# CompVis/behavior-driven-video-synthesis

Hardware: AMD Instinct MI355X
Metric: frames/sec VUnet 256x256 bs=16 fwd+bwd (higher is better)
Workload: dtype f32 (operands scaled by a power of two and split into 2 fp16 terms, 3 partial products on fp16 MFMA, fp32 accumulate; weight gradients and uncovered layers: 3 bf16 terms / 6 products, fp32-input MFMA, fp32 VALU); 1 GPU; Human3.6m shape_and_pose_net VunetAlter 256x256 per-GPU bs=16 fwd+bwd, VGG19 perceptual + KL loss, fused Adam, dropout 0.05, regressor side loop off, seeded-synthetic VGG19 weights, rasterised synthetic stickmen; global_batch=16, parallelism=dp1, conv_precision=h2, hip_streams=4, hip_graph=True, graph_settle_steps=7, rccl_world_size=1, dp_backend=none

## Files before the change

behavior_driven_video_synthesis_amd/csrc/conv_p2.hip:

```cpp
#include <stdio.h>

#include <type_traits>

#include "common.h"
#include "split_h2.h"

namespace {

constexpr int P2_META = 128, P2_AMAX0 = 16, P2_NSLOT = 64;

struct P2Args {
  const uint4* x;
  const int* xmeta;
  const uint4* w;
  const float* wk;
  const float* shift;
  const uint4* mask;
  uint4* y;
  int* ymeta;
  int N, C, H, W, M;
  int relu;
};

__device__ __forceinline__ void p2_dma(uint32_t voff, const void* sbase, uint32_t lds_addr) {
  uint32_t keep;
  asm volatile("s_mov_b32 %0, m0\n\ts_mov_b32 m0, %3\n\ts_nop 0\n\tglobal_load_lds_dwordx4 %1, %2\n\ts_mov_b32 m0, %0"
               : "=&s"(keep)
               : "v"(voff), "s"(sbase), "s"(lds_addr)
               : "memory");
}
template <int N>
__device__ __forceinline__ void p2_dma_wait() {
  static_assert(N == 0 || N == 1 || N == 2 || N == 4, "counts in use");
  if constexpr (N == 0) asm volatile("s_waitcnt vmcnt(0)" ::: "memory");
  else if constexpr (N == 1) asm volatile("s_waitcnt vmcnt(1)" ::: "memory");
  else if constexpr (N == 2) asm volatile("s_waitcnt vmcnt(2)" ::: "memory");
  else asm volatile("s_waitcnt vmcnt(4)" ::: "memory");
}
__device__ __forceinline__ const void* p2_uniform_ptr(const void* p) {
  const uint64_t v = (uint64_t)p;
  const uint32_t lo = __builtin_amdgcn_readfirstlane((uint32_t)v), hi = __builtin_amdgcn_readfirstlane((uint32_t)(v >> 32));
  return (const void*)(((uint64_t)hi << 32) | lo);
}

union P2Unit {
  uint4 u;
  h2_f16x8 b;
};

__device__ __forceinline__ float p2_meta_amax(const int* meta, int lane) {
  return wave_max(__int_as_float(meta[P2_AMAX0 + (lane & (P2_NSLOT - 1))]));
}

__device__ __forceinline__ void p2_swap16(uint32_t& a, uint32_t& b) {
  const auto r = __builtin_amdgcn_permlane16_swap(a, b, false, false);
  a = r[0];
  b = r[1];
}

__device__ __forceinline__ uint32_t p2_nonzero_halves(uint32_t t) {
  typedef unsigned short u16x2 __attribute__((ext_vector_type(2)));
  u16x2 v = __builtin_bit_cast(u16x2, t);
  const u16x2 one = {1, 1}, all = {0xFFFF, 0xFFFF};
  v = __builtin_elementwise_min(v, one) * all;
  return __builtin_bit_cast(uint32_t, v);
}

template <int NW, int CT, int XBUF>
__global__ __launch_bounds__(64 * NW, NW == 8 ? 1 : 2) void conv_p2_kernel(const P2Args a) {
  static_assert(NW == 4 || NW == 8, "waves");
  static_assert(CT == 32 || CT == 16, "tile width");
  constexpr int MW = 16 * NW;
  constexpr int RT = 8, IH = RT + 2, CW = CT + 2, XPIX = IH * CW, XU = 8 * XPIX;
  constexpr int NXI = (XU + 63) / 64, XS = NXI * 64;
  constexpr int NXW = (NXI + NW - 1) / NW;
  constexpr int WU = MW * 8;
  constexpr int NWI = WU / 64 / NW;
  constexpr int PTR = CT / 16, NPT = 2 * PTR;
  static_assert(XBUF == 1 || NXW <= 8, "the next chunk's pieces ride on the first taps");
  extern __shared__ __attribute__((aligned(16))) uint4 smem[];
  uint4* const xL = smem;
  uint4* const wL = smem + XBUF * XS;

  const int tid = threadIdx.x, lane = tid & 63;
  const int wave = __builtin_amdgcn_readfirstlane(tid >> 6);
  const int mg = wave >> 2, rg = wave & 3;
  const int px = lane & 15, cg = lane >> 4;
  const int Hp = a.H + 2, Wp = a.W + 2, CB = a.C >> 3, MB = a.M >> 3;

  const unsigned bid = xcd_remap(blockIdx.x, gridDim.x);
  const int mblocks = a.M / MW;
  const int mb = bid % mblocks;
  int t = bid / mblocks;
  const int tiles_w = a.W / CT, tiles_h = a.H / RT;
  const int tx = t % tiles_w;
  t /= tiles_w;
  const int ty = t % tiles_h;
  const int n = t / tiles_h;
  const int row0 = ty * RT, col0 = tx * CT, m0 = mb * MW;

  uint32_t xoff[NXW];
#pragma unroll
  for (int i = 0; i < NXW; ++i) {
    int j = wave + NW * i;
    if (j >= NXI) j = NXI - 1;
    int u = 64 * j + lane;
    if (u >= XU) u = XU - 1;
    const int p = u / (4 * XPIX);
    int rem = u - p * 4 * XPIX;
    const int kq = rem / XPIX;
    rem -= kq * XPIX;
    const int r = rem / CW, c = rem - r * CW;
    xoff[i] = (uint32_t)((((size_t)p * a.N * CB + kq) * Hp + (row0 + r)) * Wp + col0 + c) * 16u;
  }
  const uint32_t xL_addr = (uint32_t)(uintptr_t)(__attribute__((address_space(3))) void*)xL;
  const uint32_t wL_addr = (uint32_t)(uintptr_t)(__attribute__((address_space(3))) void*)wL;
  const char* const xsrc0 = reinterpret_cast<const char*>(a.x) + (size_t)n * CB * Hp * Wp * 16;
  const size_t xchunk = (size_t)4 * Hp * Wp * 16;
  const char* const wsrc0 = reinterpret_cast<const char*>(a.w) + (size_t)mb * (MW / 16) * 128 * 16;
  const size_t wslab = (size_t)(a.M / 16) * 128 * 16;
  const uint32_t lane16 = (uint32_t)lane * 16u;

  auto issue_x = [&](int ch, int i) {
    int j = wave + NW * i;
    if (j >= NXI) j = NXI - 1;
    const int xb = XBUF == 2 ? (ch & 1) : 0;
    p2_dma(xoff[i], p2_uniform_ptr(xsrc0 + (size_t)ch * xchunk), xL_addr + (uint32_t)(xb * XS + 64 * j) * 16u);
  };
  auto issue_w = [&](int g, int buf) {
    const char* src = wsrc0 + (size_t)g * wslab;
#pragma unroll
    for (int i = 0; i < NWI; ++i) {
      const int part = wave * NWI + i;
      p2_dma(lane16, p2_uniform_ptr(src + (size_t)part * 1024), wL_addr + (uint32_t)(buf * WU + part * 64) * 16u);
    }
  };

  issue_w(0, 0);
#pragma unroll
  for (int i = 0; i < NXW; ++i) issue_x(0, i);

  float descale, descale2, sy;
  {
    const int ex = a.xmeta[0];
    const float amax_x = p2_meta_amax(a.xmeta, lane);
    const int ew = (int)a.wk[2];
    h2_pow2_pair(-(ex + ew), descale, descale2);
    const float bound = a.wk[0] * amax_x + a.wk[1];
    const int ey = h2_scale_exp(bound);
    sy = h2_pow2(ey);
    if (blockIdx.x == 0 && tid == 0) a.ymeta[0] = ey;
  }

  f32x4 acc[4][NPT], acx[4][NPT];
#pragma unroll
  for (int mt = 0; mt < 4; ++mt)
#pragma unroll
    for (int q = 0; q < NPT; ++q)
#pragma unroll
      for (int r = 0; r < 4; ++r) acc[mt][q][r] = acx[mt][q][r] = 0.f;

  p2_dma_wait<0>();
  __syncthreads();

  const int nch = a.C >> 5;
  const uint4* const wA0 = wL + (mg * 4) * 128 + lane;
  const uint4* const xB0 = xL + cg * XPIX + px + (2 * rg) * CW;

  auto chunk = [&](int ch, auto last_c) {
    constexpr bool LAST = decltype(last_c)::value;
    const uint4* const xB = xB0 + (XBUF == 2 ? (ch & 1) * XS : 0);
    const int wpar = (ch * 9) & 1;
#pragma unroll
    for (int tap = 0; tap < 9; ++tap) {
      const int kh = tap / 3, kw = tap - 3 * kh;
      const int g = ch * 9 + tap;
      const int buf = wpar ^ (tap & 1);
      constexpr bool dummy = false;
      (void)dummy;
      const bool more_w = !(LAST && tap == 8);
      const bool xpiece = XBUF == 2 && !LAST && tap < NXW;
      if (more_w) issue_w(g + 1, buf ^ 1);
      if (xpiece) issue_x(ch + 1, tap);
      const uint4* const wA = wA0 + buf * WU;
      P2Unit av[2][4], bv[2][NPT];
#pragma unroll
      for (int p = 0; p < 2; ++p) {
#pragma unroll
        for (int mt = 0; mt < 4; ++mt) av[p][mt].u = wA[(mt * 2 + p) * 64];
#pragma unroll
        for (int q = 0; q < NPT; ++q) bv[p][q].u = xB[p * 4 * XPIX + (q / PTR + kh) * CW + (q % PTR) * 16 + kw];
      }
#pragma unroll
      for (int mt = 0; mt < 4; ++mt)
#pragma unroll
        for (int q = 0; q < NPT; ++q)
          acx[mt][q] = __builtin_amdgcn_mfma_f32_16x16x32_f16(av[1][mt].b, bv[0][q].b, acx[mt][q], 0, 0, 0);
#pragma unroll
      for (int mt = 0; mt < 4; ++mt)
#pragma unroll
        for (int q = 0; q < NPT; ++q)
          acx[mt][q] = __builtin_amdgcn_mfma_f32_16x16x32_f16(av[0][mt].b, bv[1][q].b, acx[mt][q], 0, 0, 0);
#pragma unroll
      for (int mt = 0; mt < 4; ++mt)
#pragma unroll
        for (int q = 0; q < NPT; ++q)
          acc[mt][q] = __builtin_amdgcn_mfma_f32_16x16x32_f16(av[0][mt].b, bv[0][q].b, acc[mt][q], 0, 0, 0);
      __builtin_amdgcn_sched_barrier(0);
      if (more_w) {
        if (xpiece) p2_dma_wait<1>();
        else p2_dma_wait<0>();
        __syncthreads();
        if (XBUF == 1 && tap == 8) {
#pragma unroll
          for (int i = 0; i < NXW; ++i) issue_x(ch + 1, i);
          p2_dma_wait<0>();
          __syncthreads();
        }
      }
    }
  };
  for (int ch = 0; ch + 1 < nch; ++ch) chunk(ch, std::false_type{});
  chunk(nch - 1, std::true_type{});

  const bool relu = a.relu != 0;
  const size_t plane = (size_t)a.N * MB * Hp * Wp;
  float ymax = 0.f;
#pragma unroll
  for (int mt = 0; mt < 4; ++mt) {
    const int co = m0 + 64 * mg + 16 * mt + 4 * cg;
    float sh[4] = {0.f, 0.f, 0.f, 0.f};
    if (a.shift) {
      const float4 s4 = *reinterpret_cast<const float4*>(a.shift + co);
      sh[0] = s4.x; sh[1] = s4.y; sh[2] = s4.z; sh[3] = s4.w;
    }
#pragma unroll
    for (int qp = 0; qp < NPT; qp += 2) {
      uint32_t hh[2][2], ll[2][2];
#pragma unroll
      for (int s = 0; s < 2; ++s) {
        float v[4];
#pragma unroll
        for (int r = 0; r < 4; ++r) {
          float c = (acc[mt][qp + s][r] + acx[mt][qp + s][r] * (1.f / 2048.f)) * descale * descale2 + sh[r];
          c = (relu && !(c > 0.f)) ? 0.f : c;
          ymax = fmaxf(ymax, fabsf(c));
          v[r] = c * sy;
        }
        h2_split2(v[0], v[1], hh[s][0], ll[s][0]);
        h2_split2(v[2], v[3], hh[s][1], ll[s][1]);
      }
      p2_swap16(hh[0][0], hh[1][0]);
      p2_swap16(hh[0][1], hh[1][1]);
      p2_swap16(ll[0][0], ll[1][0]);
      p2_swap16(ll[0][1], ll[1][1]);
      uint4 uh = make_uint4(hh[0][0], hh[0][1], hh[1][0], hh[1][1]);
      uint4 ul = make_uint4(ll[0][0], ll[0][1], ll[1][0], ll[1][1]);
      const int q = qp + (cg & 1);
      const int orow = row0 + 2 * rg + q / PTR, ocol = col0 + (q % PTR) * 16 + px;
      const int cb = ((m0 + 64 * mg + 16 * mt) >> 3) + (cg >> 1);
      const size_t o = (((size_t)n * MB + cb) * Hp + (orow + 1)) * Wp + (ocol + 1);
      if (a.mask) {
        const uint4 mh = a.mask[o], ml = a.mask[plane + o];
        const uint32_t k0 = p2_nonzero_halves((mh.x | ml.x) & 0x7FFF7FFFu), k1 = p2_nonzero_halves((mh.y | ml.y) & 0x7FFF7FFFu);
        const uint32_t k2 = p2_nonzero_halves((mh.z | ml.z) & 0x7FFF7FFFu), k3 = p2_nonzero_halves((mh.w | ml.w) & 0x7FFF7FFFu);
        uh.x &= k0; uh.y &= k1; uh.z &= k2; uh.w &= k3;
        ul.x &= k0; ul.y &= k1; ul.z &= k2; ul.w &= k3;
      }
      a.y[o] = uh;
      a.y[plane + o] = ul;
    }
  }
  {
    const float m_ = wave_max(ymax);
    if (lane == 0)
      atomicMax(reinterpret_cast<unsigned*>(a.ymeta) + P2_AMAX0 + ((blockIdx.x * NW + wave) & (P2_NSLOT - 1)), __float_as_uint(m_));
  }
}

template <int CT>
__global__ __launch_bounds__(512, 1) void conv_p2a_kernel(const P2Args a) {
  constexpr int NW = 8, MW = 128;
  constexpr int RT = 8, IH = RT + 2, CW = CT + 2, XPIX = IH * CW, XU = 8 * XPIX;
  constexpr int NXI = (XU + 63) / 64, XS = NXI * 64;
  constexpr int NXG = (NXI + 3) / 4;
  constexpr int XPT = 2, NXT = (NXG + XPT - 1) / XPT;
  constexpr int WU = MW * 8;
  constexpr int PTR = CT / 16, NPT = 2 * PTR;
  static_assert(NXT <= 8, "the next chunk's pieces must be visible before its first tap");
  extern __shared__ __attribute__((aligned(16))) uint4 smem[];
  uint4* const xL = smem;
  uint4* const wL = smem + 2 * XS;

  const int tid = threadIdx.x, lane = tid & 63;
  const int wave = __builtin_amdgcn_readfirstlane(tid >> 6);
  const int mg = wave >> 2, rg = wave & 3;
  const int px = lane & 15, cg = lane >> 4;
  const int Hp = a.H + 2, Wp = a.W + 2, CB = a.C >> 3, MB = a.M >> 3;

  const unsigned bid = xcd_remap(blockIdx.x, gridDim.x);
  const int mblocks = a.M / MW;
  const int mb = bid % mblocks;
  int t = bid / mblocks;
  const int tiles_w = a.W / CT, tiles_h = a.H / RT;
  const int tx = t % tiles_w;
  t /= tiles_w;
  const int ty = t % tiles_h;
  const int n = t / tiles_h;
  const int row0 = ty * RT, col0 = tx * CT, m0 = mb * MW;

  uint32_t xoff[NXG];
#pragma unroll
  for (int i = 0; i < NXG; ++i) {
    int j = rg + 4 * i;
    if (j >= NXI) j = NXI - 1;
    int u = 64 * j + lane;
    if (u >= XU) u = XU - 1;
    const int p = u / (4 * XPIX);
    int rem = u - p * 4 * XPIX;
    const int kq = rem / XPIX;
    rem -= kq * XPIX;
    const int r = rem / CW, c = rem - r * CW;
    xoff[i] = (uint32_t)((((size_t)p * a.N * CB + kq) * Hp + (row0 + r)) * Wp + col0 + c) * 16u;
  }
  const uint32_t xL_addr = (uint32_t)(uintptr_t)(__attribute__((address_space(3))) void*)xL;
  const uint32_t wL_addr = (uint32_t)(uintptr_t)(__attribute__((address_space(3))) void*)wL;
  const char* const xsrc0 = reinterpret_cast<const char*>(a.x) + (size_t)n * CB * Hp * Wp * 16;
  const size_t xchunk = (size_t)4 * Hp * Wp * 16;
  const char* const wsrc0 = reinterpret_cast<const char*>(a.w) + (size_t)mb * (MW / 16) * 128 * 16;
  const size_t wslab = (size_t)(a.M / 16) * 128 * 16;
  const uint32_t lane16 = (uint32_t)lane * 16u;

  auto issue_x = [&](int ch, int i) {
    int j = rg + 4 * i;
    if (j >= NXI) j = NXI - 1;
    p2_dma(xoff[i], p2_uniform_ptr(xsrc0 + (size_t)ch * xchunk), xL_addr + (uint32_t)((ch & 1) * XS + 64 * j) * 16u);
  };
  auto issue_w = [&](int g, int buf) {
    const char* src = wsrc0 + (size_t)g * wslab;
#pragma unroll
    for (int i = 0; i < 4; ++i) {
      const int part = rg * 4 + i;
      p2_dma(lane16, p2_uniform_ptr(src + (size_t)part * 1024), wL_addr + (uint32_t)(buf * WU + part * 64) * 16u);
    }
  };

  if (mg == 0) issue_w(0, 0);
  else {
#pragma unroll
    for (int i = 0; i < NXG; ++i) issue_x(0, i);
  }
  float descale, descale2, sy;
  {
    const int ex = a.xmeta[0];
    const float amax_x = p2_meta_amax(a.xmeta, lane);
    const int ew = (int)a.wk[2];
    h2_pow2_pair(-(ex + ew), descale, descale2);
    const float bound = a.wk[0] * amax_x + a.wk[1];
    const int ey = h2_scale_exp(bound);
    sy = h2_pow2(ey);
    if (blockIdx.x == 0 && tid == 0) a.ymeta[0] = ey;
  }
  f32x4 acc[4][NPT], acx[4][NPT];
#pragma unroll
  for (int mt = 0; mt < 4; ++mt)
#pragma unroll
    for (int q = 0; q < NPT; ++q)
#pragma unroll
      for (int r = 0; r < 4; ++r) acc[mt][q][r] = acx[mt][q][r] = 0.f;
  p2_dma_wait<0>();
  __syncthreads();
  if (mg == 1) __builtin_amdgcn_s_barrier();

  const int nch = a.C >> 5;
  const uint4* const wA0 = wL + (mg * 4) * 128 + lane;
  const uint4* const xB0 = xL + cg * XPIX + px + (2 * rg) * CW;

  auto chunk = [&](int ch, auto last_c) {
    constexpr bool LAST = decltype(last_c)::value;
    const uint4* const xB = xB0 + (ch & 1) * XS;
    const int wpar = (ch * 9) & 1;
#pragma unroll
    for (int tap = 0; tap < 9; ++tap) {
      const int kh = tap / 3, kw = tap - 3 * kh;
      const int g = ch * 9 + tap;
      const int buf = wpar ^ (tap & 1);
      const bool more_w = !(LAST && tap == 8);
      if (mg == 0) {
        if (more_w) issue_w(g + 1, buf ^ 1);
      } else if (!LAST && tap < NXT) {
#pragma unroll
        for (int i = 0; i < XPT; ++i)
          if (tap * XPT + i < NXG) issue_x(ch + 1, tap * XPT + i);
      }
      const uint4* const wA = wA0 + buf * WU;
      P2Unit av[2][4], bv[2][NPT];
#pragma unroll
      for (int p = 0; p < 2; ++p) {
#pragma unroll
        for (int mt = 0; mt < 4; ++mt) av[p][mt].u = wA[(mt * 2 + p) * 64];
#pragma unroll
        for (int q = 0; q < NPT; ++q) bv[p][q].u = xB[p * 4 * XPIX + (q / PTR + kh) * CW + (q % PTR) * 16 + kw];
      }
      asm volatile("s_waitcnt lgkmcnt(0)" ::: "memory");
      __builtin_amdgcn_sched_barrier(0);
      __builtin_amdgcn_s_barrier();
      __builtin_amdgcn_sched_barrier(0);
      __builtin_amdgcn_s_setprio(1);
#pragma unroll
      for (int mt = 0; mt < 4; ++mt)
#pragma unroll
        for (int q = 0; q < NPT; ++q)
          acx[mt][q] = __builtin_amdgcn_mfma_f32_16x16x32_f16(av[1][mt].b, bv[0][q].b, acx[mt][q], 0, 0, 0);
#pragma unroll
      for (int mt = 0; mt < 4; ++mt)
#pragma unroll
        for (int q = 0; q < NPT; ++q)
          acx[mt][q] = __builtin_amdgcn_mfma_f32_16x16x32_f16(av[0][mt].b, bv[1][q].b, acx[mt][q], 0, 0, 0);
#pragma unroll
      for (int mt = 0; mt < 4; ++mt)
#pragma unroll
        for (int q = 0; q < NPT; ++q)
          acc[mt][q] = __builtin_amdgcn_mfma_f32_16x16x32_f16(av[0][mt].b, bv[0][q].b, acc[mt][q], 0, 0, 0);
      __builtin_amdgcn_s_setprio(0);
      __builtin_amdgcn_sched_barrier(0);
      p2_dma_wait<0>();
      __builtin_amdgcn_s_barrier();
      __builtin_amdgcn_sched_barrier(0);
    }
  };
  for (int ch = 0; ch + 1 < nch; ++ch) chunk(ch, std::false_type{});
  chunk(nch - 1, std::true_type{});
  if (mg == 0) __builtin_amdgcn_s_barrier();

  const bool relu = a.relu != 0;
  const size_t plane = (size_t)a.N * MB * Hp * Wp;
  float ymax = 0.f;
#pragma unroll
  for (int mt = 0; mt < 4; ++mt) {
    const int co = m0 + 64 * mg + 16 * mt + 4 * cg;
    float sh[4] = {0.f, 0.f, 0.f, 0.f};
    if (a.shift) {
      const float4 s4 = *reinterpret_cast<const float4*>(a.shift + co);
      sh[0] = s4.x; sh[1] = s4.y; sh[2] = s4.z; sh[3] = s4.w;
    }
#pragma unroll
    for (int qp = 0; qp < NPT; qp += 2) {
      uint32_t hh[2][2], ll[2][2];
#pragma unroll
      for (int s = 0; s < 2; ++s) {
        float v[4];
#pragma unroll
        for (int r = 0; r < 4; ++r) {
          float c = (acc[mt][qp + s][r] + acx[mt][qp + s][r] * (1.f / 2048.f)) * descale * descale2 + sh[r];
          c = (relu && !(c > 0.f)) ? 0.f : c;
          ymax = fmaxf(ymax, fabsf(c));
          v[r] = c * sy;
        }
        h2_split2(v[0], v[1], hh[s][0], ll[s][0]);
        h2_split2(v[2], v[3], hh[s][1], ll[s][1]);
      }
      p2_swap16(hh[0][0], hh[1][0]);
      p2_swap16(hh[0][1], hh[1][1]);
      p2_swap16(ll[0][0], ll[1][0]);
      p2_swap16(ll[0][1], ll[1][1]);
      uint4 uh = make_uint4(hh[0][0], hh[0][1], hh[1][0], hh[1][1]);
      uint4 ul = make_uint4(ll[0][0], ll[0][1], ll[1][0], ll[1][1]);
      const int q = qp + (cg & 1);
      const int orow = row0 + 2 * rg + q / PTR, ocol = col0 + (q % PTR) * 16 + px;
      const int cb = ((m0 + 64 * mg + 16 * mt) >> 3) + (cg >> 1);
      const size_t o = (((size_t)n * MB + cb) * Hp + (orow + 1)) * Wp + (ocol + 1);
      if (a.mask) {
        const uint4 mh = a.mask[o], ml = a.mask[plane + o];
        const uint32_t k0 = p2_nonzero_halves((mh.x | ml.x) & 0x7FFF7FFFu), k1 = p2_nonzero_halves((mh.y | ml.y) & 0x7FFF7FFFu);
        const uint32_t k2 = p2_nonzero_halves((mh.z | ml.z) & 0x7FFF7FFFu), k3 = p2_nonzero_halves((mh.w | ml.w) & 0x7FFF7FFFu);
        uh.x &= k0; uh.y &= k1; uh.z &= k2; uh.w &= k3;
        ul.x &= k0; ul.y &= k1; ul.z &= k2; ul.w &= k3;
      }
      a.y[o] = uh;
      a.y[plane + o] = ul;
    }
  }
  {
    const float m_ = wave_max(ymax);
    if (lane == 0)
      atomicMax(reinterpret_cast<unsigned*>(a.ymeta) + P2_AMAX0 + ((blockIdx.x * NW + wave) & (P2_NSLOT - 1)), __float_as_uint(m_));
  }
}

template <int CT>
int p2a_launch(const P2Args& a, hipStream_t st) {
  constexpr int XU = 8 * 10 * (CT + 2), XS = (XU + 63) / 64 * 64, WU = 128 * 8;
  constexpr size_t lds = (size_t)(2 * XS + 2 * WU) * 16;
  const int blocks = a.N * (a.H / 8) * (a.W / CT) * (a.M / 128);
  auto kern = conv_p2a_kernel<CT>;
  if (hipFuncSetAttribute((const void*)kern, hipFuncAttributeMaxDynamicSharedMemorySize, (int)lds) != hipSuccess) return VUNET_ERR_LAUNCH;
  VUNET_LAUNCH(kern, dim3((unsigned)blocks), dim3(512), lds, st, a);
  return vunet_check_launch();
}

template <int NW, int CT, int XBUF>
int p2_launch(const P2Args& a, hipStream_t st) {
  constexpr int XU = 8 * 10 * (CT + 2), XS = (XU + 63) / 64 * 64, WU = 16 * NW * 8;
  constexpr size_t lds = (size_t)(XBUF * XS + 2 * WU) * 16;
  const int blocks = a.N * (a.H / 8) * (a.W / CT) * (a.M / (16 * NW));
  auto kern = conv_p2_kernel<NW, CT, XBUF>;
  if (lds > 64 * 1024 && hipFuncSetAttribute((const void*)kern, hipFuncAttributeMaxDynamicSharedMemorySize, (int)lds) != hipSuccess)
    return VUNET_ERR_LAUNCH;
  VUNET_LAUNCH(kern, dim3((unsigned)blocks), dim3(64 * NW), lds, st, a);
  return vunet_check_launch();
}

}

static bool p2_shape_ok(const vunet_p2_desc* d) {
  if (!d || d->N < 1 || d->C < 32 || d->C % 32 || d->M < 64 || d->M % 64 || d->H < 8 || d->H % 8) return false;
  if (!(d->W == 16 || (d->W >= 32 && d->W % 32 == 0))) return false;
  const double plane_bytes = (double)d->N * (d->C / 8) * (d->H + 2) * (d->W + 2) * 16.0;
  return plane_bytes * 2.0 < 4.0e9;
}

extern "C" int vunet_p2_conv_supported(const vunet_p2_desc* d) { return p2_shape_ok(d) ? 1 : 0; }

static int p2_form(const vunet_p2_desc* d) {
  const long px_tiles = (long)d->N * (d->H / 8) * (d->W / (d->W == 16 ? 16 : 32));
  const int force = g_vunet_tune[VUNET_TUNE_P2_FORM];
  const bool wide = d->M % 128 == 0 && (force == 2 || force == 3 || (force != 1 && px_tiles * (d->M / 128) >= 256));
  return wide ? 8 : 4;
}

extern "C" int vunet_p2_conv(const vunet_p2_desc* d, const void* x, const int32_t* xmeta, const void* w_image, const float* wk,
                             const float* shift, const void* mask, void* y, int32_t* ymeta, void* stream) {
  if (!d || !x || !xmeta || !w_image || !wk || !y || !ymeta) return VUNET_ERR_ARG;
  if (!p2_shape_ok(d)) return VUNET_ERR_UNSUPPORTED;
  if (((uintptr_t)x | (uintptr_t)w_image | (uintptr_t)y | (uintptr_t)mask | (uintptr_t)shift) & 15) return VUNET_ERR_ARG;
  P2Args a;
  a.x = (const uint4*)x; a.xmeta = xmeta; a.w = (const uint4*)w_image; a.wk = wk; a.shift = shift; a.mask = (const uint4*)mask;
  a.y = (uint4*)y; a.ymeta = ymeta;
  a.N = d->N; a.C = d->C; a.H = d->H; a.W = d->W; a.M = d->M; a.relu = d->relu;
  hipStream_t st = (hipStream_t)stream;
  const int form = p2_form(d);
  const bool lockstep = g_vunet_tune[VUNET_TUNE_P2_FORM] == 3;
  if (d->W == 16) return form == 8 ? (lockstep ? p2_launch<8, 16, 2>(a, st) : p2a_launch<16>(a, st)) : p2_launch<4, 16, 1>(a, st);
  return form == 8 ? (lockstep ? p2_launch<8, 32, 2>(a, st) : p2a_launch<32>(a, st)) : p2_launch<4, 32, 1>(a, st);
}

extern "C" int vunet_p2_conv_variant(const vunet_p2_desc* d, char* name, int32_t len) {
  if (!d || !name || len < 32) return VUNET_ERR_ARG;
  if (!p2_shape_ok(d)) return VUNET_ERR_UNSUPPORTED;
  const int form = p2_form(d);
  if (form == 8 && g_vunet_tune[VUNET_TUNE_P2_FORM] != 3) snprintf(name, (size_t)len, "conv_p2a_kernel<%d>", d->W == 16 ? 16 : 32);
  else snprintf(name, (size_t)len, "conv_p2_kernel<%d, %d, %d>", form, d->W == 16 ? 16 : 32, form == 8 ? 2 : 1);
  return VUNET_OK;
}

namespace {
__global__ __launch_bounds__(256) void p2_wstat_kernel(const float* __restrict__ w, int Cout, int Cin, int dgrad,
                                                       float* __restrict__ rows) {
  __shared__ float red[8];
  const int r = blockIdx.x;
  float s = 0.f, m = 0.f;
  const int K = dgrad ? Cout : Cin;
  for (int i = threadIdx.x; i < K * 9; i += 256) {
    const int k = i / 9, t = i - 9 * k;
    const float v = fabsf(dgrad ? w[((size_t)k * Cin + r) * 9 + t] : w[((size_t)r * Cin + k) * 9 + t]);
    s += v;
    m = fmaxf(m, v);
  }
  s = wave_sum(s);
  m = wave_max(m);
  if ((threadIdx.x & 63) == 0) {
    red[threadIdx.x >> 6] = s;
    red[4 + (threadIdx.x >> 6)] = m;
  }
  __syncthreads();
  if (threadIdx.x == 0) {
    rows[2 * r] = (red[0] + red[1]) + (red[2] + red[3]);
    rows[2 * r + 1] = fmaxf(fmaxf(red[4], red[5]), fmaxf(red[6], red[7]));
  }
}
__global__ __launch_bounds__(256) void p2_wk_kernel(const float* __restrict__ rows, int R, const float* __restrict__ shift,
                                                    int nshift, float* __restrict__ wk) {
  __shared__ float red[12];
  float s = 0.f, m = 0.f, b = 0.f;
  for (int i = threadIdx.x; i < R; i += 256) {
    s = fmaxf(s, rows[2 * i]);
    m = fmaxf(m, rows[2 * i + 1]);
  }
  for (int i = threadIdx.x; i < nshift; i += 256) b = fmaxf(b, fabsf(shift[i]));
  s = wave_max(s);
  m = wave_max(m);
  b = wave_max(b);
  if ((threadIdx.x & 63) == 0) {
    red[threadIdx.x >> 6] = s;
    red[4 + (threadIdx.x >> 6)] = m;
    red[8 + (threadIdx.x >> 6)] = b;
  }
  __syncthreads();
  if (threadIdx.x == 0) {
    const float mx = fmaxf(fmaxf(red[4], red[5]), fmaxf(red[6], red[7]));
    wk[0] = fmaxf(fmaxf(red[0], red[1]), fmaxf(red[2], red[3])) * (1.f + 1e-6f);
    wk[1] = fmaxf(fmaxf(red[8], red[9]), fmaxf(red[10], red[11]));
    wk[2] = (float)h2_scale_exp(mx);
    wk[3] = mx;
  }
}
__global__ __launch_bounds__(256) void p2_wpack_kernel(const float* __restrict__ w, int Cout, int Cin, int dgrad,
                                                       const float* __restrict__ wk, uint4* __restrict__ img) {
  const int R = dgrad ? Cin : Cout, K = dgrad ? Cout : Cin;
  const int MT = R / 16;
  const size_t units = (size_t)(K / 32) * 9 * MT * 2 * 64;
  const float sw = h2_pow2((int)wk[2]);
  for (size_t u = (size_t)blockIdx.x * 256 + threadIdx.x; u < units; u += (size_t)gridDim.x * 256) {
    size_t v = u;
    const int l = (int)(v & 63);
    v >>= 6;
    const int p = (int)(v & 1);
    v >>= 1;
    const int mt = (int)(v % MT);
    v /= MT;
    const int tap = (int)(v % 9);
    const int ch = (int)(v / 9);
    const int row = mt * 16 + (l & 15), k0 = ch * 32 + (l >> 4) * 8;
    const int kh = tap / 3, kw = tap - 3 * kh;
    float e[8];
#pragma unroll
    for (int j = 0; j < 8; ++j) {
      const int k = k0 + j;
      const float x = dgrad ? w[(((size_t)k * Cin + row) * 3 + (2 - kh)) * 3 + (2 - kw)] : w[(((size_t)row * Cin + k) * 3 + kh) * 3 + kw];
      e[j] = x * sw;
    }
    uint32_t h[4], lo[4];
#pragma unroll
    for (int j = 0; j < 4; ++j) h2_split2(e[2 * j], e[2 * j + 1], h[j], lo[j]);
    img[u] = p ? make_uint4(lo[0], lo[1], lo[2], lo[3]) : make_uint4(h[0], h[1], h[2], h[3]);
  }
}
}

extern "C" int vunet_p2_weight_image_bytes(int32_t Cout, int32_t Cin, int32_t dgrad) {
  const int R = dgrad ? Cin : Cout, K = dgrad ? Cout : Cin;
  if (R < 16 || R % 16 || K < 32 || K % 32 || (int64_t)R * K > (1 << 22)) return 0;
  return (K / 32) * 9 * (R / 16) * 2 * 64 * 16;
}

extern "C" int vunet_p2_pack_weights(const float* w, const float* shift, int32_t Cout, int32_t Cin, int32_t dgrad, void* image,
                                     float* wk, float* workspace, void* stream) {
  if (!w || !image || !wk || !workspace) return VUNET_ERR_ARG;
  if (vunet_p2_weight_image_bytes(Cout, Cin, dgrad) == 0) return VUNET_ERR_UNSUPPORTED;
  const int R = dgrad ? Cin : Cout;
  hipStream_t st = (hipStream_t)stream;
  VUNET_LAUNCH(p2_wstat_kernel, dim3((unsigned)R), dim3(256), 0, st, w, (int)Cout, (int)Cin, (int)dgrad, workspace);
  VUNET_LAUNCH(p2_wk_kernel, dim3(1), dim3(256), 0, st, (const float*)workspace, R, dgrad ? nullptr : shift,
               (dgrad || !shift) ? 0 : (int)Cout, wk);
  const size_t units = (size_t)vunet_p2_weight_image_bytes(Cout, Cin, dgrad) / 16;
  size_t nb = (units + 255) / 256;
  if (nb > 2048) nb = 2048;
  VUNET_LAUNCH(p2_wpack_kernel, dim3((unsigned)nb), dim3(256), 0, st, w, (int)Cout, (int)Cin, (int)dgrad, (const float*)wk,
               (uint4*)image);
  return vunet_check_launch();
}

extern "C" int vunet_p2_weight_bound(const float* w, const float* shift, int32_t Cout, int32_t Cin, float* wk, float* workspace,
                                     void* stream) {
  if (!w || !wk || !workspace || Cout < 1 || Cin < 1) return VUNET_ERR_ARG;
  hipStream_t st = (hipStream_t)stream;
  VUNET_LAUNCH(p2_wstat_kernel, dim3((unsigned)Cout), dim3(256), 0, st, w, (int)Cout, (int)Cin, 0, workspace);
  VUNET_LAUNCH(p2_wk_kernel, dim3(1), dim3(256), 0, st, (const float*)workspace, (int)Cout, shift, shift ? (int)Cout : 0, wk);
  return vunet_check_launch();
}

namespace {
__global__ __launch_bounds__(256) void p2_from_nchw_kernel(const float* __restrict__ x, const float* __restrict__ amax, int n_amax,
                                                           int relu, uint4* __restrict__ y, int* __restrict__ ymeta, int N, int C,
                                                           int H, int W) {
  __shared__ float red[4];
  float m = 0.f;
  for (int i = threadIdx.x; i < n_amax; i += 256) m = fmaxf(m, amax[i]);
  m = wave_max(m);
  if ((threadIdx.x & 63) == 0) red[threadIdx.x >> 6] = m;
  __syncthreads();
  m = fmaxf(fmaxf(red[0], red[1]), fmaxf(red[2], red[3]));
  const int e = h2_scale_exp(m);
  const float s = h2_pow2(e);
  if (blockIdx.x == 0 && threadIdx.x == 0) {
    ymeta[0] = e;
    ymeta[P2_AMAX0] = __float_as_int(m);
  }
  const int CB = C >> 3, Hp = H + 2, Wp = W + 2;
  const size_t HW = (size_t)H * W, total = (size_t)N * CB * HW, plane = (size_t)N * CB * Hp * Wp;
  for (size_t i = (size_t)blockIdx.x * 256 + threadIdx.x; i < total; i += (size_t)gridDim.x * 256) {
    const int xw = (int)(i % W);
    size_t t = i / W;
    const int yh = (int)(t % H);
    t /= H;
    const float* src = x + (t * 8) * HW + (size_t)yh * W + xw;
    float v[8];
#pragma unroll
    for (int j = 0; j < 8; ++j) {
      float f = src[j * HW];
      if (relu) f = f > 0.f ? f : 0.f;
      v[j] = f * s;
    }
    uint4 h, l;
    h2_split2(v[0], v[1], h.x, l.x);
    h2_split2(v[2], v[3], h.y, l.y);
    h2_split2(v[4], v[5], h.z, l.z);
    h2_split2(v[6], v[7], h.w, l.w);
    const size_t o = (t * Hp + (yh + 1)) * Wp + (xw + 1);
    y[o] = h;
    y[plane + o] = l;
  }
}
__device__ __forceinline__ void p2_unpack(const uint4& h, const uint4& l, float inv, float* v) {
  const uint32_t hs[4] = {h.x, h.y, h.z, h.w}, ls[4] = {l.x, l.y, l.z, l.w};
#pragma unroll
  for (int j = 0; j < 4; ++j) {
    const h2_f16x2 a = __builtin_bit_cast(h2_f16x2, hs[j]), b = __builtin_bit_cast(h2_f16x2, ls[j]);
    v[2 * j] = ((float)a[0] + (float)b[0] * (1.f / 2048.f)) * inv;
    v[2 * j + 1] = ((float)a[1] + (float)b[1] * (1.f / 2048.f)) * inv;
  }
}
__global__ __launch_bounds__(256) void p2_to_nchw_kernel(const uint4* __restrict__ x, const int* __restrict__ xmeta,
                                                         float* __restrict__ y, int N, int C, int H, int W) {
  const int CB = C >> 3, Hp = H + 2, Wp = W + 2;
  const float inv = h2_pow2(-xmeta[0]);
  const size_t HW = (size_t)H * W, total = (size_t)N * CB * HW, plane = (size_t)N * CB * Hp * Wp;
  for (size_t i = (size_t)blockIdx.x * 256 + threadIdx.x; i < total; i += (size_t)gridDim.x * 256) {
    const int xw = (int)(i % W);
    size_t t = i / W;
    const int yh = (int)(t % H);
    t /= H;
    const size_t o = (t * Hp + (yh + 1)) * Wp + (xw + 1);
    float v[8];
    p2_unpack(x[o], x[plane + o], inv, v);
    float* dst = y + (t * 8) * HW + (size_t)yh * W + xw;
#pragma unroll
    for (int j = 0; j < 8; ++j) dst[j * HW] = v[j];
  }
}
}

extern "C" int vunet_p2_from_nchw(const float* x, const float* amax, int32_t n_amax, int32_t relu, void* y, int32_t* ymeta,
                                  int32_t N, int32_t C, int32_t H, int32_t W, void* stream) {
  if (!x || !amax || n_amax < 1 || !y || !ymeta || C % 8 || N < 1) return VUNET_ERR_ARG;
  const size_t total = (size_t)N * (C / 8) * H * W;
  size_t nb = (total + 255) / 256;
  if (nb > 4096) nb = 4096;
  VUNET_LAUNCH(p2_from_nchw_kernel, dim3((unsigned)nb), dim3(256), 0, (hipStream_t)stream, x, amax, (int)n_amax, (int)relu, (uint4*)y,
               (int*)ymeta, (int)N, (int)C, (int)H, (int)W);
  return vunet_check_launch();
}

extern "C" int vunet_p2_to_nchw(const void* x, const int32_t* xmeta, float* y, int32_t N, int32_t C, int32_t H, int32_t W,
                                void* stream) {
  if (!x || !xmeta || !y || C % 8 || N < 1) return VUNET_ERR_ARG;
  const size_t total = (size_t)N * (C / 8) * H * W;
  size_t nb = (total + 255) / 256;
  if (nb > 4096) nb = 4096;
  VUNET_LAUNCH(p2_to_nchw_kernel, dim3((unsigned)nb), dim3(256), 0, (hipStream_t)stream, (const uint4*)x, (const int*)xmeta, y, (int)N,
               (int)C, (int)H, (int)W);
  return vunet_check_launch();
}
```

behavior_driven_video_synthesis_amd/csrc/planes.hip:

```cpp
#include "common.h"
#include "split_h2.h"

namespace {

constexpr int P2_AMAX0 = 16, P2_NSLOT = 64;

__device__ __forceinline__ void p2_unpack8(const uint4& h, const uint4& l, float inv, float* v) {
  const uint32_t hs[4] = {h.x, h.y, h.z, h.w}, ls[4] = {l.x, l.y, l.z, l.w};
#pragma unroll
  for (int j = 0; j < 4; ++j) {
    const h2_f16x2 a = __builtin_bit_cast(h2_f16x2, hs[j]), b = __builtin_bit_cast(h2_f16x2, ls[j]);
    v[2 * j] = ((float)a[0] + (float)b[0] * (1.f / 2048.f)) * inv;
    v[2 * j + 1] = ((float)a[1] + (float)b[1] * (1.f / 2048.f)) * inv;
  }
}
__device__ __forceinline__ void p2_pack8(const float* v, float s, uint4& h, uint4& l) {
  h2_split2(v[0] * s, v[1] * s, h.x, l.x);
  h2_split2(v[2] * s, v[3] * s, h.y, l.y);
  h2_split2(v[4] * s, v[5] * s, h.z, l.z);
  h2_split2(v[6] * s, v[7] * s, h.w, l.w);
}
__device__ __forceinline__ float block_sum4(float v, float* red) {
  v = wave_sum(v);
  __syncthreads();
  if ((threadIdx.x & 63) == 0) red[threadIdx.x >> 6] = v;
  __syncthreads();
  return red[0] + red[1] + red[2] + red[3];
}
__device__ __forceinline__ float meta_amax(const int* meta) {
  return wave_max(__int_as_float(meta[P2_AMAX0 + (threadIdx.x & (P2_NSLOT - 1))]));
}
__device__ __forceinline__ void publish_amax(int* meta, float vmax) {
  const float m = wave_max(vmax);
  if ((threadIdx.x & 63) == 0)
    atomicMax(reinterpret_cast<unsigned*>(meta) + P2_AMAX0 + ((blockIdx.x * 4u + (threadIdx.x >> 6)) & (P2_NSLOT - 1)), __float_as_uint(m));
}

__global__ __launch_bounds__(256) void p2_finish_sum_kernel(const float* partial, int nb, float* out, float scale) {
  __shared__ float red[4];
  float s = 0.f;
  for (int i = threadIdx.x; i < nb; i += 256) s += partial[i];
  const float t = block_sum4(s, red);
  if (threadIdx.x == 0) out[0] += scale * t;
}

__global__ __launch_bounds__(256) void p2_l1_partial_kernel(const uint4* __restrict__ t, const int* __restrict__ tmeta,
                                                            const uint4* __restrict__ p, const int* __restrict__ pmeta,
                                                            float* __restrict__ partial, size_t plane) {
  __shared__ float red[4];
  const float it = h2_pow2(-tmeta[0]), ip = h2_pow2(-pmeta[0]);
  float s = 0.f;
  for (size_t i = (size_t)blockIdx.x * 256 + threadIdx.x; i < plane; i += (size_t)gridDim.x * 256) {
    float a[8], b[8];
    p2_unpack8(t[i], t[plane + i], it, a);
    p2_unpack8(p[i], p[plane + i], ip, b);
    s += ((fabsf(a[0] - b[0]) + fabsf(a[1] - b[1])) + (fabsf(a[2] - b[2]) + fabsf(a[3] - b[3]))) +
         ((fabsf(a[4] - b[4]) + fabsf(a[5] - b[5])) + (fabsf(a[6] - b[6]) + fabsf(a[7] - b[7])));
  }
  const float tot = block_sum4(s, red);
  if (threadIdx.x == 0) partial[blockIdx.x] = tot;
}

template <bool L1>
__global__ __launch_bounds__(256) void p2_pool_fwd_kernel(const uint4* __restrict__ t, const int* __restrict__ tmeta,
                                                          const uint4* __restrict__ p, const int* __restrict__ pmeta,
                                                          float* __restrict__ partial, uint4* __restrict__ y, int* __restrict__ ymeta,
                                                          int NCB, int H, int W) {
  __shared__ float red[4];
  const int Ho = H >> 1, Wo = W >> 1, Wp = W + 2, Wpo = Wo + 2;
  const size_t plane = (size_t)NCB * (H + 2) * Wp, plane_o = (size_t)NCB * (Ho + 2) * Wpo, total = (size_t)NCB * Ho * Wo;
  const float ip = h2_pow2(-pmeta[0]);
  const float it = L1 ? h2_pow2(-tmeta[0]) : 0.f;
  if (blockIdx.x == 0 && threadIdx.x < 64) {
    if (threadIdx.x == 0) ymeta[0] = pmeta[0];
    ymeta[P2_AMAX0 + threadIdx.x] = pmeta[P2_AMAX0 + threadIdx.x];
  }
  float s = 0.f;
  for (size_t o = (size_t)blockIdx.x * 256 + threadIdx.x; o < total; o += (size_t)gridDim.x * 256) {
    const int xo = (int)(o % Wo);
    size_t r = o / Wo;
    const int yo = (int)(r % Ho);
    const size_t ncb = r / Ho;
    const size_t i0 = (ncb * (H + 2) + (2 * yo + 1)) * Wp + (2 * xo + 1);
    const size_t off[4] = {i0, i0 + 1, i0 + Wp, i0 + Wp + 1};
    uint32_t hs[4][4], ls[4][4];
    float v[4][8];
#pragma unroll
    for (int e = 0; e < 4; ++e) {
      const uint4 h = p[off[e]], l = p[plane + off[e]];
      hs[e][0] = h.x; hs[e][1] = h.y; hs[e][2] = h.z; hs[e][3] = h.w;
      ls[e][0] = l.x; ls[e][1] = l.y; ls[e][2] = l.z; ls[e][3] = l.w;
      p2_unpack8(h, l, ip, v[e]);
    }
    if (L1) {
#pragma unroll
      for (int e = 0; e < 4; ++e) {
        float a[8];
        p2_unpack8(t[off[e]], t[plane + off[e]], it, a);
#pragma unroll
        for (int j = 0; j < 8; ++j) s += fabsf(a[j] - v[e][j]);
      }
    }
    uint32_t oh[4] = {0, 0, 0, 0}, ol[4] = {0, 0, 0, 0};
#pragma unroll
    for (int j = 0; j < 8; ++j) {
      const float m = fmaxf(fmaxf(v[0][j], v[1][j]), fmaxf(v[2][j], v[3][j]));
      const int k = v[0][j] == m ? 0 : (v[1][j] == m ? 1 : (v[2][j] == m ? 2 : 3));
      const uint32_t hsel = k == 0 ? hs[0][j >> 1] : (k == 1 ? hs[1][j >> 1] : (k == 2 ? hs[2][j >> 1] : hs[3][j >> 1]));
      const uint32_t lsel = k == 0 ? ls[0][j >> 1] : (k == 1 ? ls[1][j >> 1] : (k == 2 ? ls[2][j >> 1] : ls[3][j >> 1]));
      const uint32_t keep = (j & 1) ? 0xFFFF0000u : 0x0000FFFFu;
      oh[j >> 1] |= hsel & keep;
      ol[j >> 1] |= lsel & keep;
    }
    const size_t oo = (ncb * (Ho + 2) + (yo + 1)) * Wpo + (xo + 1);
    y[oo] = make_uint4(oh[0], oh[1], oh[2], oh[3]);
    y[plane_o + oo] = make_uint4(ol[0], ol[1], ol[2], ol[3]);
  }
  if (L1) {
    const float tot = block_sum4(s, red);
    if (threadIdx.x == 0) partial[blockIdx.x] = tot;
  }
}

__global__ __launch_bounds__(256) void p2_l1_bwd_kernel(const uint4* __restrict__ t, const int* __restrict__ tmeta,
                                                        const uint4* __restrict__ p, const int* __restrict__ pmeta,
                                                        const uint4* __restrict__ add, const int* __restrict__ addmeta,
                                                        uint4* __restrict__ g, int* __restrict__ gmeta, float gscale,
                                                        const float* __restrict__ gout, int NCB, int H, int W) {
  const float c = gscale * (gout ? gout[0] : 1.f);
  const float bound = (add ? meta_amax(addmeta) : 0.f) + fabsf(c);
  const int eg = h2_scale_exp(bound);
  const float sg = h2_pow2(eg);
  if (blockIdx.x == 0 && threadIdx.x == 0) gmeta[0] = eg;
  const float it = h2_pow2(-tmeta[0]), ip = h2_pow2(-pmeta[0]), ia = add ? h2_pow2(-addmeta[0]) : 0.f;
  const int Wp = W + 2;
  const size_t plane = (size_t)NCB * (H + 2) * Wp, total = (size_t)NCB * H * W;
  float vmax = 0.f;
  for (size_t o = (size_t)blockIdx.x * 256 + threadIdx.x; o < total; o += (size_t)gridDim.x * 256) {
    const int xw = (int)(o % W);
    size_t r = o / W;
    const int yh = (int)(r % H);
    const size_t i = ((r / H) * (H + 2) + (yh + 1)) * Wp + (xw + 1);
    float a[8], b[8], d[8];
    p2_unpack8(t[i], t[plane + i], it, a);
    p2_unpack8(p[i], p[plane + i], ip, b);
    if (add) p2_unpack8(add[i], add[plane + i], ia, d);
#pragma unroll
    for (int j = 0; j < 8; ++j) {
      const float df = b[j] - a[j];
      float v = (add ? d[j] : 0.f) + (df > 0.f ? c : (df < 0.f ? -c : 0.f));
      if (!(b[j] > 0.f)) v = 0.f;
      d[j] = v;
      vmax = fmaxf(vmax, fabsf(v));
    }
    uint4 h, l;
    p2_pack8(d, sg, h, l);
    g[i] = h;
    g[plane + i] = l;
  }
  publish_amax(gmeta, vmax);
}

template <bool L1>
__global__ __launch_bounds__(256) void p2_pool_bwd_kernel(const uint4* __restrict__ t, const int* __restrict__ tmeta,
                                                          const uint4* __restrict__ p, const int* __restrict__ pmeta,
                                                          const uint4* __restrict__ dy, const int* __restrict__ dymeta,
                                                          uint4* __restrict__ g, int* __restrict__ gmeta, float gscale,
                                                          const float* __restrict__ gout, int NCB, int H, int W) {
  const float c = L1 ? gscale * (gout ? gout[0] : 1.f) : 0.f;
  const float bound = meta_amax(dymeta) + fabsf(c);
  const int eg = h2_scale_exp(bound);
  const float sg = h2_pow2(eg);
  if (blockIdx.x == 0 && threadIdx.x == 0) gmeta[0] = eg;
  const float ip = h2_pow2(-pmeta[0]), idy = h2_pow2(-dymeta[0]);
  const float it = L1 ? h2_pow2(-tmeta[0]) : 0.f;
  const int Ho = H >> 1, Wo = W >> 1, Wp = W + 2, Wpo = Wo + 2;
  const size_t plane = (size_t)NCB * (H + 2) * Wp, plane_o = (size_t)NCB * (Ho + 2) * Wpo, total = (size_t)NCB * Ho * Wo;
  float vmax = 0.f;
  for (size_t o = (size_t)blockIdx.x * 256 + threadIdx.x; o < total; o += (size_t)gridDim.x * 256) {
    const int xo = (int)(o % Wo);
    size_t r = o / Wo;
    const int yo = (int)(r % Ho);
    const size_t ncb = r / Ho;
    const size_t i0 = (ncb * (H + 2) + (2 * yo + 1)) * Wp + (2 * xo + 1);
    const size_t off[4] = {i0, i0 + 1, i0 + Wp, i0 + Wp + 1};
    const size_t oo = (ncb * (Ho + 2) + (yo + 1)) * Wpo + (xo + 1);
    float v[4][8], gy[8];
#pragma unroll
    for (int e = 0; e < 4; ++e) p2_unpack8(p[off[e]], p[plane + off[e]], ip, v[e]);
    p2_unpack8(dy[oo], dy[plane_o + oo], idy, gy);
    float res[4][8];
#pragma unroll
    for (int j = 0; j < 8; ++j) {
      const float m = fmaxf(fmaxf(v[0][j], v[1][j]), fmaxf(v[2][j], v[3][j]));
      const int k = v[0][j] == m ? 0 : (v[1][j] == m ? 1 : (v[2][j] == m ? 2 : 3));
#pragma unroll
      for (int e = 0; e < 4; ++e) res[e][j] = k == e ? gy[j] : 0.f;
    }
#pragma unroll
    for (int e = 0; e < 4; ++e) {
      float a[8];
      if (L1) p2_unpack8(t[off[e]], t[plane + off[e]], it, a);
#pragma unroll
      for (int j = 0; j < 8; ++j) {
        float x = res[e][j];
        if (L1) {
          const float df = v[e][j] - a[j];
          x += df > 0.f ? c : (df < 0.f ? -c : 0.f);
        }
        if (!(v[e][j] > 0.f)) x = 0.f;
        res[e][j] = x;
        vmax = fmaxf(vmax, fabsf(x));
      }
      uint4 h, l;
      p2_pack8(res[e], sg, h, l);
      g[off[e]] = h;
      g[plane + off[e]] = l;
    }
  }
  publish_amax(gmeta, vmax);
}

inline unsigned grid_for(size_t n, unsigned cap) {
  size_t b = (n + 255) / 256;
  if (b > cap) b = cap;
  if (b < 1) b = 1;
  return (unsigned)b;
}

}

extern "C" int vunet_p2_l1_fwd(const void* t, const int32_t* tmeta, const void* p, const int32_t* pmeta, float* partial, float* out,
                               float weight, int32_t N, int32_t C, int32_t H, int32_t W, void* stream) {
  if (!t || !tmeta || !p || !pmeta || !partial || !out || C % 8 || N < 1) return VUNET_ERR_ARG;
  const size_t plane = (size_t)N * (C / 8) * (H + 2) * (W + 2);
  const unsigned nb = grid_for(plane, 1024);
  hipStream_t st = (hipStream_t)stream;
  VUNET_LAUNCH(p2_l1_partial_kernel, dim3(nb), dim3(256), 0, st, (const uint4*)t, (const int*)tmeta, (const uint4*)p, (const int*)pmeta,
               partial, plane);
  VUNET_LAUNCH(p2_finish_sum_kernel, dim3(1), dim3(256), 0, st, (const float*)partial, (int)nb, out,
               weight / ((float)N * C * H * W));
  return vunet_check_launch();
}

extern "C" int vunet_p2_pool_fwd(const void* t, const int32_t* tmeta, const void* p, const int32_t* pmeta, float* partial, float* out,
                                 float weight, void* y, int32_t* ymeta, int32_t N, int32_t C, int32_t H, int32_t W, void* stream) {
  if (!p || !pmeta || !y || !ymeta || C % 8 || N < 1 || (H & 1) || (W & 1)) return VUNET_ERR_ARG;
  if (t && (!tmeta || !partial || !out)) return VUNET_ERR_ARG;
  const int NCB = N * (C / 8);
  const size_t total = (size_t)NCB * (H / 2) * (W / 2);
  const unsigned nb = grid_for(total, 1024);
  hipStream_t st = (hipStream_t)stream;
  if (t) {
    VUNET_LAUNCH(p2_pool_fwd_kernel<true>, dim3(nb), dim3(256), 0, st, (const uint4*)t, (const int*)tmeta, (const uint4*)p,
                 (const int*)pmeta, partial, (uint4*)y, (int*)ymeta, NCB, (int)H, (int)W);
    VUNET_LAUNCH(p2_finish_sum_kernel, dim3(1), dim3(256), 0, st, (const float*)partial, (int)nb, out,
                 weight / ((float)N * C * H * W));
  } else {
    VUNET_LAUNCH(p2_pool_fwd_kernel<false>, dim3(nb), dim3(256), 0, st, (const uint4*)nullptr, (const int*)nullptr, (const uint4*)p,
                 (const int*)pmeta, (float*)nullptr, (uint4*)y, (int*)ymeta, NCB, (int)H, (int)W);
  }
  return vunet_check_launch();
}

extern "C" int vunet_p2_l1_bwd(const void* t, const int32_t* tmeta, const void* p, const int32_t* pmeta, const void* add,
                               const int32_t* addmeta, void* g, int32_t* gmeta, float gscale, const float* gout, int32_t N, int32_t C,
                               int32_t H, int32_t W, void* stream) {
  if (!t || !tmeta || !p || !pmeta || !g || !gmeta || C % 8 || N < 1 || (add && !addmeta)) return VUNET_ERR_ARG;
  const int NCB = N * (C / 8);
  const size_t total = (size_t)NCB * H * W;
  VUNET_LAUNCH(p2_l1_bwd_kernel, dim3(grid_for(total, 2048)), dim3(256), 0, (hipStream_t)stream, (const uint4*)t, (const int*)tmeta,
               (const uint4*)p, (const int*)pmeta, (const uint4*)add, (const int*)addmeta, (uint4*)g, (int*)gmeta, gscale, gout, NCB,
               (int)H, (int)W);
  return vunet_check_launch();
}

extern "C" int vunet_p2_pool_bwd(const void* t, const int32_t* tmeta, const void* p, const int32_t* pmeta, const void* dy,
                                 const int32_t* dymeta, void* g, int32_t* gmeta, float gscale, const float* gout, int32_t N, int32_t C,
                                 int32_t H, int32_t W, void* stream) {
  if (!p || !pmeta || !dy || !dymeta || !g || !gmeta || C % 8 || N < 1 || (H & 1) || (W & 1) || (t && !tmeta)) return VUNET_ERR_ARG;
  const int NCB = N * (C / 8);
  const size_t total = (size_t)NCB * (H / 2) * (W / 2);
  const unsigned nb = grid_for(total, 2048);
  hipStream_t st = (hipStream_t)stream;
  if (t)
    VUNET_LAUNCH(p2_pool_bwd_kernel<true>, dim3(nb), dim3(256), 0, st, (const uint4*)t, (const int*)tmeta, (const uint4*)p,
                 (const int*)pmeta, (const uint4*)dy, (const int*)dymeta, (uint4*)g, (int*)gmeta, gscale, gout, NCB, (int)H, (int)W);
  else
    VUNET_LAUNCH(p2_pool_bwd_kernel<false>, dim3(nb), dim3(256), 0, st, (const uint4*)nullptr, (const int*)nullptr, (const uint4*)p,
                 (const int*)pmeta, (const uint4*)dy, (const int*)dymeta, (uint4*)g, (int*)gmeta, 0.f, (const float*)nullptr, NCB, (int)H,
                 (int)W);
  return vunet_check_launch();
}
```

behavior_driven_video_synthesis_amd/models/imagenet_pretrained.py:

```python
from __future__ import annotations

import math

import torch
from torch import nn

from .. import ops
from ..lib.modules import Conv2d

VGG19_CFG = [64, 64, "M", 128, 128, "M", 256, 256, 256, 256, "M", 512, 512, 512, 512, "M", 512, 512, 512, 512, "M"]


class _Marker(nn.Module):

    def __init__(self, kind):
        super().__init__()
        self.kind = kind


class VGG19(nn.Module):

    def __init__(self, width_div: int = 1):
        super().__init__()
        layers, cin = [], 3
        for v in VGG19_CFG:
            if v == "M":
                layers.append(_Marker("pool"))
            else:
                cout = max(v // width_div, 4)
                layers += [Conv2d(cin, cout, 3, padding=1), _Marker("relu")]
                cin = cout
        self.features = nn.Sequential(*layers)

    def init_synthetic(self, seed: int = 1234):
        g = torch.Generator().manual_seed(seed)
        with torch.no_grad():
            for m in self.features:
                if isinstance(m, Conv2d):
                    cout, cin = m.weight.shape[:2]
                    m.weight.copy_(torch.randn(cout, cin, 3, 3, generator=g) * math.sqrt(2.0 / (cin * 9)))
                    m.bias.copy_((torch.rand(cout, generator=g) - 0.5) * 0.1)
        return self


def vgg19(pretrained: bool = False, weights_path: str = None, width_div: int = 1, seed: int = 1234,
          synthetic: bool = False) -> VGG19:
    if pretrained and weights_path is None and not synthetic:
        import warnings
        warnings.warn("vgg19(pretrained=True) without weights_path: torchvision's weights cannot be fetched here, "
                      "using SEEDED-SYNTHETIC VGG19 weights (pass weights_path=<torchvision vgg19 state dict>, or "
                      "synthetic=True to silence this)", stacklevel=2)
    net = VGG19(width_div)
    if weights_path is not None:
        sd = torch.load(weights_path, map_location="cpu")
        net.load_state_dict({k: v for k, v in sd.items() if k.startswith("features.")})
    else:
        net.init_synthetic(seed)
    return net


def _adopt_features(features: nn.Sequential) -> nn.Sequential:
    mods = list(features)
    if all(isinstance(m, (Conv2d, _Marker)) for m in mods):
        return features
    layers = []
    for m in mods:
        if isinstance(m, nn.Conv2d):
            if m.kernel_size != (3, 3) or m.stride != (1, 1) or m.padding != (1, 1) or m.bias is None:
                raise NotImplementedError("PerceptualVGG expects VGG-style 3x3 / stride 1 / pad 1 convolutions with bias")
            c = Conv2d(m.in_channels, m.out_channels, 3, padding=1)
            with torch.no_grad():
                c.weight.copy_(m.weight)
                c.bias.copy_(m.bias)
            layers.append(c.to(m.weight.device))
        elif isinstance(m, nn.ReLU):
            layers.append(_Marker("relu"))
        elif isinstance(m, nn.MaxPool2d):
            layers.append(_Marker("pool"))
        else:
            raise NotImplementedError(f"PerceptualVGG: unexpected module {type(m).__name__} in vgg.features")
    return nn.Sequential(*layers)


_p2_switch = {"on": __import__("os").environ.get("VUNET_VGG_P2", "1") != "0"}


def enable_p2(on: bool = True):
    _p2_switch["on"] = bool(on)


class _P2Target(dict):

    planes = None
    generation = 0


class _P2Engine:

    def __init__(self, program, n, h, w, device):
        self.program, self.geo, self.device = program, (n, h, w), device
        self.roles = {}
        self.generation = 0
        self.pred_generation = 0

    @staticmethod
    def build_program(mods, last, taps):
        steps, first, i = [], None, 0
        while i < len(mods):
            name, m = mods[i]
            if int(name) > last:
                break
            if isinstance(m, Conv2d):
                nxt = mods[i + 1] if i + 1 < len(mods) else None
                if nxt is None or not (isinstance(nxt[1], _Marker) and nxt[1].kind == "relu"):
                    return None
                tap = taps.get(nxt[0])
                if first is None:
                    if tap is not None:
                        return None
                    first = m
                else:
                    steps.append(("conv", m, tap))
                i += 2
            elif isinstance(m, _Marker) and m.kind == "pool":
                if first is None:
                    return None
                steps.append(("pool",))
                i += 1
            else:
                return None
        if first is None or not steps or steps[-1][0] != "conv" or steps[-1][2] is None:
            return None
        return first, steps

    def shapes(self):
        first, steps = self.program
        n, h, w = self.geo
        c = first.weight.shape[0]
        out = [(c, h, w)]
        for st in steps:
            if st[0] == "pool":
                if h % 2 or w % 2:
                    return None
                h, w = h // 2, w // 2
            else:
                m = st[1]
                if m.weight.shape[1] != c or tuple(m.weight.shape[2:]) != (3, 3) or not ops.p2_conv_supported(n, c, h, w, m.weight.shape[0]):
                    return None
                if not ops.p2_conv_supported(n, m.weight.shape[0], h, w, c):
                    return None
                c = m.weight.shape[0]
            out.append((c, h, w))
        return out

    def _role(self, role):
        st = self.roles.get(role)
        if st is None:
            shp = self.shapes()
            n = self.geo[0]
            L = len(shp)
            metas = torch.zeros(3 * L, ops.P2_META_INTS, device=self.device, dtype=torch.int32)
            acts = [ops.Planes((n, c, h, w), self.device, meta=metas[k]) for k, (c, h, w) in enumerate(shp)]
            st = self.roles[role] = {"metas": metas, "A": acts, "G": [None] * L, "U": [None] * L, "shp": shp}
        return st

    def _grad_buf(self, st, kind, k):
        lst = st[kind]
        if lst[k] is None:
            c, h, w = st["shp"][k]
            L = len(st["shp"])
            lst[k] = ops.Planes((self.geo[0], c, h, w), self.device, meta=st["metas"][(1 if kind == "G" else 2) * L + k])
        return lst[k]

    @staticmethod
    def _weights(m):
        w = m.__dict__.get("_p2w")
        if w is None or w.weight is not m.weight:
            w = ops.P2Weights(m.weight, m.bias)
            object.__setattr__(m, "_p2w", w)
        return w

    def _first(self):
        m = self.program[0]
        stamp = (m.weight.data_ptr(), m.weight._version, m.bias._version)
        rec = m.__dict__.get("_p2first")
        if rec is None or rec[0] != stamp:
            w, b = m.weight.detach().contiguous(), m.bias.detach().contiguous()
            wt_f, wt_d, _, shift, _, _, wx_d = ops.pack_weights(w, None, b, None, None, 3, 0, 1, True)
            wk = torch.empty(4, device=w.device, dtype=torch.float32)
            work = torch.empty(2 * w.shape[0], device=w.device, dtype=torch.float32)
            ops._call("vunet_p2_weight_bound", ops._p(w), ops._p(b), int(w.shape[0]), 3, ops._p(wk), ops._p(work), ops._stream())
            rec = (stamp, wt_f, wt_d, shift, wx_d, wk)
            object.__setattr__(m, "_p2first", rec)
        return rec

    def forward(self, role, xp, targets=None, tap_weights=None):
        st = self._role(role)
        st["metas"].zero_()
        A = st["A"]
        _, wt_f, _, shift, _, wk = self._first()
        n, _, h, w = xp.shape
        amax = ops._tagged_amax(xp)
        if amax is None:
            amax = ops.absmax_partials(xp)
        ops._call("vunet_p2_conv_first", ops._p(xp), ops._p(amax), 512, ops._p(wt_f), int(wt_f.shape[1]), ops._p(shift), ops._p(wk),
                  ops._p(A[0].buf), ops._p(A[0].meta), n, h, w, A[0].shape[1], ops._stream())
        taps, losses = {}, {}
        steps = self.program[1]
        for k, step in enumerate(steps, start=1):
            if step[0] == "conv":
                ops.p2_conv(A[k - 1], self._weights(step[1]), A[k], relu=True)
                tap = step[2]
                if tap is not None:
                    taps[tap] = A[k]
                    pool_next = k < len(steps) and steps[k][0] == "pool"
                    if targets is not None and not pool_next:
                        losses[tap] = ops.p2_l1_fwd(targets[tap], A[k], tap_weights[tap])
            else:
                prev = steps[k - 2] if k >= 2 else None
                tap = prev[2] if (prev is not None and prev[0] == "conv") else None
                if targets is not None and tap is not None:
                    losses[tap] = ops.p2_pool_fwd(A[k - 1], A[k], t=targets[tap], weight=tap_weights[tap])
                else:
                    ops.p2_pool_fwd(A[k - 1], A[k])
        return taps, losses

    def backward(self, targets, tap_weights, gouts):
        st = self.roles["p"]
        A, steps = st["A"], self.program[1]
        L = len(steps)

        def tap_scale(tap, k):
            c, h, w = st["shp"][k]
            return float(tap_weights[tap]) / (self.geo[0] * c * h * w)

        def has(tap):
            return tap is not None and gouts.get(tap) is not None
        k = L
        top = steps[L - 1][2]
        D = None
        if has(top):
            D = ops.p2_l1_bwd(targets[top], A[L], None, self._grad_buf(st, "G", L), tap_scale(top, L), gouts[top])
        while k >= 1:
            step = steps[k - 1]
            if step[0] == "pool":
                prev = steps[k - 2]
                tap = prev[2] if has(prev[2]) else None
                if D is None and tap is None:
                    k -= 1
                    continue
                if D is None:
                    D = ops.p2_l1_bwd(targets[tap], A[k - 1], None, self._grad_buf(st, "G", k - 1), tap_scale(tap, k - 1), gouts[tap])
                else:
                    D = ops.p2_pool_bwd(A[k - 1], D, self._grad_buf(st, "G", k - 1), t=None if tap is None else targets[tap],
                                        gscale=0.0 if tap is None else tap_scale(tap, k - 1), gout=None if tap is None else gouts[tap])
                k -= 1
                continue
            below = steps[k - 2] if k >= 2 else None
            if D is None:
                tap = below[2] if (below is not None and below[0] == "conv" and has(below[2])) else None
                if tap is not None:
                    D = ops.p2_l1_bwd(targets[tap], A[k - 1], None, self._grad_buf(st, "G", k - 1), tap_scale(tap, k - 1), gouts[tap])
                k -= 1
                continue
            wts = self._weights(step[1])
            if below is None:
                D = ops.p2_conv(D, wts, self._grad_buf(st, "G", 0), dgrad=True, mask=A[0])
            elif below[0] == "pool":
                D = ops.p2_conv(D, wts, self._grad_buf(st, "G", k - 1), dgrad=True)
            elif has(below[2]):
                up = ops.p2_conv(D, wts, self._grad_buf(st, "U", k - 1), dgrad=True)
                D = ops.p2_l1_bwd(targets[below[2]], A[k - 1], up, self._grad_buf(st, "G", k - 1), tap_scale(below[2], k - 1),
                                  gouts[below[2]])
            else:
                D = ops.p2_conv(D, wts, self._grad_buf(st, "G", k - 1), dgrad=True, mask=A[k - 1])
            k -= 1
        if D is None:
            return None
        _, _, wt_d, _, wx_d, _ = self._first()
        n, h, w = self.geo
        c0 = st["shp"][0][0]
        dconv = D.to_nchw()
        dx = torch.empty(n, 3, h, w, device=self.device, dtype=torch.float32)
        d = ops.ConvDesc(N=n, C1=c0, C2=0, Hs=h, Ws=w, M=3, m_off=0, Mpad=wt_d.shape[1], Ho=h, Wo=w, KH=3, KW=3, stride=1, pad=1,
                         mode=1, in_act=ops.ACT_NONE, in_slope=0.0, drop_p=0.0, drop_seed=0, out_act=ops.ACT_NONE, d2s=0)
        ops._conv_gather(d, dconv, None, wt_d, None, None, None, dx, wx_d)
        return dx


class P2VggLoss(torch.autograd.Function):

    @staticmethod
    def forward(ctx, xp, engine, target, tap_weights, names):
        _, losses = engine.forward("p", xp, target.planes, tap_weights)
        engine.pred_generation += 1
        ctx.engine, ctx.target, ctx.tap_weights, ctx.names = engine, target, tap_weights, names
        ctx.generation, ctx.pred_generation = target.generation, engine.pred_generation
        return tuple(losses[n] for n in names)

    @staticmethod
    def backward(ctx, *gouts):
        if ctx.target.generation != ctx.generation:
            raise RuntimeError("P2VggLoss.backward: the target features were overwritten by a later target pass of the same "
                               "PerceptualVGG (its planes buffers are persistent): run forward + backward per target")
        if ctx.engine.pred_generation != ctx.pred_generation:
            raise RuntimeError("P2VggLoss.backward: a later vgg_loss() of the same PerceptualVGG and input geometry has overwritten "
                               "this pass's activations (persistent planes buffers): call backward() before the next vgg_loss(), "
                               "or switch the planes path off (models.imagenet_pretrained.enable_p2(False)) for this use")
        g = ctx.engine.backward(ctx.target.planes, ctx.tap_weights,
                                {n: (None if go is None else go.contiguous()) for n, go in zip(ctx.names, gouts)})
        return g, None, None, None, None


class PerceptualVGG(nn.Module):

    def __init__(self, vgg, weights):
        super().__init__()
        feats = vgg.module.features if isinstance(vgg, nn.DataParallel) else vgg.features
        self.vgg_layers = _adopt_features(feats)
        self.loss_weights = weights
        self.register_buffer("mean", torch.tensor([0.485, 0.456, 0.406], dtype=torch.float).view(1, 3, 1, 1))
        self.register_buffer("std", torch.tensor([0.229, 0.224, 0.225], dtype=torch.float).view(1, 3, 1, 1))
        self.target_layers = {"3": "relu1_2", "8": "relu2_2", "13": "relu3_2", "22": "relu4_2", "31": "relu5_2"}
        for p in self.vgg_layers.parameters():
            p.requires_grad_(False)

    def _walk(self, x, on_tap, on_tap_pool=None):
        x = on_tap("input", ops.VggPreprocess.apply(x))
        last = max(int(k) for k in self.target_layers)
        mods = list(self.vgg_layers._modules.items())
        i = 0
        while i < len(mods):
            name, m = mods[i]
            if int(name) > last:
                break
            if isinstance(m, Conv2d):
                nxt = mods[i + 1][1] if i + 1 < len(mods) else None
                if isinstance(nxt, _Marker) and nxt.kind == "relu":
                    x = m.fused(x, out_act=ops.ACT_RELU)
                    i += 1
                    name = mods[i][0]
                else:
                    x = m(x)
            elif m.kind == "pool":
                x = ops.MaxPool2.apply(x)
            else:
                x = ops.Activation.apply(x, ops.ACT_RELU, 0.0)
            if name in self.target_layers:
                nxt = mods[i + 1][1] if i + 1 < len(mods) else None
                if (on_tap_pool is not None and isinstance(nxt, _Marker) and nxt.kind == "pool"
                        and int(mods[i + 1][0]) <= last):
                    x = on_tap_pool(self.target_layers[name], x)
                    i += 1
                else:
                    x = on_tap(self.target_layers[name], x)
            i += 1

    def forward(self, x):
        out = {}

        def keep(name, t):
            out[name] = t
            return t
        self._walk(x, keep)
        return out

    def _p2_engine(self, x):
        if not (_p2_switch["on"] and x.is_cuda and x.dim() == 4 and ops.conv_precision() == "h2"):
            return None
        cache = self.__dict__.setdefault("_p2_engines", {})
        key = (tuple(x.shape), x.device.index)
        if key not in cache:
            eng = None
            prog = _P2Engine.build_program(list(self.vgg_layers._modules.items()), max(int(k) for k in self.target_layers),
                                           self.target_layers)
            if prog is not None and not any(p.requires_grad for p in self.vgg_layers.parameters()):
                eng = _P2Engine(prog, x.shape[0], x.shape[2], x.shape[3], x.device)
                first = prog[0]
                if (eng.shapes() is None or x.shape[1] != 3 or first.weight.shape[1] != 3 or x.shape[2] % 32 or x.shape[3] % 32
                        or first.weight.shape[0] % 8 or first.weight.shape[0] > 128):
                    eng = None
            cache[key] = eng
        return cache[key]

    def _tap_weights(self):
        names = ["input"] + [self.target_layers[k] for k in sorted(self.target_layers, key=int)]
        return dict(zip(names, (float(w) for w in self.loss_weights)))

    def features_for_loss(self, x):
        eng = self._p2_engine(x)
        if eng is None or torch.is_grad_enabled():
            return self.forward(x)
        xp = ops.VggPreprocess.apply(x)
        taps, _ = eng.forward("t", xp)
        out = _P2Target({"input": xp})
        out.update({k: v.buf for k, v in taps.items()})
        out.planes = taps
        eng.generation += 1
        out.generation = eng.generation
        out.engine = eng
        return out

    def loss_terms(self, pred, target_features):
        weights = dict(zip(["input"] + [self.target_layers[k] for k in sorted(self.target_layers, key=int)],
                           self.loss_weights))
        losses = {}
        if isinstance(target_features, _P2Target):
            eng = target_features.engine
            if target_features.generation != eng.generation:
                raise RuntimeError("loss_terms: these target features were overwritten by a later features_for_loss() call")
            xp = ops.VggPreprocess.apply(pred)
            losses["input"], xp_alias = ops.L1MeanThrough.apply(target_features["input"], xp, float(weights["input"]))
            ops.carry_amax_tag(xp, xp_alias)
            names = tuple(st[2] for st in eng.program[1] if st[0] == "conv" and st[2] is not None)
            terms = P2VggLoss.apply(xp_alias, eng, target_features, self._tap_weights(), names)
            losses.update(dict(zip(names, terms)))
            return losses

        def term(name, t):
            losses[name], alias = ops.L1MeanThrough.apply(target_features[name], t, float(weights[name]))
            ops.carry_amax_tag(t, alias)
            return alias
        def term_pool(name, t):
            losses[name], pooled = ops.L1ThroughPool.apply(target_features[name], t, float(weights[name]))
            return pooled
        self._walk(pred, term, term_pool if ops.l1_pool_fusion["on"] else None)
        return losses
```

behavior_driven_video_synthesis_amd/ops.py:

```python
from __future__ import annotations

import contextlib
import ctypes
import os
from dataclasses import dataclass
from typing import Optional, Tuple

import torch

from . import _lib

ACT_NONE, ACT_ELU, ACT_RELU, ACT_SIGMOID, ACT_LRELU = 0, 1, 2, 3, 4
SEED2_OFFSET = 0x9E3779B9


class ConvDesc(ctypes.Structure):
    _fields_ = [("N", ctypes.c_int32), ("C1", ctypes.c_int32), ("C2", ctypes.c_int32), ("Hs", ctypes.c_int32),
                ("Ws", ctypes.c_int32), ("M", ctypes.c_int32), ("m_off", ctypes.c_int32), ("Mpad", ctypes.c_int32),
                ("Ho", ctypes.c_int32), ("Wo", ctypes.c_int32), ("KH", ctypes.c_int32), ("KW", ctypes.c_int32),
                ("stride", ctypes.c_int32), ("pad", ctypes.c_int32), ("mode", ctypes.c_int32),
                ("in_act", ctypes.c_int32), ("in_slope", ctypes.c_float), ("drop_p", ctypes.c_float),
                ("drop_seed", ctypes.c_uint32), ("out_act", ctypes.c_int32), ("d2s", ctypes.c_int32),
                ("aux_act", ctypes.c_int32), ("aux_slope", ctypes.c_float), ("aux_drop_p", ctypes.c_float),
                ("aux_drop_seed", ctypes.c_uint32)]


class WgradDesc(ctypes.Structure):
    _fields_ = [("N", ctypes.c_int32), ("C1", ctypes.c_int32), ("C2", ctypes.c_int32), ("Hs", ctypes.c_int32),
                ("Ws", ctypes.c_int32), ("Cout", ctypes.c_int32), ("Ho", ctypes.c_int32), ("Wo", ctypes.c_int32),
                ("KH", ctypes.c_int32), ("KW", ctypes.c_int32), ("stride", ctypes.c_int32), ("pad", ctypes.c_int32),
                ("in_act", ctypes.c_int32), ("in_slope", ctypes.c_float), ("drop_p", ctypes.c_float),
                ("drop_seed", ctypes.c_uint32), ("nsplit", ctypes.c_int32), ("flags", ctypes.c_int32)]


class WgradItem(ctypes.Structure):
    _fields_ = [("d", WgradDesc)] + [(n, ctypes.c_void_p) for n in ("x1", "x2", "dy", "slabs", "dshift", "amax_x", "amax_x2",
                                                                   "amax_dy")]


class WnDesc(ctypes.Structure):
    _fields_ = [("Cout", ctypes.c_int32), ("C1", ctypes.c_int32), ("C2", ctypes.c_int32), ("KH", ctypes.c_int32),
                ("KW", ctypes.c_int32), ("kind", ctypes.c_int32), ("split", ctypes.c_int32)]


class WnBwdItem(ctypes.Structure):
    _fields_ = ([(n, ctypes.c_void_p) for n in ("slabs", "dshift", "v", "g", "bias", "gamma", "invnorm", "dv", "dg", "dbias",
                                                "dgamma", "dbeta", "workspace")] +
                [("d", WnDesc), ("nsplit", ctypes.c_int32), ("accumulate", ctypes.c_int32)])


def _p(t: Optional[torch.Tensor]):
    return None if t is None else ctypes.c_void_p(t.data_ptr())


_raw_stream = getattr(torch._C, "_cuda_getCurrentRawStream", None)


def _stream():
    if _raw_stream is not None:
        return ctypes.c_void_p(_raw_stream(torch.cuda.current_device()))
    return ctypes.c_void_p(torch.cuda.current_stream().cuda_stream)


def _dev(*ts):
    for t in ts:
        if t is not None and not t.is_cuda:
            raise RuntimeError("vunet HIP path needs device tensors (hand-written gfx950 kernels; no CPU fallback)")
        if t is not None and t.dtype != torch.float32:
            raise RuntimeError(f"vunet HIP path computes in fp32, got {t.dtype}")


def _call(name: str, *args):
    rc = getattr(_lib.lib(), name)(*args)
    if rc != 0:
        raise RuntimeError(f"{name} failed with code {rc}")


def _c(t: Optional[torch.Tensor]) -> Optional[torch.Tensor]:
    return None if t is None else (t if t.is_contiguous() else t.contiguous())


def _r2(x: int) -> int:
    return (x + 1) // 2 * 2


def _r32(x: int) -> int:
    return (x + 31) // 32 * 32


_drop_state = {"base": None, "ctr": 0, "step": None, "host_step": 0}


def set_dropout_seed(seed: int):
    _drop_state["base"] = int(seed) & 0xFFFFFFFF
    _drop_state["ctr"] = 0


def set_dropout_host_step(step: int):
    _drop_state["host_step"] = int(step) & 0xFFFFFFFF


def reset_dropout_counter():
    if _drop_state["base"] is None:
        set_dropout_seed(torch.initial_seed())
    _drop_state["ctr"] = 0


def set_dropout_step(counter: Optional[torch.Tensor]):
    if counter is not None and not (counter.is_cuda and counter.dtype == torch.int32 and counter.numel() == 1):
        raise RuntimeError("dropout step counter: one int32 element on the GPU")
    _drop_state["step"] = counter
    _call("vunet_set_dropout_step", _p(counter))


def dropout_step_counter() -> Optional[torch.Tensor]:
    return _drop_state["step"]


def next_dropout_seed() -> int:
    if _drop_state["base"] is None:
        set_dropout_seed(torch.initial_seed())
    _drop_state["ctr"] += 1
    x = (_drop_state["base"] * 0x9E3779B1 + _drop_state["ctr"] * 0x85EBCA77) & 0xFFFFFFFF
    x ^= x >> 15
    return ((x * 0x2C1B3C6D) + _drop_state["host_step"] * 0x9E3779B1) & 0xFFFFFFFF


@dataclass
class ConvCfg:
    kind: int = 0
    k: int = 3
    stride: int = 1
    pad: int = 0
    in_act: int = ACT_NONE
    in_slope: float = 0.0
    drop_p: float = 0.0
    drop_seed: int = 0
    out_act: int = ACT_NONE
    d2s: bool = False
    res_is_x1: bool = False
    owner: object = None
    bf16: bool = False
    passthrough: bool = False


def conv_out_size(h: int, k: int, stride: int, pad: int) -> int:
    return (h + 2 * pad - k) // stride + 1


_SCHEMES = {"f32": 0, "x6": 1, "h2": 2}
_conv_precision = {"mode": os.environ.get("VUNET_CONV_SCHEME", "h2")}


def set_conv_precision(mode: str):
    if mode not in _SCHEMES:
        raise ValueError(f"unknown conv precision {mode!r} (h2 | x6 | f32)")
    _conv_precision["mode"] = mode


def conv_precision() -> str:
    return _conv_precision["mode"]


def _scheme() -> int:
    return _SCHEMES[_conv_precision["mode"]]


_wants_split_cache = {}
_TUNING_KEYS = {"split_force_nt": 0, "tiled_force_nt": 1, "force_small": 2, "blk_force_nt": 3, "parity_launches": 4, "blk_ws": 5, "wgrad_rowsplit": 6, "s2_fwd_f32": 7, "p2_form": 8}


def set_tuning(key: str, value: int):
    _call("vunet_set_tuning", _TUNING_KEYS[key], int(value))
    _wants_split_cache.clear()


def apply_env_tuning():
    spec = os.environ.get("VUNET_TUNING", "")
    for kv in filter(None, (t.strip() for t in spec.split(","))):
        k, _, v = kv.partition("=")
        set_tuning(k.strip(), int(v))


def absmax_partials(x1, x2=None):
    out = torch.empty(1024, device=x1.device, dtype=torch.float32)
    _call("vunet_absmax_partials", _p(x1), x1.numel(), _p(x2), 0 if x2 is None else x2.numel(), _p(out), _stream())
    return out


_amax_arena = {}


def _new_amax_out(dev):
    idx = dev.index if dev.index is not None else torch.cuda.current_device()
    key = (idx, _raw_stream(idx) if _raw_stream is not None else 0)
    a = _amax_arena.get(key)
    if a is None or a[1] >= a[0].shape[0]:
        a = _amax_arena[key] = [torch.zeros(128, 1024, device=dev, dtype=torch.float32), 0]
    a[1] += 1
    return a[0][a[1] - 1]


def _zero_scalar(dev, shape=(1,)):
    idx = dev.index if dev.index is not None else torch.cuda.current_device()
    key = (idx, _raw_stream(idx) if _raw_stream is not None else 0)
    z = _zero_rows.get(key)
    if z is None or z[1] + 16 > z[0].numel():
        z = _zero_rows[key] = [_new_amax_out(dev), 0]
    z[1] += 16
    return z[0][z[1] - 16:z[1] - 15].view(shape)


_zero_rows = {}
_amax_retired = []


def _reset_amax_arena():
    _amax_retired[:] = [list(_amax_arena.values())]
    _amax_arena.clear()
    _zero_rows.clear()


def _tag_amax(t, buf):
    t._vunet_amax = (buf, t._version)


def _tagged_amax(t):
    rec = getattr(t, "_vunet_amax", None)
    return rec[0] if rec is not None and rec[1] == t._version else None


def carry_amax_tag(src, dst):
    tag = _tagged_amax(src)
    if tag is not None:
        _tag_amax(dst, tag)
    if _is_relu_out(src):
        _tag_relu_out(dst)


_relu_premask = os.environ.get("VUNET_RELU_PREMASK", "1") != "0"


def enable_relu_premask(on: bool = True):
    global _relu_premask
    _relu_premask = bool(on)


def _tag_relu_out(t):
    t._vunet_relu_out = t._version


def _is_relu_out(t) -> bool:
    return t is not None and getattr(t, "_vunet_relu_out", None) == t._version


def _tag_masked(g, by):
    g._vunet_masked = (by.data_ptr(), g._version)


def _is_masked_by(g, y) -> bool:
    rec = getattr(g, "_vunet_masked", None)
    return rec is not None and y is not None and rec[0] == y.data_ptr() and rec[1] == g._version


def _amax_for(x1, x2=None):
    t1 = _tagged_amax(x1)
    if x2 is None:
        return t1 if t1 is not None else absmax_partials(x1)
    t2 = _tagged_amax(x2)
    if t1 is None and t2 is None:
        return absmax_partials(x1, x2)
    return (t1 if t1 is not None else absmax_partials(x1), t2 if t2 is not None else absmax_partials(x2))


def _amax_pair(amax):
    return amax if isinstance(amax, tuple) else (amax, None)


def _publishes_amax(desc, has_aux: bool, has_res: bool, has_wx: bool) -> bool:
    key = ("p", desc.N, desc.C1, desc.C2, desc.Hs, desc.Ws, desc.M, desc.m_off, desc.Mpad, desc.Ho, desc.Wo, desc.KH,
           desc.stride, desc.pad, desc.mode, desc.in_act, desc.drop_p > 0, desc.out_act, desc.d2s, desc.aux_act,
           desc.aux_drop_p > 0, has_aux, has_res, has_wx)
    r = _wants_split_cache.get(key)
    if r is None:
        r = _wants_split_cache[key] = _lib.lib().vunet_conv2d_publishes_amax(ctypes.byref(desc), int(has_aux),
                                                                             int(has_res), 2 if has_wx else 0) == 1
    return r


def _wgrad_wants_split(wd) -> bool:
    key = ("w", wd.N, wd.C1, wd.C2, wd.Hs, wd.Ws, wd.Cout, wd.Ho, wd.Wo, wd.KH, wd.stride, wd.pad, wd.flags & 1)
    r = _wants_split_cache.get(key)
    if r is None:
        r = _wants_split_cache[key] = _lib.lib().vunet_conv2d_wgrad_wants_split(ctypes.byref(wd)) == 1
    return r


def _wants_split(desc, has_aux: bool, has_res: bool, has_mask: bool = False) -> bool:
    key = (desc.N, desc.C1, desc.C2, desc.Hs, desc.Ws, desc.M, desc.m_off, desc.Mpad, desc.Ho, desc.Wo, desc.KH, desc.stride,
           desc.pad, desc.mode, desc.in_act, desc.drop_p > 0, desc.out_act, desc.d2s, desc.aux_act, desc.aux_drop_p > 0,
           has_aux, has_res, has_mask, _scheme())
    r = _wants_split_cache.get(key)
    if r is None:
        r = _wants_split_cache[key] = _lib.lib().vunet_conv2d_wants_split(ctypes.byref(desc), int(has_aux), int(has_res),
                                                                          int(has_mask), _scheme()) == 1
    return r


def x6_mtiles(m: int) -> int:
    return (((m + 31) // 32 + 1) + 1) & ~1


def x6_image_units(cout: int, c1: int, c2: int, k: int, dgrad: bool, split: int = 1) -> int:
    if k != 3:
        return 0
    slab, hdr = (384, 1) if split == 2 else (576, 0)
    if dgrad:
        return (cout // 16) * 3 * x6_mtiles(c1 + c2) * slab + hdr if cout % 16 == 0 else 0
    return ((c1 + c2) // 16) * 3 * x6_mtiles(cout) * slab + hdr if (c1 % 16 == 0 and c2 % 16 == 0) else 0


def _alloc_x6(cout, c1, c2, k, dgrad, dev):
    if _scheme() == 0:
        return None
    n = x6_image_units(cout, c1, c2, k, dgrad, _scheme())
    return torch.zeros(n * 4, device=dev, dtype=torch.int32) if n else None


def pack_weights(v, g, bias, gamma, beta, c1: int, c2: int, kind: int, need_dgrad: bool):
    cout, ctot, kh, kw = v.shape
    assert ctot == c1 + c2
    t = kh * kw
    dev = v.device
    wt_f = torch.empty(t * (_r2(c1) + _r2(c2)), _r32(cout), device=dev, dtype=torch.float32)
    wt_d = torch.empty(t * _r2(cout), _r32(ctot), device=dev, dtype=torch.float32) if need_dgrad else None
    wx_f = _alloc_x6(cout, c1, c2, kh, False, dev) if kh == kw else None
    wx_d = _alloc_x6(cout, c1, c2, kh, True, dev) if (need_dgrad and kh == kw) else None
    small = torch.empty(4, cout, device=dev, dtype=torch.float32)
    d = WnDesc(cout, c1, c2, kh, kw, kind, _scheme())
    _call("vunet_weightnorm_fwd", ctypes.byref(d), _p(v), _p(g), _p(bias), _p(gamma), _p(beta), _p(wt_f), _p(wt_d),
          _p(wx_f), _p(wx_d), _p(small[0]), _p(small[1]), _p(small[2]), _p(small[3]), _stream())
    return wt_f, wt_d, small[0], small[1], small[2], wx_f, wx_d


_prof = {"on": False, "recs": []}
_NO_TIMER = contextlib.nullcontext()


def profile_start():
    _prof["on"], _prof["recs"] = True, []


def profile_stop(detail: bool = False, by_kernel: bool = False):
    _prof["on"] = False
    if _prof["recs"]:
        torch.cuda.synchronize()
    fam = {}
    for name, flop, e0, e1 in _prof["recs"]:
        if by_kernel:
            name = name[-1]
        elif not detail:
            name = name[0]
        f = fam.setdefault(name, {"ms": 0.0, "flop": 0.0, "n": 0})
        f["ms"] += e0.elapsed_time(e1)
        f["flop"] += flop
        f["n"] += 1
    _prof["recs"] = []
    return fam


class _Timed:
    def __init__(self, name, flop):
        self.name, self.flop = name, flop

    def __enter__(self):
        if _prof["on"]:
            self.e0 = torch.cuda.Event(enable_timing=True)
            self.e1 = torch.cuda.Event(enable_timing=True)
            self.e0.record()

    def __exit__(self, *a):
        if _prof["on"]:
            self.e1.record()
            _prof["recs"].append((self.name, self.flop, self.e0, self.e1))


def _conv_gather(desc: ConvDesc, x1, x2, wt, shift, res, aux, y, wx=None, amax=None, res2=None):
    t = desc.KH * desc.KW
    scheme = _scheme() if wx is not None else 0
    amax_out = None
    if scheme == 2:
        if _wants_split(desc, aux is not None, res is not None):
            if amax is None:
                amax = _amax_for(x1, x2)
        else:
            wx = amax = None
    else:
        amax = None
    if _scheme() == 2 and _publishes_amax(desc, aux is not None, res is not None, wx is not None):
        amax_out = _new_amax_out(y.device)
    if desc.mode == 0:
        name, flop = "conv_gather_fwd", 2.0 * desc.N * desc.Ho * desc.Wo * desc.M * (desc.C1 + desc.C2) * t
    else:
        name, flop = "conv_gather_dgrad", 2.0 * desc.N * desc.Hs * desc.Ws * desc.C1 * desc.M * t
    kname = ""
    if _prof["on"]:
        buf = ctypes.create_string_buffer(96)
        _call("vunet_conv2d_variant", ctypes.byref(desc), 0 if aux is None else 1, 0 if wx is None else scheme, 0, buf, 96)
        kname = buf.value.decode()
    with (_Timed((name, desc.N, desc.C1, desc.C2, desc.Hs, desc.Ws, desc.M, desc.KH, desc.stride, desc.in_act, kname),
                flop) if _prof["on"] else _NO_TIMER):
        a1, a2 = _amax_pair(amax)
        rc = _lib.lib().vunet_conv2d_a2(ctypes.byref(desc), _p(x1), _p(x2), _p(wt), _p(wx), _p(shift), _p(res), _p(res2),
                                        _p(aux), _p(y), _p(a1), _p(a2), _p(amax_out), _stream())
        if rc == -3 and res2 is not None:
            _call("vunet_conv2d_a2", ctypes.byref(desc), _p(x1), _p(x2), _p(wt), _p(wx), _p(shift), _p(res), None, _p(aux),
                  _p(y), _p(a1), _p(a2), None, _stream())
            y.add_(res2)
            amax_out = None
        elif rc != 0:
            raise RuntimeError(f"vunet_conv2d_a2 failed with code {rc}")
    if amax_out is not None:
        _tag_amax(y, amax_out)
    return amax


def _plain_pack(w, need_dgrad):
    cout, cin = w.shape[0], w.shape[1]
    return pack_weights(w.contiguous(), None, None, None, None, cin, 0, 1, need_dgrad)


def _plain_desc(n, cin, hs, ws, m, ho, wo, k, stride, pad, mode, mpad):
    return ConvDesc(N=n, C1=cin, C2=0, Hs=hs, Ws=ws, M=m, m_off=0, Mpad=mpad, Ho=ho, Wo=wo, KH=k, KW=k,
                    stride=stride, pad=pad, mode=mode, in_act=ACT_NONE, in_slope=0.0, drop_p=0.0, drop_seed=0,
                    out_act=ACT_NONE, d2s=0, aux_act=ACT_NONE, aux_slope=0.0, aux_drop_p=0.0, aux_drop_seed=0)


class ConvPlainFwd(torch.autograd.Function):

    @staticmethod
    def forward(ctx, x, w, stride, pad):
        _dev(x, w)
        x, w = _c(x), _c(w)
        n, cin, hs, ws = x.shape
        cout, _, k, _ = w.shape
        ho, wo = conv_out_size(hs, k, stride, pad), conv_out_size(ws, k, stride, pad)
        pk = _plain_pack(w, False)
        wt_f = pk[0]
        y = torch.empty(n, cout, ho, wo, device=x.device, dtype=torch.float32)
        _conv_gather(_plain_desc(n, cin, hs, ws, cout, ho, wo, k, stride, pad, 0, wt_f.shape[1]), x, None, wt_f, None,
                     None, None, y, pk[5])
        ctx.save_for_backward(x, w)
        ctx.geo = (stride, pad)
        return y

    @staticmethod
    def backward(ctx, gy):
        x, w = ctx.saved_tensors
        stride, pad = ctx.geo
        gx = ConvPlainDgrad.apply(gy, w, x.shape[2], x.shape[3], stride, pad) if ctx.needs_input_grad[0] else None
        gw = ConvPlainWgrad.apply(x, gy, w.shape[2], stride, pad) if ctx.needs_input_grad[1] else None
        return gx, gw, None, None


class ConvPlainDgrad(torch.autograd.Function):

    @staticmethod
    def forward(ctx, dy, w, hs, ws, stride, pad):
        _dev(dy, w)
        dy, w = _c(dy), _c(w)
        n, cout, ho, wo = dy.shape
        cin, k = w.shape[1], w.shape[2]
        pk = _plain_pack(w, True)
        wt_d = pk[1]
        dx = torch.empty(n, cin, hs, ws, device=dy.device, dtype=torch.float32)
        _conv_gather(_plain_desc(n, cout, ho, wo, cin, hs, ws, k, stride, pad, 1, wt_d.shape[1]), dy, None, wt_d, None,
                     None, None, dx, pk[6])
        ctx.save_for_backward(dy, w)
        ctx.geo = (stride, pad)
        return dx

    @staticmethod
    def backward(ctx, gdx):
        dy, w = ctx.saved_tensors
        stride, pad = ctx.geo
        gdy = ConvPlainFwd.apply(gdx, w, stride, pad) if ctx.needs_input_grad[0] else None
        gw = ConvPlainWgrad.apply(gdx, dy, w.shape[2], stride, pad) if ctx.needs_input_grad[1] else None
        return gdy, gw, None, None, None, None


class ConvPlainWgrad(torch.autograd.Function):

    @staticmethod
    def forward(ctx, x, dy, k, stride, pad):
        _dev(x, dy)
        x, dy = _c(x), _c(dy)
        n, cin, hs, ws = x.shape
        cout, ho, wo = dy.shape[1], dy.shape[2], dy.shape[3]
        wd = WgradDesc(N=n, C1=cin, C2=0, Hs=hs, Ws=ws, Cout=cout, Ho=ho, Wo=wo, KH=k, KW=k, stride=stride, pad=pad,
                       in_act=ACT_NONE, in_slope=0.0, drop_p=0.0, drop_seed=0, nsplit=1,
                       flags=0 if _scheme() else 1)
        ns = _lib.lib().vunet_conv2d_wgrad_nsplit(ctypes.byref(wd))
        wd.nsplit = ns
        ktot = k * k * cin
        slabs = torch.empty(ns * _r32(cout) * (ktot + 1), device=x.device, dtype=torch.float32)
        dshift = slabs[ns * _r32(cout) * ktot:]
        _call("vunet_conv2d_wgrad", ctypes.byref(wd), _p(x), None, _p(dy), _p(slabs), _p(dshift), None, None, _stream())
        dw = torch.empty(cout, cin, k, k, device=x.device, dtype=torch.float32)
        work = torch.empty(cout * (ktot + 1), device=x.device, dtype=torch.float32)
        wn = WnDesc(cout, cin, 0, k, k, 1, 0)
        _call("vunet_weightnorm_bwd", ctypes.byref(wn), _p(slabs), _p(dshift), ns, _p(dw), None, None, None, None,
              _p(dw), None, None, None, None, _p(work), 0, _stream())
        ctx.save_for_backward(x, dy)
        ctx.geo = (k, stride, pad)
        return dw

    @staticmethod
    def backward(ctx, gw):
        x, dy = ctx.saved_tensors
        k, stride, pad = ctx.geo
        gx = ConvPlainDgrad.apply(dy, gw, x.shape[2], x.shape[3], stride, pad) if ctx.needs_input_grad[0] else None
        gdy = ConvPlainFwd.apply(x, gw, stride, pad) if ctx.needs_input_grad[1] else None
        return gx, gdy, None, None, None


def _differentiable_layer(x1, x2, res, v, g, bias, gamma, beta, cfg):
    x = x1 if x2 is None else torch.cat([x1, x2], dim=1)
    if cfg.in_act == ACT_ELU:
        x = torch.nn.functional.elu(x)
    elif cfg.in_act == ACT_RELU:
        x = torch.relu(x)
    elif cfg.in_act == ACT_LRELU:
        x = torch.nn.functional.leaky_relu(x, cfg.in_slope)
    if cfg.drop_p > 0:
        m1 = dropout_keep_mask(x1.shape, cfg.drop_p, cfg.drop_seed, x1.device)
        mask = m1 if x2 is None else torch.cat(
            [m1, dropout_keep_mask(x2.shape, cfg.drop_p, (cfg.drop_seed + SEED2_OFFSET) & 0xFFFFFFFF, x2.device)], dim=1)
        x = x * mask / (1.0 - cfg.drop_p)
    cout = v.shape[0]
    if cfg.kind == 1:
        w, scale_out = v, None
    else:
        nrm = v.flatten(1).norm(dim=1)
        if cfg.kind == 2:
            nrm = nrm.clamp_min(1e-12)
        w = v * ((g.reshape(-1) if cfg.kind == 0 else 1.0) / nrm).view(-1, 1, 1, 1)
        scale_out = gamma.reshape(1, cout, 1, 1) if gamma is not None else None
    y = ConvPlainFwd.apply(x, w, cfg.stride, cfg.pad)
    if bias is not None:
        y = y + bias.view(1, cout, 1, 1)
    if scale_out is not None:
        y = scale_out * y
    if cfg.kind != 1 and beta is not None:
        y = y + beta.reshape(1, cout, 1, 1)
    if cfg.out_act == ACT_RELU:
        y = torch.relu(y)
    elif cfg.out_act == ACT_SIGMOID:
        y = torch.sigmoid(y)
    elif cfg.out_act == ACT_ELU:
        y = torch.nn.functional.elu(y)
    elif cfg.out_act == ACT_LRELU:
        y = torch.nn.functional.leaky_relu(y, cfg.in_slope)
    if cfg.d2s:
        y = DepthToSpace.apply(y)
    if res is not None:
        y = y + res
    return y


_grad_hooks = []
_direct_grads_enabled = True
_wgrad_streams = {"on": False, "by_stream": {}, "dirty": set()}


def enable_wgrad_streams(on: bool = True):
    _wgrad_streams["on"] = bool(on)


_stream_objs = {}


def _current_stream_obj():
    if _raw_stream is None:
        return torch.cuda.current_stream()
    idx = torch.cuda.current_device()
    key = (idx, _raw_stream(idx))
    st = _stream_objs.get(key)
    if st is None:
        st = _stream_objs[key] = torch.cuda.current_stream()
    return st


def _wgrad_stream_for(cur):
    ws = _wgrad_streams["by_stream"].get(cur.cuda_stream)
    if ws is None:
        ws = _wgrad_streams["by_stream"][cur.cuda_stream] = torch.cuda.Stream()
    _wgrad_streams["dirty"].add(cur.cuda_stream)
    return ws


def join_wgrad_streams():
    flush_weight_grads()
    cur = torch.cuda.current_stream()
    for key in _wgrad_streams["dirty"]:
        ws = _wgrad_streams["by_stream"][key]
        if ws.cuda_stream != cur.cuda_stream:
            cur.wait_stream(ws)
    _wgrad_streams["dirty"].clear()


_inference_bf16 = False


class inference_precision:

    def __init__(self, dtype: str = "bf16"):
        if dtype not in ("bf16", "f32", "fp32"):
            raise ValueError(f"unknown inference precision {dtype!r}")
        self.on = dtype == "bf16"

    def __enter__(self):
        global _inference_bf16
        self.prev, _inference_bf16 = _inference_bf16, self.on

    def __exit__(self, *exc):
        global _inference_bf16
        _inference_bf16 = self.prev
        return False


class direct_grads:

    def __init__(self, enabled: bool):
        self.enabled = bool(enabled)

    def __enter__(self):
        global _direct_grads_enabled
        self.prev, _direct_grads_enabled = _direct_grads_enabled, self.enabled

    def __exit__(self, *exc):
        global _direct_grads_enabled
        _direct_grads_enabled = self.prev
        return False


def _has_direct_grad(p) -> bool:
    return (_direct_grads_enabled and getattr(p, "_vunet_direct_grad", False) and p.grad is not None
            and p.grad.is_contiguous())


def add_grad_hook(fn):
    _grad_hooks.append(fn)


def remove_grad_hook(fn):
    if fn in _grad_hooks:
        _grad_hooks.remove(fn)


class WnItem(ctypes.Structure):
    _fields_ = [(n, ctypes.c_void_p) for n in ("v", "g", "bias", "gamma", "beta", "wt_f", "wt_d", "scale", "shift",
                                                "invnorm", "wx_f", "wx_d", "wmax")] + [("d", WnDesc)]


_prepack_sets = {}
_active_prepack = {}


def _ptr_or_none(t):
    return None if t is None else t.data_ptr()


def _build_prepack_set(model):
    convs = model.__dict__.get("_vunet_conv_modules")
    if convs is None:
        convs = [m for m in model.modules() if hasattr(m, "_params")]
        object.__setattr__(model, "_vunet_conv_modules", convs)
    mods = [m for m in convs if m.__dict__.get("_last_split") is not None]
    sig = (_scheme(),) + tuple((id(m), m.__dict__["_last_split"]) for m in mods)
    cur = _prepack_sets.get(id(model))
    if cur is not None and cur["signature"] == sig:
        return cur
    if not mods:
        return None
    dev = next(model.parameters()).device
    items, entries, keep, max_cout = (WnItem * len(mods))(), {}, [], 1
    for i, m in enumerate(mods):
        v, g, b, gamma, beta = m._params()
        c1, c2, need_x = m._last_split
        cout, ctot, kh, kw = v.shape
        t = kh * kw
        wt_f = torch.zeros(t * (_r2(c1) + _r2(c2)), _r32(cout), device=dev, dtype=torch.float32)
        wt_d = torch.zeros(t * _r2(cout), _r32(ctot), device=dev, dtype=torch.float32) if need_x else None
        wx_f = _alloc_x6(cout, c1, c2, kh, False, dev) if kh == kw else None
        wx_d = _alloc_x6(cout, c1, c2, kh, True, dev) if (need_x and kh == kw) else None
        small = torch.empty(4, cout, device=dev, dtype=torch.float32)
        it = items[i]
        it.v, it.g, it.bias, it.gamma, it.beta = (_ptr_or_none(x) for x in (v, g, b, gamma, beta))
        it.wt_f, it.wt_d = wt_f.data_ptr(), _ptr_or_none(wt_d)
        it.wx_f, it.wx_d = _ptr_or_none(wx_f), _ptr_or_none(wx_d)
        it.scale, it.shift, it.invnorm = small[0].data_ptr(), small[1].data_ptr(), small[2].data_ptr()
        it.wmax = small[3].data_ptr()
        it.d = WnDesc(cout, c1, c2, kh, kw, m.kind, _scheme())
        entries[id(m)] = ((c1, c2, need_x), wt_f, wt_d, small[0], small[1], small[2], wx_f, wx_d)
        keep.append((wt_f, wt_d, small, wx_f, wx_d))
        max_cout = max(max_cout, cout)
    raw = bytes(items)
    table = torch.frombuffer(bytearray(raw), dtype=torch.uint8).to(dev)
    cur = {"signature": sig, "table": table, "n": len(mods), "max_cout": max_cout, "entries": entries, "keep": keep}
    _prepack_sets[id(model)] = cur
    return cur


def invalidate_active_prepack(module):
    _active_prepack.pop(id(module), None)


class prepacked:

    _depth = 0

    def __init__(self, *models):
        self.models = [m for m in models if m is not None]
        self._keys = []

    def __enter__(self):
        if prepacked._depth == 0:
            _reset_amax_arena()
        prepacked._depth += 1
        try:
            for model in self.models:
                cur = _build_prepack_set(model)
                if cur is not None:
                    _call("vunet_weightnorm_fwd_multi", _p(cur["table"]), cur["n"], cur["max_cout"], _stream())
                    _active_prepack.update(cur["entries"])
                    self._keys.extend(cur["entries"].keys())
        except BaseException:
            self.__exit__(None, None, None)
            raise
        return self

    def __exit__(self, *a):
        prepacked._depth -= 1
        if prepacked._depth == 0:
            _active_prepack.clear()
        else:
            for k in self._keys:
                _active_prepack.pop(k, None)
        self._keys = []


_WN_GROUP = int(os.environ.get("VUNET_WN_GROUP", "64"))
_WN_ARENA_FLOATS = 48 << 20
_wn_batch = {"on": os.environ.get("VUNET_WN_BATCH", "1") != "0", "pending": {}, "arena": {}, "tables": {},
             "callback_queued": False, "capture": os.environ.get("VUNET_WN_BATCH_CAPTURE", "1") != "0",
             "wgrad": os.environ.get("VUNET_WGRAD_BATCH", "1") != "0"}
_wgrad_batchable_cache = {}


def _wgrad_batchable(wd) -> bool:
    key = (wd.N, wd.C1, wd.C2, wd.Hs, wd.Ws, wd.Cout, wd.Ho, wd.Wo, wd.KH, wd.KW, wd.stride, wd.pad, wd.in_act, wd.drop_p > 0,
           wd.nsplit, wd.flags)
    r = _wgrad_batchable_cache.get(key)
    if r is None:
        r = _wgrad_batchable_cache[key] = _lib.lib().vunet_conv2d_wgrad_batchable(ctypes.byref(wd)) == 1
    return r


def enable_wn_batching(on: bool = True):
    flush_weight_grads()
    _wn_batch["on"] = bool(on)


def _wn_buffers(n_slab: int, n_work: int, dev):
    idx = torch.cuda.current_device()
    key = (idx, _raw_stream(idx))
    need = ((n_slab + 63) & ~63) + ((n_work + 63) & ~63)
    ar = _wn_batch["arena"].get(key)
    if ar is None or ar[0].numel() < need:
        flush_weight_grads()
        ar = _wn_batch["arena"][key] = [torch.empty(max(_WN_ARENA_FLOATS, need), device=dev, dtype=torch.float32), 0]
    if ar[1] + need > ar[0].numel():
        _wn_flush_stream(key)
    off = ar[1]
    ar[1] = off + need
    return ar[0][off:off + n_slab], ar[0][off + ((n_slab + 63) & ~63):off + ((n_slab + 63) & ~63) + n_work]


def _wn_flush_stream(stream_key):
    items = _wn_batch["pending"].pop(stream_key, None)
    ar = _wn_batch["arena"].get(stream_key)
    if ar is not None:
        ar[1] = 0
    if not items:
        return
    dev_idx, raw = stream_key
    sig = tuple(it[0] for it in items)
    tab = _wn_batch["tables"].get(sig)
    if tab is None:
        if torch.cuda.is_current_stream_capturing():
            raise RuntimeError("batched weight-norm backward: this group's item table has not been built yet and cannot be "
                               "uploaded while a hipGraph is being captured -- run an eager step of the same geometry on "
                               "the capture stream first (ShapePoseNet does)")
        arr = (WnBwdItem * len(items))()
        max_cout = max_blocks = 1
        for i, item in enumerate(items):
            fields = item[0]
            (slabs, dshift, v, g, bias, gamma, invnorm, dv, dg, dbias, dgamma, dbeta, work, dsc, ns) = fields
            it = arr[i]
            it.slabs, it.dshift, it.v, it.g, it.bias, it.gamma, it.invnorm = slabs, dshift, v, g, bias, gamma, invnorm
            it.dv, it.dg, it.dbias, it.dgamma, it.dbeta, it.workspace = dv, dg, dbias, dgamma, dbeta, work
            cout, c1, c2, kh, kw, kind = dsc
            it.d = WnDesc(cout, c1, c2, kh, kw, kind, 0)
            it.nsplit, it.accumulate = ns, 1
            max_cout = max(max_cout, cout)
            max_blocks = max(max_blocks, cout * ((kh * kw * (c1 + c2) + 63) // 64))
        table = torch.frombuffer(bytearray(bytes(arr)), dtype=torch.uint8).to(torch.device("cuda", dev_idx))
        tab = _wn_batch["tables"][sig] = (table, len(items), max_cout, max_blocks)
    table, n, max_cout, max_blocks = tab
    wg = [it[3] for it in items if len(it) > 3 and it[3] is not None]
    if wg:
        arr = (WgradItem * len(wg))()
        for i, (wd_bytes, ptrs) in enumerate(wg):
            ctypes.memmove(ctypes.addressof(arr[i].d), wd_bytes, ctypes.sizeof(WgradDesc))
            (arr[i].x1, arr[i].x2, arr[i].dy, arr[i].slabs, arr[i].dshift, arr[i].amax_x, arr[i].amax_x2,
             arr[i].amax_dy) = ptrs
        _call("vunet_conv2d_wgrad_multi", arr, len(wg), ctypes.c_void_p(raw))
    _call("vunet_weightnorm_bwd_multi", _p(table), n, max_cout, max_blocks, ctypes.c_void_p(raw))
    for it in items:
        for p_ in it[1]:
            for hook in _grad_hooks:
                hook(p_)


def flush_weight_grads():
    for key in list(_wn_batch["pending"].keys()):
        _wn_flush_stream(key)
    _wn_batch["callback_queued"] = False


def _wn_defer(fields, params, keep, wgrad=None):
    idx = torch.cuda.current_device()
    key = (idx, _raw_stream(idx))
    lst = _wn_batch["pending"].setdefault(key, [])
    lst.append((fields, params, keep, wgrad))
    if len(lst) >= _WN_GROUP:
        _wn_flush_stream(key)
    elif not _wn_batch["callback_queued"]:
        _wn_batch["callback_queued"] = True
        torch.autograd.Variable._execution_engine.queue_callback(flush_weight_grads)


class FusedConv(torch.autograd.Function):

    @staticmethod
    def forward(ctx, x1, x2, res, v, g, bias, gamma, beta, cfg: ConvCfg):
        _dev(x1, x2, res, v, g, bias, gamma, beta)
        x1, x2, res = _c(x1), _c(x2), _c(res)
        v, g, bias, gamma, beta = _c(v), _c(g), _c(bias), _c(gamma), _c(beta)
        n, c1, hs, ws = x1.shape
        c2 = 0 if x2 is None else x2.shape[1]
        cout = v.shape[0]
        k = cfg.k
        ho, wo = conv_out_size(hs, k, cfg.stride, cfg.pad), conv_out_size(ws, k, cfg.stride, cfg.pad)
        need_x = (ctx.needs_input_grad[0] or (x2 is not None and ctx.needs_input_grad[1]))
        need_w = any(ctx.needs_input_grad[3:8])
        frozen = not any(t is not None and t.requires_grad for t in (v, g, bias, gamma, beta))
        sub = stamp = hit = pre = None
        if frozen:
            sub = (c1, c2, cfg.kind, bool(need_x), _scheme())
            stamp = tuple(None if t is None else (t.data_ptr(), t._version) for t in (v, g, bias, gamma, beta))
            hit = getattr(v, "_vunet_frozen_pack", {}).get(sub)
        if cfg.owner is not None and not frozen:
            old = cfg.owner.__dict__.get("_last_split")
            new = (c1, c2, bool(need_x) or (old is not None and old[2]))
            if new != old:
                object.__setattr__(cfg.owner, "_last_split", new)
            pre = _active_prepack.get(id(cfg.owner))
            if pre is not None and (pre[0][:2] != (c1, c2) or (need_x and pre[2] is None)):
                pre = None
        if pre is not None:
            _, wt_f, wt_d, scale, shift, invnorm, wx_f, wx_d = pre
        elif hit is not None and hit[0] == stamp:
            wt_f, wt_d, scale, shift, invnorm, wx_f, wx_d = hit[1]
        else:
            wt_f, wt_d, scale, shift, invnorm, wx_f, wx_d = pack_weights(v, g, bias, gamma, beta, c1, c2, cfg.kind,
                                                                          need_x)
            if frozen:
                if not hasattr(v, "_vunet_frozen_pack"):
                    v._vunet_frozen_pack = {}
                v._vunet_frozen_pack[sub] = (stamp, (wt_f, wt_d, scale, shift, invnorm, wx_f, wx_d))
        if cfg.d2s:
            y = torch.empty(n, cout // 4, 2 * ho, 2 * wo, device=x1.device, dtype=torch.float32)
        else:
            y = torch.empty(n, cout, ho, wo, device=x1.device, dtype=torch.float32)
        d = ConvDesc(N=n, C1=c1, C2=c2, Hs=hs, Ws=ws, M=cout, m_off=0, Mpad=wt_f.shape[1], Ho=ho, Wo=wo, KH=k, KW=k,
                     stride=cfg.stride, pad=cfg.pad, mode=0, in_act=cfg.in_act, in_slope=cfg.in_slope,
                     drop_p=cfg.drop_p, drop_seed=cfg.drop_seed, out_act=cfg.out_act, d2s=int(cfg.d2s))
        ctx.amax_x = None
        if cfg.bf16 and _lib.lib().vunet_conv2d_bf16_supported(ctypes.byref(d)) == 1:
            wb = torch.empty((c1 + c2) * 9 * wt_f.shape[1], device=x1.device, dtype=torch.bfloat16)
            _call("vunet_pack_bf16", _p(wt_f), _p(wb), c1, c2, wt_f.shape[1], _stream())
            with (_Timed(("conv_bf16_fwd", n, c1, c2, hs, ws, cout, k, cfg.stride, cfg.in_act, "conv_bf16_kernel"),
                        2.0 * n * ho * wo * cout * (c1 + c2) * k * k) if _prof["on"] else _NO_TIMER):
                _call("vunet_conv2d_bf16", ctypes.byref(d), _p(x1), _p(x2), _p(wb), _p(shift), _p(res), _p(y), _stream())
        else:
            ctx.amax_x = _conv_gather(d, x1, x2, wt_f, shift, res, None, y, wx_f)
        ctx.cfg = cfg
        ctx.prepacked = pre is not None
        ctx.param_refs = (v, g, bias, gamma, beta)
        ctx.res_ref = res
        ctx.dims = (n, c1, c2, hs, ws, cout, ho, wo)
        ctx.need_w = need_w
        ctx.save_for_backward(x1, x2, v, g, bias, gamma, invnorm, wt_d,
                              y if cfg.out_act in (ACT_SIGMOID, ACT_RELU, ACT_LRELU, ACT_ELU) else None, wx_d)
        if cfg.out_act == ACT_RELU:
            _tag_relu_out(y)
        ctx.x1_relu_out = _relu_premask and _is_relu_out(x1)
        if cfg.passthrough:
            ctx.set_materialize_grads(False)
            return y, x1
        return y

    @staticmethod
    def backward(ctx, dy, g_alias=None):
        x1, x2, v, g, bias, gamma, invnorm, wt_d, y, wx_d = ctx.saved_tensors
        cfg: ConvCfg = ctx.cfg
        if dy is None:
            return g_alias, None, None, None, None, None, None, None, None
        if g_alias is not None:
            g_alias = _c(g_alias)
        if torch.is_grad_enabled():
            res, beta = ctx.res_ref, ctx.param_refs[4]
            with torch.enable_grad():
                y2 = _differentiable_layer(x1, x2, res, v, g, bias, gamma, beta, cfg)
            needs = list(ctx.needs_input_grad[:8])
            if cfg.res_is_x1:
                needs[2] = False
            tensors = (x1, x2, res, v, g, bias, gamma, beta)
            wanted = [t for t, need in zip(tensors, needs) if need and t is not None]
            grads = iter(torch.autograd.grad(y2, wanted, dy, create_graph=True, allow_unused=True))
            out = [next(grads) if (need and t is not None) else None for t, need in zip(tensors, needs)]
            if g_alias is not None:
                out[0] = g_alias if out[0] is None else out[0] + g_alias
            return (*out, None)
        n, c1, c2, hs, ws, cout, ho, wo = ctx.dims
        dy = _c(dy)
        dres = dy if (ctx.needs_input_grad[2] and not cfg.res_is_x1) else None
        k = cfg.k
        premasked = cfg.out_act == ACT_RELU and _is_masked_by(dy, y)
        if (cfg.out_act == ACT_RELU and not premasked and not ctx.need_w and not cfg.d2s and x2 is None
                and ctx.needs_input_grad[0] and cfg.in_act == ACT_NONE and cfg.drop_p == 0 and wt_d is not None):
            dx = torch.empty_like(x1)
            d = ConvDesc(N=n, C1=cout, C2=0, Hs=ho, Ws=wo, M=c1, m_off=0, Mpad=wt_d.shape[1], Ho=hs, Wo=ws, KH=k, KW=k,
                         stride=cfg.stride, pad=cfg.pad, mode=1, in_act=ACT_NONE, in_slope=0.0, drop_p=0.0, drop_seed=0,
                         out_act=ACT_NONE, d2s=0)
            kname = ""
            if _prof["on"]:
                buf = ctypes.create_string_buffer(96)
                _call("vunet_conv2d_variant", ctypes.byref(d), 0, 0 if wx_d is None else _scheme(), 1, buf, 96)
                kname = buf.value.decode()
                if kname.startswith("conv_tiled"):
                    kname = kname.replace(", 1, 0, ", ", 1, 4, ")
            with (_Timed(("conv_gather_dgrad", n, cout, 0, ho, wo, c1, k, cfg.stride, 0, kname),
                        2.0 * n * ho * wo * cout * c1 * k * k) if _prof["on"] else _NO_TIMER):
                rc = -3
                if wx_d is not None and _wants_split(d, False, cfg.res_is_x1, True):
                    amax = _amax_for(dy) if _scheme() == 2 else None
                    amax_out = _new_amax_out(dx.device) if _scheme() == 2 else None
                    rc = _lib.lib().vunet_conv2d_dgrad_relu_x6(ctypes.byref(d), _p(dy), _p(y), _p(wx_d),
                                                               _p(dy if cfg.res_is_x1 else g_alias), _p(dx), _p(amax),
                                                               _p(amax_out), _stream())
                    if rc == 0 and amax_out is not None:
                        _tag_amax(dx, amax_out)
                if rc == -3:
                    rc = _lib.lib().vunet_conv2d_dgrad_relu(ctypes.byref(d), _p(dy), _p(y), _p(wt_d),
                                                            _p(dy if cfg.res_is_x1 else g_alias), _p(dx), _stream())
            if rc == 0:
                if cfg.res_is_x1 and g_alias is not None:
                    dx.add_(g_alias)
                return dx, None, dres, None, None, None, None, None, None
            if rc != -3:
                raise RuntimeError(f"vunet_conv2d_dgrad_relu failed with code {rc}")
            if _prof["on"] and _prof["recs"]:
                _prof["recs"].pop()
        dconv = dy
        if cfg.out_act != ACT_NONE and not premasked:
            dconv = torch.empty_like(dy)
            _call("vunet_act_bwd_from_out", _p(y), _p(dy), _p(dconv), cfg.out_act, cfg.in_slope, dy.numel(), _stream())
        if cfg.d2s:
            t = torch.empty(n, cout, ho, wo, device=dy.device, dtype=torch.float32)
            _call("vunet_space_to_depth", _p(dconv), _p(t), n, cout // 4, 2 * ho, 2 * wo, _stream())
            carry_amax_tag(dconv, t)
            dconv = t
        dv = dg = dbias = dgamma = dbeta = None
        dy_amax = []

        def get_dy_amax():
            if not dy_amax:
                dy_amax.append(_amax_for(dconv))
            return dy_amax[0]

        wd = WgradDesc(N=n, C1=c1, C2=c2, Hs=hs, Ws=ws, Cout=cout, Ho=ho, Wo=wo, KH=k, KW=k, stride=cfg.stride,
                       pad=cfg.pad, in_act=cfg.in_act, in_slope=cfg.in_slope, drop_p=cfg.drop_p,
                       drop_seed=cfg.drop_seed, nsplit=1, flags=(0, 0, 2)[_scheme()] if _scheme() else 1)
        wg_amax = (None, None)
        if ctx.need_w and _scheme() == 2 and _wgrad_wants_split(wd):
            wg_amax = (ctx.amax_x if ctx.amax_x is not None else _amax_for(x1, x2), get_dy_amax())

        def weight_gradients(defer: bool = False):
            ns = _lib.lib().vunet_conv2d_wgrad_nsplit(ctypes.byref(wd))
            if ns < 1:
                raise RuntimeError(f"vunet_conv2d_wgrad_nsplit failed with code {ns}")
            wd.nsplit = ns
            ktot = k * k * (c1 + c2)
            n_slab = ns * _r32(cout) * ktot + ns * _r32(cout)
            if defer:
                slabs, work = _wn_buffers(n_slab, cout * (ktot + 1), dy.device)
            else:
                slabs = torch.empty(n_slab, device=dy.device, dtype=torch.float32)
            dshift = slabs[ns * _r32(cout) * ktot:]
            kname = ""
            if _prof["on"]:
                buf = ctypes.create_string_buffer(96)
                _call("vunet_conv2d_wgrad_variant", ctypes.byref(wd), buf, 96)
                kname = buf.value.decode()
            ax1, ax2 = _amax_pair(wg_amax[0])
            late = (defer and _wn_batch["wgrad"] and not _prof["on"]
                    and _wgrad_batchable(wd))
            if not late:
                with (_Timed(("conv_wgrad", n, c1, c2, hs, ws, cout, k, cfg.stride, cfg.in_act, kname),
                            2.0 * n * ho * wo * cout * (c1 + c2) * k * k) if _prof["on"] else _NO_TIMER):
                    _call("vunet_conv2d_wgrad_a2", ctypes.byref(wd), _p(x1), _p(x2), _p(dconv), _p(slabs), _p(dshift),
                          _p(ax1), _p(ax2), _p(wg_amax[1]), _stream())
            ni = ctx.needs_input_grad
            if defer:
                outs = [p_.grad if (p_ is not None and need) else None for p_, need in zip(ctx.param_refs, ni[3:8])]
                ptrs = tuple(None if t is None else t.data_ptr() for t in
                             (slabs, dshift, v, g, bias, gamma, invnorm, outs[0], outs[1], outs[2], outs[3], outs[4], work))
                wg_item, keep = None, (invnorm,)
                if late:
                    wg_item = (bytes(wd), tuple(None if t is None else t.data_ptr() for t in
                                                (x1, x2, dconv, slabs, dshift, ax1, ax2, wg_amax[1])))
                    keep = (invnorm, x1, x2, dconv, ax1, ax2, wg_amax[1])
                _wn_defer(ptrs + ((cout, c1, c2, k, k, cfg.kind), ns),
                          [p_ for p_, o in zip(ctx.param_refs, outs) if o is not None], keep, wg_item)
                return None, None, None, None, None
            params = (v, g, bias, gamma, gamma)
            outs, direct = [], []
            for idx, (p_, need) in enumerate(zip(ctx.param_refs, ni[3:8])):
                if p_ is None or not need:
                    outs.append(None)
                    direct.append(False)
                elif _has_direct_grad(p_):
                    outs.append(p_.grad)
                    direct.append(True)
                else:
                    outs.append(torch.empty_like(params[idx]))
                    direct.append(False)
            n_direct = sum(direct)
            n_needed = sum(o is not None for o in outs)
            wn = WnDesc(cout, c1, c2, k, k, cfg.kind, 0)
            work = torch.empty(cout * (ktot + 1), device=dy.device, dtype=torch.float32)

            def run(sel_direct: bool):
                sel = [o if (o is not None and d_ == sel_direct) else None for o, d_ in zip(outs, direct)]
                _call("vunet_weightnorm_bwd", ctypes.byref(wn), _p(slabs), _p(dshift), ns, _p(v), _p(g), _p(bias),
                      _p(gamma), _p(invnorm), _p(sel[0]), _p(sel[1]), _p(sel[2]), _p(sel[3]), _p(sel[4]), _p(work),
                      1 if sel_direct else 0, _stream())
            if n_direct:
                run(True)
            if n_needed > n_direct:
                run(False)
            dv, dg, dbias, dgamma, dbeta = [None if d_ else o for o, d_ in zip(outs, direct)]
            for p_, d_ in zip(ctx.param_refs, direct):
                if d_:
                    for hook in _grad_hooks:
                        hook(p_)
            return dv, dg, dbias, dgamma, dbeta

        if ctx.need_w:
            ni_ = ctx.needs_input_grad
            all_direct = all((not ni_[3 + i]) or p_ is None or _has_direct_grad(p_) for i, p_ in enumerate(ctx.param_refs))
            defer_ok = (_wn_batch["on"] and ctx.prepacked and all_direct and dy.is_cuda
                        and (_wn_batch["capture"] or not torch.cuda.is_current_stream_capturing()))
            if _wgrad_streams["on"] and all_direct and dy.is_cuda:
                cur = _current_stream_obj()
                wstream = _wgrad_stream_for(cur)
                wstream.wait_stream(cur)
                for t_ in (x1, x2, dconv, *_amax_pair(wg_amax[0]), wg_amax[1], None if ctx.prepacked else invnorm):
                    if t_ is not None:
                        t_.record_stream(wstream)
                torch.cuda.set_stream(wstream)
                try:
                    weight_gradients(defer_ok)
                finally:
                    torch.cuda.set_stream(cur)
            else:
                dv, dg, dbias, dgamma, dbeta = weight_gradients(defer_ok)
        dx1 = dx2 = None
        if ctx.needs_input_grad[0] or (x2 is not None and ctx.needs_input_grad[1]):
            def dgrad(x, cs, m_off, seed, add, mask_by_x=False, add2=None):
                dx = torch.empty_like(x)
                has_aux = cfg.in_act != ACT_NONE or cfg.drop_p > 0
                mask_by_x = mask_by_x and not has_aux
                d = ConvDesc(N=n, C1=cout, C2=0, Hs=ho, Ws=wo, M=cs, m_off=m_off, Mpad=wt_d.shape[1], Ho=hs, Wo=ws,
                             KH=k, KW=k, stride=cfg.stride, pad=cfg.pad, mode=1, in_act=ACT_NONE, in_slope=0.0,
                             drop_p=0.0, drop_seed=0, out_act=ACT_NONE, d2s=0,
                             aux_act=ACT_RELU if mask_by_x else cfg.in_act,
                             aux_slope=cfg.in_slope, aux_drop_p=cfg.drop_p, aux_drop_seed=seed)
                has_aux = has_aux or mask_by_x
                amax = None
                if wx_d is not None and _scheme() == 2 and _wants_split(d, has_aux, add is not None):
                    amax = get_dy_amax()
                _conv_gather(d, dconv, None, wt_d, None, add, x if has_aux else None, dx, wx_d, amax, res2=add2)
                if mask_by_x:
                    _tag_masked(dx, x)
                return dx
            if ctx.needs_input_grad[0]:
                dx1 = dgrad(x1, c1, 0, cfg.drop_seed, dy if cfg.res_is_x1 else g_alias, ctx.x1_relu_out,
                            add2=g_alias if cfg.res_is_x1 else None)
                g_alias = None
            if x2 is not None and ctx.needs_input_grad[1]:
                dx2 = dgrad(x2, c2, c1, (cfg.drop_seed + SEED2_OFFSET) & 0xFFFFFFFF, None)
        if g_alias is not None:
            dx1 = g_alias
        return dx1, dx2, dres, dv, dg, dbias, dgamma, dbeta, None


def fused_conv(x1, x2, res, v, g, bias, gamma, beta, cfg: ConvCfg):
    assert res is None or cfg.out_act == ACT_NONE, "fused_conv: residual together with an output activation"
    if res is not None and res is x1 and not cfg.d2s and cfg.out_act == ACT_NONE:
        cfg.res_is_x1 = True
    cfg.bf16 = _inference_bf16 and not torch.is_grad_enabled()
    if cfg.passthrough and not (torch.is_grad_enabled() and x1.requires_grad and x1.is_contiguous() and _grad_passthrough):
        cfg.passthrough = False
        return FusedConv.apply(x1, x2, res, v, g, bias, gamma, beta, cfg), x1
    if cfg.passthrough:
        y, alias = FusedConv.apply(x1, x2, res, v, g, bias, gamma, beta, cfg)
        carry_amax_tag(x1, alias)
        return y, alias
    return FusedConv.apply(x1, x2, res, v, g, bias, gamma, beta, cfg)


_grad_passthrough = os.environ.get("VUNET_GRAD_PASSTHROUGH", "1") != "0"


def enable_grad_passthrough(on: bool = True):
    global _grad_passthrough
    _grad_passthrough = bool(on)


class DepthToSpace(torch.autograd.Function):
    @staticmethod
    def forward(ctx, x):
        _dev(x)
        x = _c(x)
        n, c, h, w = x.shape
        y = torch.empty(n, c // 4, 2 * h, 2 * w, device=x.device, dtype=x.dtype)
        _call("vunet_depth_to_space", _p(x), _p(y), n, c, h, w, _stream())
        return y

    @staticmethod
    def backward(ctx, dy):
        dy = _c(dy)
        n, c, h, w = dy.shape
        dx = torch.empty(n, 4 * c, h // 2, w // 2, device=dy.device, dtype=dy.dtype)
        _call("vunet_space_to_depth", _p(dy), _p(dx), n, c, h, w, _stream())
        return dx


class SpaceToDepth(torch.autograd.Function):
    @staticmethod
    def forward(ctx, x):
        _dev(x)
        x = _c(x)
        n, c, h, w = x.shape
        y = torch.empty(n, 4 * c, h // 2, w // 2, device=x.device, dtype=x.dtype)
        _call("vunet_space_to_depth", _p(x), _p(y), n, c, h, w, _stream())
        return y

    @staticmethod
    def backward(ctx, dy):
        dy = _c(dy)
        n, c, h, w = dy.shape
        dx = torch.empty(n, c // 4, 2 * h, 2 * w, device=dy.device, dtype=dy.dtype)
        _call("vunet_depth_to_space", _p(dy), _p(dx), n, c, h, w, _stream())
        return dx


class CropWindow(torch.autograd.Function):

    @staticmethod
    def forward(ctx, x, off, size):
        _dev(x)
        x = _c(x)
        n, c, h, w = x.shape
        y = torch.empty(n, c, size, size, device=x.device, dtype=x.dtype)
        _call("vunet_crop_window", _p(x), _p(y), n * c, h, w, size, _p(off), _stream())
        ctx.off, ctx.geo = off, (n, c, h, w, size)
        return y

    @staticmethod
    def backward(ctx, dy):
        n, c, h, w, size = ctx.geo
        dx = torch.zeros(n, c, h, w, device=dy.device, dtype=dy.dtype)
        _call("vunet_crop_window_bwd", _p(_c(dy)), _p(dx), n * c, h, w, size, _p(ctx.off), _stream())
        return dx, None, None


class UpsampleBilinear2x(torch.autograd.Function):

    @staticmethod
    def forward(ctx, x):
        _dev(x)
        x = _c(x)
        n, c, h, w = x.shape
        y = torch.empty(n, c, 2 * h, 2 * w, device=x.device, dtype=x.dtype)
        _call("vunet_upsample_bilinear2x_fwd", _p(x), _p(y), n * c, h, w, _stream())
        return y

    @staticmethod
    def backward(ctx, dy):
        dy = _c(dy)
        n, c, h2, w2 = dy.shape
        dx = torch.empty(n, c, h2 // 2, w2 // 2, device=dy.device, dtype=dy.dtype)
        _call("vunet_upsample_bilinear2x_bwd", _p(dy), _p(dx), n * c, h2 // 2, w2 // 2, _stream())
        return dx


class Reparam(torch.autograd.Function):

    @staticmethod
    def forward(ctx, mu, logstd, eps):
        _dev(mu, logstd, eps)
        mu, logstd, eps = _c(mu), _c(logstd), _c(eps)
        z = torch.empty_like(mu)
        if eps is None:
            eps = torch.empty_like(mu)
            _call("vunet_unit_sample", _p(mu), _p(logstd), _p(z), _p(eps), mu.numel(), next_dropout_seed(), _stream())
        else:
            _call("vunet_reparam_fwd", _p(mu), _p(logstd), _p(eps), _p(z), mu.numel(), _stream())
        ctx.save_for_backward(logstd, eps)
        return z

    @staticmethod
    def backward(ctx, dz):
        logstd, eps = ctx.saved_tensors
        dz = _c(dz)
        dmu, dls = torch.empty_like(dz), torch.empty_like(dz)
        _call("vunet_reparam_bwd", _p(dz), _p(logstd), _p(eps), _p(dmu), _p(dls), dz.numel(), _stream())
        return dmu, dls, None


_kernel_noise = {"on": False}


def kernel_noise_enabled() -> bool:
    return _kernel_noise["on"]


class kernel_noise:
    def __init__(self, on: bool = True):
        self.on = bool(on)

    def __enter__(self):
        self.prev, _kernel_noise["on"] = _kernel_noise["on"], self.on
        return self

    def __exit__(self, *exc):
        _kernel_noise["on"] = self.prev
        return False


class FanOut(torch.autograd.Function):

    @staticmethod
    def forward(ctx, x, n: int):
        ctx.set_materialize_grads(False)
        return tuple(x.view_as(x) for _ in range(n))

    @staticmethod
    def backward(ctx, *gs):
        gs = [_c(g) for g in reversed(gs) if g is not None]
        if not gs:
            return None, None
        if len(gs) == 1:
            return gs[0], None
        _dev(*gs)
        out = torch.empty_like(gs[0])
        amax_out = _new_amax_out(out.device) if _scheme() == 2 else None
        ptrs = (ctypes.c_void_p * len(gs))(*[g.data_ptr() for g in gs])
        _call("vunet_sum_amax", ptrs, len(gs), _p(out), _p(amax_out), out.numel(), _stream())
        if amax_out is not None:
            _tag_amax(out, amax_out)
        return out, None


_FAN_OUT = os.environ.get("VUNET_FAN_OUT", "1") != "0"


def fan_out(x, n: int):
    if n < 2 or not (_grad_passthrough and _FAN_OUT and x.is_cuda and torch.is_grad_enabled() and x.requires_grad):
        return (x,) * n
    outs = FanOut.apply(x, n)
    for o in outs:
        carry_amax_tag(x, o)
    return outs


class UnitSample(torch.autograd.Function):

    @staticmethod
    def forward(ctx, mu):
        _dev(mu)
        mu = _c(mu)
        z = torch.empty_like(mu)
        _call("vunet_unit_sample", _p(mu), None, _p(z), None, mu.numel(), next_dropout_seed(), _stream())
        return z

    @staticmethod
    def backward(ctx, dz):
        return dz


def set_schedule_(lr_dev, lr: float, imax_dev, imax: float, step_dev, step: int):
    _call("vunet_set_schedule", _p(lr_dev), float(lr), _p(imax_dev), float(imax), _p(step_dev), int(step), _stream())


class TotalLoss(torch.autograd.Function):

    @staticmethod
    def forward(ctx, kl, gamma, ll_weight: float, use_kl: bool, *terms):
        _dev(kl, *terms)
        n = len(terms)
        g_t = gamma if torch.is_tensor(gamma) else None
        g_c = 0.0 if g_t is not None else float(gamma)
        loss = torch.empty((), device=kl.device, dtype=torch.float32)
        ll = torch.empty((), device=kl.device, dtype=torch.float32)
        ptrs = (ctypes.c_void_p * n)(*[t.data_ptr() for t in terms])
        _call("vunet_total_loss", ptrs, n, _p(kl), _p(g_t), g_c, float(ll_weight), int(bool(use_kl)), _p(loss), _p(ll), _stream())
        ctx.cfg = (n, g_t, g_c, float(ll_weight), int(bool(use_kl)), [t.shape for t in terms], kl.shape)
        return loss, ll

    @staticmethod
    def backward(ctx, g_loss, g_ll):
        n, g_t, g_c, llw, use_kl, shapes, kl_shape = ctx.cfg
        ref = g_loss if g_loss is not None else g_ll
        d = torch.empty(n + 1, device=ref.device, dtype=torch.float32)
        _call("vunet_total_loss_bwd", _p(None if g_loss is None else _c(g_loss)), _p(None if g_ll is None else _c(g_ll)), n,
              _p(g_t), g_c, llw, use_kl, _p(d), _stream())
        return (d[n:n + 1].view(kl_shape) if use_kl else None, None, None, None,
                *[d[i:i + 1].view(sh) for i, sh in enumerate(shapes)])


def gamma_update_(gamma, imax, avg_kl, gamma_step: float):
    _dev(gamma, imax, avg_kl)
    _call("vunet_gamma_update", _p(gamma), _p(imax), _p(avg_kl), float(gamma_step), _stream())
    return gamma


class L1Mean(torch.autograd.Function):

    @staticmethod
    def forward(ctx, target, pred, weight: float):
        _dev(target, pred)
        target, pred = _c(target), _c(pred)
        out = _zero_scalar(pred.device)
        partial = torch.empty(1024, device=pred.device, dtype=torch.float32)
        _call("vunet_l1_mean_fwd", _p(target), _p(pred), _p(partial), _p(out), float(weight), pred.numel(), _stream())
        ctx.save_for_backward(target, pred)
        ctx.weight = float(weight)
        ctx.pred_relu_out = _relu_premask and _is_relu_out(pred)
        return out

    @staticmethod
    def backward(ctx, gout):
        target, pred = ctx.saved_tensors
        return None, _l1_backward(target, pred, None, ctx.weight, gout, ctx.pred_relu_out), None


def _l1_backward(target, pred, add, weight, gout, relu_mask=False):
    db = torch.empty_like(pred)
    amax_out = _new_amax_out(db.device) if (_scheme() == 2 and db.is_cuda) else None
    _call("vunet_l1_mean_bwd_amax", _p(target), _p(pred), _p(add), _p(db), weight / pred.numel(), _p(_c(gout)),
          pred.numel(), _p(amax_out), int(relu_mask), _stream())
    if amax_out is not None:
        _tag_amax(db, amax_out)
    if relu_mask:
        _tag_masked(db, pred)
    return db


class L1MeanThrough(torch.autograd.Function):

    @staticmethod
    def forward(ctx, target, pred, weight: float):
        _dev(target, pred)
        assert pred.is_contiguous()
        target = _c(target)
        out = _zero_scalar(pred.device)
        partial = torch.empty(1024, device=pred.device, dtype=torch.float32)
        _call("vunet_l1_mean_fwd", _p(target), _p(pred), _p(partial), _p(out), float(weight), pred.numel(), _stream())
        ctx.save_for_backward(target, pred)
        ctx.weight = float(weight)
        ctx.pred_relu_out = _relu_premask and _is_relu_out(pred)
        ctx.set_materialize_grads(False)
        return out, pred

    @staticmethod
    def backward(ctx, gout, g_alias):
        target, pred = ctx.saved_tensors
        if gout is None:
            return None, g_alias, None
        return None, _l1_backward(target, pred, None if g_alias is None else _c(g_alias), ctx.weight, gout,
                                  ctx.pred_relu_out), None


l1_pool_fusion = {"on": os.environ.get("VUNET_L1_POOL_FUSE", "1") != "0"}


class L1ThroughPool(torch.autograd.Function):

    @staticmethod
    def forward(ctx, target, pred, weight: float):
        _dev(target, pred)
        target, pred = _c(target), _c(pred)
        n, c, h, w = pred.shape
        out = _zero_scalar(pred.device)
        partial = torch.empty(1024, device=pred.device, dtype=torch.float32)
        y = torch.empty(n, c, h // 2, w // 2, device=pred.device, dtype=pred.dtype)
        _call("vunet_l1_pool_fwd", _p(target), _p(pred), _p(partial), _p(out), _p(y), float(weight), n * c, h, w, _stream())
        tag = _tagged_amax(pred)
        if tag is not None:
            _tag_amax(y, tag)
        ctx.save_for_backward(target, pred)
        ctx.weight = float(weight)
        ctx.pred_relu_out = _relu_premask and _is_relu_out(pred)
        ctx.set_materialize_grads(False)
        return out, y

    @staticmethod
    def backward(ctx, gout, gy):
        target, pred = ctx.saved_tensors
        n, c, h, w = pred.shape
        db = torch.empty_like(pred)
        amax_out = _new_amax_out(db.device) if _scheme() == 2 else None
        scale = ctx.weight / pred.numel() if gout is not None else 0.0
        _call("vunet_l1_pool_bwd", _p(target), _p(pred), _p(None if gy is None else _c(gy)), _p(db), scale,
              _p(None if gout is None else _c(gout)), n * c, h, w, _p(amax_out), int(ctx.pred_relu_out), _stream())
        if amax_out is not None:
            _tag_amax(db, amax_out)
        if ctx.pred_relu_out:
            _tag_masked(db, pred)
        return None, db, None


class KLPrior(torch.autograd.Function):

    @staticmethod
    def forward(ctx, mu, logstd, weight: float):
        _dev(mu, logstd)
        mu, logstd = _c(mu), _c(logstd)
        n = mu.shape[0]
        d = mu.numel() // n
        out = _zero_scalar(mu.device, ())
        partial = torch.empty(256, device=mu.device, dtype=torch.float32)
        _call("vunet_kl_fwd", _p(mu), _p(logstd), _p(partial), _p(out), float(weight), n, d, _stream())
        ctx.save_for_backward(mu, logstd)
        ctx.scale = float(weight) / n
        return out

    @staticmethod
    def backward(ctx, gout):
        mu, logstd = ctx.saved_tensors
        dmu, dls = torch.empty_like(mu), torch.empty_like(mu)
        _call("vunet_kl_bwd", _p(mu), _p(logstd), _p(dmu), _p(dls), ctx.scale, _p(_c(gout)), mu.numel(), _stream())
        return dmu, dls, None


class SqDiff(torch.autograd.Function):

    @staticmethod
    def forward(ctx, p, q, weight: float):
        _dev(p, q)
        p, q = _c(p), _c(q)
        n = p.shape[0]
        out = _zero_scalar(p.device, ())
        partial = torch.empty(256, device=p.device, dtype=torch.float32)
        _call("vunet_sqdiff_fwd", _p(p), _p(q), _p(partial), _p(out), float(weight), n, p.numel() // n, _stream())
        ctx.save_for_backward(p, q)
        ctx.scale = float(weight) / n
        return out

    @staticmethod
    def backward(ctx, gout):
        p, q = ctx.saved_tensors
        dp, dq = torch.empty_like(p), torch.empty_like(p)
        _call("vunet_sqdiff_bwd", _p(p), _p(q), _p(dp), _p(dq), ctx.scale, _p(_c(gout)), p.numel(), _stream())
        return dp, dq, None


class VggPreprocess(torch.autograd.Function):
    @staticmethod
    def forward(ctx, x):
        _dev(x)
        x = _c(x)
        n, c, h, w = x.shape
        assert c == 3
        y = torch.empty_like(x)
        _call("vunet_vgg_preprocess", _p(x), _p(y), n, h, w, _stream())
        return y

    @staticmethod
    def backward(ctx, dy):
        dy = _c(dy)
        n, _, h, w = dy.shape
        dx = torch.empty_like(dy)
        _call("vunet_vgg_preprocess_bwd", _p(dy), None, _p(dx), n, h, w, _stream())
        return dx


class MaxPool2(torch.autograd.Function):
    @staticmethod
    def forward(ctx, x):
        _dev(x)
        x = _c(x)
        n, c, h, w = x.shape
        y = torch.empty(n, c, h // 2, w // 2, device=x.device, dtype=x.dtype)
        _call("vunet_maxpool2_fwd", _p(x), _p(y), n * c, h, w, _stream())
        ctx.save_for_backward(x, y)
        ctx.x_relu_out = _relu_premask and _is_relu_out(x)
        tag = _tagged_amax(x)
        if tag is not None:
            _tag_amax(y, tag)
        return y

    @staticmethod
    def backward(ctx, dy):
        x, y = ctx.saved_tensors
        dy = _c(dy)
        n, c, h, w = x.shape
        dx = torch.empty_like(x)
        _call("vunet_maxpool2_bwd_relu" if ctx.x_relu_out else "vunet_maxpool2_bwd", _p(x), _p(y), _p(dy), _p(dx), n * c, h,
              w, _stream())
        tag = _tagged_amax(dy)
        if tag is not None:
            _tag_amax(dx, tag)
        if ctx.x_relu_out:
            _tag_masked(dx, x)
        return dx


class InstanceNorm(torch.autograd.Function):
    @staticmethod
    def forward(ctx, x, eps: float):
        _dev(x)
        x = _c(x)
        n, c, h, w = x.shape
        y = torch.empty_like(x)
        stats = torch.empty(n * c, 2, device=x.device, dtype=torch.float32)
        _call("vunet_instnorm_fwd", _p(x), _p(y), _p(stats), n * c, h * w, float(eps), _stream())
        ctx.save_for_backward(y, stats)
        return y

    @staticmethod
    def backward(ctx, dy):
        y, stats = ctx.saved_tensors
        dy = _c(dy)
        n, c, h, w = y.shape
        dx = torch.empty_like(y)
        _call("vunet_instnorm_bwd", _p(y), _p(dy), _p(stats), _p(dx), n * c, h * w, _stream())
        return dx, None


class Activation(torch.autograd.Function):
    @staticmethod
    def forward(ctx, x, act: int, slope: float):
        _dev(x)
        x = _c(x)
        y = torch.empty_like(x)
        _call("vunet_act_fwd", _p(x), _p(y), act, float(slope), x.numel(), _stream())
        ctx.save_for_backward(y)
        ctx.act, ctx.slope = act, float(slope)
        return y

    @staticmethod
    def backward(ctx, dy):
        (y,) = ctx.saved_tensors
        dy = _c(dy)
        dx = torch.empty_like(dy)
        _call("vunet_act_bwd_from_out", _p(y), _p(dy), _p(dx), ctx.act, ctx.slope, dy.numel(), _stream())
        return dx, None, None


def dropout_keep_mask(shape, p: float, seed: int, device) -> torch.Tensor:
    m = torch.empty(shape, device=device, dtype=torch.float32)
    _call("vunet_dropout_mask", _p(m), m.numel(), float(p), int(seed) & 0xFFFFFFFF, _stream())
    return m


def adam_step_flat(param, grad, exp_avg, exp_avg_sq, lr, beta1, beta2, eps, weight_decay, step, grad_scale=1.0):
    _dev(param, grad, exp_avg, exp_avg_sq)
    _call("vunet_adam_step", _p(param), _p(grad), _p(exp_avg), _p(exp_avg_sq), param.numel(), float(lr), float(beta1),
          float(beta2), float(eps), float(weight_decay), int(step), float(grad_scale), _stream())


def adam_step_flat_dev(param, grad, exp_avg, exp_avg_sq, lr_dev, beta1, beta2, eps, weight_decay, step_dev,
                       grad_scale=1.0):
    _dev(param, grad, exp_avg, exp_avg_sq)
    if not (lr_dev.is_cuda and lr_dev.dtype == torch.float64 and step_dev.is_cuda and step_dev.dtype == torch.int64):
        raise RuntimeError("adam_step_flat_dev: lr as a float64 and step as an int64 device tensor")
    _call("vunet_adam_step_dev", _p(param), _p(grad), _p(exp_avg), _p(exp_avg_sq), param.numel(), _p(lr_dev),
          float(beta1), float(beta2), float(eps), float(weight_decay), _p(step_dev), float(grad_scale), _stream())


P2_META_INTS = 128


class P2Desc(ctypes.Structure):
    _fields_ = [(n, ctypes.c_int32) for n in ("N", "C", "H", "W", "M", "relu")]


class Planes:

    __slots__ = ("buf", "meta", "shape")

    def __init__(self, shape, device, meta=None):
        n, c, h, w = shape
        assert c % 8 == 0
        self.shape = (int(n), int(c), int(h), int(w))
        self.buf = torch.zeros(2, n, c // 8, h + 2, w + 2, 8, device=device, dtype=torch.float16)
        self.meta = meta if meta is not None else torch.zeros(P2_META_INTS, device=device, dtype=torch.int32)

    def to_nchw(self):
        n, c, h, w = self.shape
        y = torch.empty(n, c, h, w, device=self.buf.device, dtype=torch.float32)
        _call("vunet_p2_to_nchw", _p(self.buf), _p(self.meta), _p(y), n, c, h, w, _stream())
        return y


def p2_from_nchw(x, out: Planes = None, relu: bool = False, amax=None, zero_meta: bool = True) -> Planes:
    _dev(x)
    x = _c(x)
    if out is None:
        out = Planes(tuple(x.shape), x.device)
    if amax is None:
        amax = _tagged_amax(x)
    if amax is None:
        amax = absmax_partials(x)
    n, c, h, w = x.shape
    if zero_meta:
        out.meta.zero_()
    _call("vunet_p2_from_nchw", _p(x), _p(amax), min(int(amax.numel()), 512), int(relu), _p(out.buf), _p(out.meta), n, c, h, w,
          _stream())
    return out


class P2Weights:

    def __init__(self, weight, bias):
        self.weight, self.bias = weight, bias
        self.cout, self.cin = int(weight.shape[0]), int(weight.shape[1])
        self._img = {}

    def image(self, dgrad: bool):
        rec = self._img.get(dgrad)
        stamp = (self.weight.data_ptr(), self.weight._version, None if self.bias is None else self.bias._version)
        if rec is None or rec[0] != stamp:
            nbytes = _lib.lib().vunet_p2_weight_image_bytes(self.cout, self.cin, int(dgrad))
            if nbytes <= 0:
                raise RuntimeError("p2 weight image: geometry not covered")
            dev = self.weight.device
            img = torch.empty(nbytes // 2, device=dev, dtype=torch.float16)
            wk = torch.empty(4, device=dev, dtype=torch.float32)
            work = torch.empty(2 * max(self.cout, self.cin), device=dev, dtype=torch.float32)
            _call("vunet_p2_pack_weights", _p(_c(self.weight.detach())), _p(None if self.bias is None else _c(self.bias.detach())),
                  self.cout, self.cin, int(dgrad), _p(img), _p(wk), _p(work), _stream())
            rec = self._img[dgrad] = (stamp, img, wk)
        return rec[1], rec[2]


def p2_conv_supported(n, c, h, w, m) -> bool:
    d = P2Desc(n, c, h, w, m, 0)
    return _lib.lib().vunet_p2_conv_supported(ctypes.byref(d)) == 1


def p2_conv(x: Planes, wts: P2Weights, out: Planes, relu: bool = True, dgrad: bool = False, mask: Planes = None):
    n, c, h, w = x.shape
    m = wts.cin if dgrad else wts.cout
    assert c == (wts.cout if dgrad else wts.cin) and out.shape == (n, m, h, w)
    img, wk = wts.image(dgrad)
    d = P2Desc(n, c, h, w, m, int(relu and not dgrad))
    timer = _NO_TIMER
    if _prof["on"]:
        buf = ctypes.create_string_buffer(96)
        _call("vunet_p2_conv_variant", ctypes.byref(d), buf, 96)
        timer = _Timed(("conv_gather_dgrad" if dgrad else "conv_gather_fwd", n, c, 0, h, w, m, 3, 1, 0, buf.value.decode()),
                       2.0 * n * h * w * c * m * 9)
    with timer:
        _call("vunet_p2_conv", ctypes.byref(d), _p(x.buf), _p(x.meta), _p(img), _p(wk),
              _p(None if dgrad or wts.bias is None else wts.bias), _p(None if mask is None else mask.buf), _p(out.buf), _p(out.meta),
              _stream())
    return out


def p2_l1_fwd(t: Planes, p: Planes, weight: float):
    n, c, h, w = p.shape
    assert t.shape == p.shape
    out = _zero_scalar(p.buf.device)
    partial = torch.empty(1024, device=p.buf.device, dtype=torch.float32)
    _call("vunet_p2_l1_fwd", _p(t.buf), _p(t.meta), _p(p.buf), _p(p.meta), _p(partial), _p(out), float(weight), n, c, h, w, _stream())
    return out


def p2_pool_fwd(p: Planes, out: Planes, t: Planes = None, weight: float = 0.0):
    n, c, h, w = p.shape
    assert out.shape == (n, c, h // 2, w // 2)
    loss = partial = None
    if t is not None:
        loss = _zero_scalar(p.buf.device)
        partial = torch.empty(1024, device=p.buf.device, dtype=torch.float32)
    _call("vunet_p2_pool_fwd", _p(None if t is None else t.buf), _p(None if t is None else t.meta), _p(p.buf), _p(p.meta), _p(partial),
          _p(loss), float(weight), _p(out.buf), _p(out.meta), n, c, h, w, _stream())
    return loss


def p2_l1_bwd(t: Planes, p: Planes, add, g: Planes, gscale: float, gout):
    n, c, h, w = p.shape
    _call("vunet_p2_l1_bwd", _p(t.buf), _p(t.meta), _p(p.buf), _p(p.meta), _p(None if add is None else add.buf),
          _p(None if add is None else add.meta), _p(g.buf), _p(g.meta), float(gscale), _p(gout), n, c, h, w, _stream())
    return g


def p2_pool_bwd(p: Planes, dy: Planes, g: Planes, t: Planes = None, gscale: float = 0.0, gout=None):
    n, c, h, w = p.shape
    _call("vunet_p2_pool_bwd", _p(None if t is None else t.buf), _p(None if t is None else t.meta), _p(p.buf), _p(p.meta), _p(dy.buf),
          _p(dy.meta), _p(g.buf), _p(g.meta), float(gscale), _p(gout), n, c, h, w, _stream())
    return g
```

include/vunet_hip.h:

```cpp
#ifndef VUNET_HIP_H
#define VUNET_HIP_H
#include <stddef.h>
#include <stdint.h>

#ifdef __cplusplus
extern "C" {
#endif

#define VUNET_OK 0
#define VUNET_ERR_ARG (-1)
#define VUNET_ERR_LAUNCH (-2)
#define VUNET_ERR_UNSUPPORTED (-3)

#define VUNET_ACT_NONE 0
#define VUNET_ACT_ELU 1
#define VUNET_ACT_RELU 2
#define VUNET_ACT_SIGMOID 3
#define VUNET_ACT_LRELU 4

int vunet_abi_version(void);

typedef struct vunet_conv_desc {
  int32_t N;
  int32_t C1, C2;
  int32_t Hs, Ws;
  int32_t M;
  int32_t m_off;
  int32_t Mpad;
  int32_t Ho, Wo;
  int32_t KH, KW, stride, pad;
  int32_t mode;
  int32_t in_act;
  float in_slope;
  float drop_p;
  uint32_t drop_seed;
  int32_t out_act;
  int32_t d2s;
  int32_t aux_act;
  float aux_slope;
  float aux_drop_p;
  uint32_t aux_drop_seed;
} vunet_conv_desc;

int vunet_conv2d_gather(const vunet_conv_desc* d, const float* x1, const float* x2, const float* wt,
                        const float* shift, const float* res, const float* aux, float* y, void* stream);

int vunet_conv2d_dgrad_relu(const vunet_conv_desc* d, const float* dy, const float* y, const float* wt,
                            const float* res, float* dx, void* stream);

int vunet_conv2d_gather_variant(const vunet_conv_desc* d, int32_t has_aux, char* name, int32_t len);

int vunet_conv2d(const vunet_conv_desc* d, const float* x1, const float* x2, const float* wt, const void* wx,
                 const float* shift, const float* res, const float* aux, float* y, const float* amax, float* amax_out,
                 void* stream);
int vunet_conv2d_a2(const vunet_conv_desc* d, const float* x1, const float* x2, const float* wt, const void* wx,
                    const float* shift, const float* res, const float* res2, const float* aux, float* y, const float* amax,
                    const float* amax2, float* amax_out, void* stream);
int vunet_conv2d_x6(const vunet_conv_desc* d, const float* x1, const float* x2, const void* wx, const float* shift,
                    const float* res, const float* aux, const float* mask, float* y, const float* amax, float* amax_out,
                    void* stream);
int vunet_conv2d_x6_supported(const vunet_conv_desc* d, int32_t has_mask);
int vunet_conv2d_wants_split(const vunet_conv_desc* d, int32_t has_aux, int32_t has_res, int32_t has_mask, int32_t split);
int vunet_conv2d_dgrad_relu_x6(const vunet_conv_desc* d, const float* dy, const float* y, const void* wx,
                               const float* res, float* dx, const float* amax, float* amax_out, void* stream);
int vunet_conv2d_publishes_amax(const vunet_conv_desc* d, int32_t has_aux, int32_t has_res, int32_t split);
int vunet_absmax_partials(const float* x1, int64_t n1, const float* x2, int64_t n2, float* out, void* stream);
int vunet_conv2d_variant(const vunet_conv_desc* d, int32_t has_aux, int32_t has_wx, int32_t has_mask, char* name,
                         int32_t len);

int vunet_conv2d_bf16_supported(const vunet_conv_desc* d);
int vunet_pack_bf16(const float* wt_f, void* wb, int32_t C1, int32_t C2, int32_t Mpad, void* stream);
int vunet_conv2d_bf16(const vunet_conv_desc* d, const float* x1, const float* x2, const void* wb,
                      const float* shift, const float* res, float* y, void* stream);

int vunet_conv2d_blk(const vunet_conv_desc* d, const void* x1, const void* x2, const void* wb, const float* shift,
                     const void* res, void* y, int32_t y_fp32_nchw, void* stream);
int vunet_conv2d_blk_rnb_supported(const vunet_conv_desc* d);
int vunet_conv2d_blk_rnb(const vunet_conv_desc* d, const void* x, const void* skip, const void* wb_nin, const float* shift_nin,
                         int32_t Mpad_nin, const void* wb, const float* shift, const void* res, void* y, void* stream);
int vunet_conv2d_blk_tiled(const vunet_conv_desc* d);
int vunet_pack_bf16_taps(const float* wt_f, void* wb, int32_t C1, int32_t C2, int32_t Mpad, int32_t taps, void* stream);
int vunet_nchw_to_blk(const float* x, void* y, int32_t N, int32_t C, int32_t H, int32_t W, void* stream);
int vunet_blk_to_nchw(const void* x, float* y, int32_t N, int32_t C, int32_t H, int32_t W, void* stream);
int vunet_conv1x1_few_to_blk(const float* x, const float* wt_f, const float* shift, void* y, int32_t N, int32_t C,
                             int32_t H, int32_t W, int32_t M, int32_t Mpad, void* stream);

typedef struct vunet_wgrad_desc {
  int32_t N, C1, C2, Hs, Ws;
  int32_t Cout, Ho, Wo;
  int32_t KH, KW, stride, pad;
  int32_t in_act;
  float in_slope;
  float drop_p;
  uint32_t drop_seed;
  int32_t nsplit;
  int32_t flags;
} vunet_wgrad_desc;

int vunet_conv2d_wgrad(const vunet_wgrad_desc* d, const float* x1, const float* x2, const float* dy,
                       float* slabs, float* dshift, const float* amax_x, const float* amax_dy, void* stream);
int vunet_conv2d_wgrad_a2(const vunet_wgrad_desc* d, const float* x1, const float* x2, const float* dy,
                          float* slabs, float* dshift, const float* amax_x, const float* amax_x2, const float* amax_dy,
                          void* stream);
typedef struct vunet_wgrad_item {
  vunet_wgrad_desc d;
  const float* x1;
  const float* x2;
  const float* dy;
  float* slabs;
  float* dshift;
  const float* amax_x;
  const float* amax_x2;
  const float* amax_dy;
} vunet_wgrad_item;
int vunet_conv2d_wgrad_multi(const vunet_wgrad_item* items, int32_t n, void* stream);
int vunet_conv2d_wgrad_batchable(const vunet_wgrad_desc* d);
int vunet_conv2d_wgrad_wants_split(const vunet_wgrad_desc* d);
int vunet_conv2d_wgrad_variant(const vunet_wgrad_desc* d, char* name, int32_t len);
int vunet_conv2d_wgrad_nsplit(const vunet_wgrad_desc* d);

typedef struct vunet_wn_desc {
  int32_t Cout, C1, C2, KH, KW;
  int32_t kind;
  int32_t split;
} vunet_wn_desc;

int vunet_weightnorm_fwd(const vunet_wn_desc* d, const float* v, const float* g, const float* bias,
                         const float* gamma, const float* beta, float* wt_f, float* wt_d, void* wx_f, void* wx_d,
                         float* scale, float* shift, float* invnorm, float* wmax, void* stream);

typedef struct vunet_wn_item {
  const float *v, *g, *bias, *gamma, *beta;
  float *wt_f, *wt_d, *scale, *shift, *invnorm;
  void *wx_f, *wx_d;
  float* wmax;
  vunet_wn_desc d;
} vunet_wn_item;
int vunet_weightnorm_fwd_multi(const vunet_wn_item* items_dev, int32_t n_items, int32_t max_cout, void* stream);
int vunet_x6_image_bytes(const vunet_wn_desc* d, int32_t dgrad);
int vunet_x6_mtiles(int32_t M);

int vunet_weightnorm_bwd(const vunet_wn_desc* d, const float* slabs, const float* dshift, int32_t nsplit,
                         const float* v, const float* g, const float* bias, const float* gamma,
                         const float* invnorm, float* dv, float* dg, float* dbias, float* dgamma,
                         float* dbeta, float* workspace, int32_t accumulate, void* stream);

typedef struct vunet_wn_bwd_item {
  const float *slabs, *dshift, *v, *g, *bias, *gamma, *invnorm;
  float *dv, *dg, *dbias, *dgamma, *dbeta;
  float* workspace;
  vunet_wn_desc d;
  int32_t nsplit, accumulate;
} vunet_wn_bwd_item;
int vunet_weightnorm_bwd_multi(const vunet_wn_bwd_item* items_dev, int32_t n_items, int32_t max_cout,
                               int32_t max_reduce_blocks, void* stream);

int vunet_depth_to_space(const float* x, float* y, int32_t N, int32_t C, int32_t H, int32_t W, void* stream);
int vunet_space_to_depth(const float* x, float* y, int32_t N, int32_t C, int32_t H, int32_t W, void* stream);

int vunet_upsample_bilinear2x_fwd(const float* x, float* y, int64_t NC, int32_t H, int32_t W, void* stream);
int vunet_upsample_bilinear2x_bwd(const float* dy, float* dx, int64_t NC, int32_t H, int32_t W, void* stream);

int vunet_axpby(const float* x, const float* y_in, float* y, float a, float b, int64_t n, void* stream);
int vunet_act_bwd_from_out(const float* y, const float* dy, float* dx, int32_t act, float slope, int64_t n,
                           void* stream);
int vunet_act_fwd(const float* x, float* y, int32_t act, float slope, int64_t n, void* stream);

int vunet_reparam_fwd(const float* mu, const float* logstd, const float* eps, float* z, int64_t n, void* stream);
int vunet_reparam_bwd(const float* dz, const float* logstd, const float* eps, float* dmu, float* dlogstd,
                      int64_t n, void* stream);

int vunet_l1_mean_fwd(const float* a, const float* b, float* partial, float* out, float weight, int64_t n,
                      void* stream);
int vunet_l1_mean_bwd(const float* a, const float* b, const float* add, float* db, float gscale,
                      const float* gout, int64_t n, void* stream);
int vunet_l1_mean_bwd_amax(const float* a, const float* b, const float* add, float* db, float gscale,
                           const float* gout, int64_t n, float* amax_out, int32_t relu_mask, void* stream);

int vunet_kl_fwd(const float* mu, const float* logstd, float* partial, float* out, float weight, int32_t N, int64_t D,
                 void* stream);
int vunet_kl_bwd(const float* mu, const float* logstd, float* dmu, float* dlogstd, float gscale,
                 const float* gout, int64_t n, void* stream);
int vunet_sqdiff_fwd(const float* p, const float* q, float* partial, float* out, float weight, int32_t N, int64_t D,
                     void* stream);
int vunet_sqdiff_bwd(const float* p, const float* q, float* dp, float* dq, float gscale, const float* gout,
                     int64_t n, void* stream);

int vunet_vgg_preprocess(const float* x, float* y, int32_t N, int32_t H, int32_t W, void* stream);
int vunet_vgg_preprocess_bwd(const float* dy, const float* add, float* dx, int32_t N, int32_t H, int32_t W,
                             void* stream);
int vunet_maxpool2_fwd(const float* x, float* y, int32_t NC, int32_t H, int32_t W, void* stream);
int vunet_l1_pool_fwd(const float* a, const float* b, float* partial, float* out, float* y, float weight, int32_t NC,
                      int32_t H, int32_t W, void* stream);
int vunet_l1_pool_bwd(const float* a, const float* b, const float* dy_pool, float* db, float gscale, const float* gout,
                      int32_t NC, int32_t H, int32_t W, float* amax_out, int32_t relu_mask, void* stream);
int vunet_maxpool2_bwd_relu(const float* x, const float* y, const float* dy, float* dx, int32_t NC, int32_t H, int32_t W,
                            void* stream);
int vunet_maxpool2_bwd(const float* x, const float* y, const float* dy, float* dx, int32_t NC, int32_t H,
                       int32_t W, void* stream);

int vunet_instnorm_fwd(const float* x, float* y, float* stats, int32_t NC, int32_t HW, float eps, void* stream);
int vunet_instnorm_bwd(const float* y, const float* dy, const float* stats, float* dx, int32_t NC, int32_t HW,
                       void* stream);

int vunet_adam_step(float* param, const float* grad, float* exp_avg, float* exp_avg_sq, int64_t n, float lr,
                    float beta1, float beta2, float eps, float weight_decay, int32_t step, float grad_scale,
                    void* stream);

int vunet_adam_step_dev(float* param, const float* grad, float* exp_avg, float* exp_avg_sq, int64_t n,
                        const double* lr_dev, float beta1, float beta2, float eps, float weight_decay,
                        const int64_t* step_dev, float grad_scale, void* stream);

int vunet_set_dropout_step(const uint32_t* step_dev);

#define VUNET_TUNE_SPLIT_FORCE_NT 0
#define VUNET_TUNE_TILED_FORCE_NT 1
#define VUNET_TUNE_FORCE_SMALL 2
#define VUNET_TUNE_BLK_FORCE_NT 3
#define VUNET_TUNE_PARITY_LAUNCHES 4
#define VUNET_TUNE_BLK_WS 5
#define VUNET_TUNE_WGRAD_ROWSPLIT 6
#define VUNET_TUNE_S2_FWD_F32 7
#define VUNET_TUNE_P2_FORM 8
#define VUNET_TUNE_COUNT 9
int vunet_set_tuning(int32_t key, int32_t value);

int vunet_dropout_mask(float* mask, int64_t n, float p, uint32_t seed, void* stream);

int vunet_stickman_raster(const float* kps, int32_t B, int32_t J, const int32_t* body, int32_t n_body,
                          const int32_t* cmds, int32_t n_cmds, uint8_t* out_u8, float* out_f32, int32_t H, int32_t W,
                          void* stream);
int vunet_stickman_raster_thick(const float* kps, int32_t B, int32_t J, const int32_t* body, int32_t n_body,
                                const int32_t* cmds, int32_t n_cmds, uint8_t* out_u8, float* out_f32, int32_t H, int32_t W,
                                int32_t thickness, void* stream);
int vunet_u8_to_unit(const uint8_t* in, float* out, int64_t n, void* stream);

int vunet_ssim_partial(const float* x, const float* y, int32_t planes, int32_t H, int32_t W, float data_range,
                       const float* window11, float* partial, void* stream);

int vunet_dp_available(void);
int vunet_dp_unique_id(void* id128);
int vunet_dp_init(int32_t world, int32_t rank, const void* id128);
int vunet_dp_world(void);
int vunet_dp_allreduce_bucket(float* buf, int64_t n, int32_t average, void* stream);
int vunet_dp_finalize(void);

int vunet_crop_window(const float* x, float* y, int32_t planes, int32_t H, int32_t W, int32_t P, const int32_t* off,
                      void* stream);
int vunet_crop_window_bwd(const float* dy, float* dx, int32_t planes, int32_t H, int32_t W, int32_t P, const int32_t* off,
                          void* stream);

#define VUNET_LOSS_MAX_TERMS 8
int vunet_total_loss(const float* const* terms, int32_t n, const float* kl, const float* gamma, float gamma_const,
                     float ll_weight, int32_t use_kl, float* loss, float* ll, void* stream);
int vunet_total_loss_bwd(const float* g_loss, const float* g_ll, int32_t n, const float* gamma, float gamma_const,
                         float ll_weight, int32_t use_kl, float* d, void* stream);
int vunet_gamma_update(float* gamma, const float* imax, const float* avg_kl, float gamma_step, void* stream);

int vunet_unit_sample(const float* mu, const float* logstd, float* z, float* eps_out, int64_t n, uint32_t seed, void* stream);

int vunet_set_schedule(double* lr_dev, double lr, float* imax_dev, float imax, int32_t* step_dev, int32_t step, void* stream);

int vunet_sum_amax(const float* const* srcs, int32_t n, float* out, float* amax_out, int64_t numel, void* stream);

typedef struct vunet_p2_desc {
  int32_t N, C, H, W;
  int32_t M;
  int32_t relu;
} vunet_p2_desc;
int vunet_p2_conv_supported(const vunet_p2_desc* d);
int vunet_p2_conv_variant(const vunet_p2_desc* d, char* name, int32_t len);
int vunet_p2_conv(const vunet_p2_desc* d, const void* x, const int32_t* xmeta, const void* w_image, const float* wk,
                  const float* shift, const void* mask, void* y, int32_t* ymeta, void* stream);
int vunet_p2_weight_image_bytes(int32_t Cout, int32_t Cin, int32_t dgrad);
int vunet_p2_pack_weights(const float* w, const float* shift, int32_t Cout, int32_t Cin, int32_t dgrad, void* image, float* wk,
                          float* workspace, void* stream);
int vunet_p2_weight_bound(const float* w, const float* shift, int32_t Cout, int32_t Cin, float* wk, float* workspace, void* stream);
int vunet_p2_conv_first(const float* x, const float* amax_x, int32_t n_amax, const float* wt_f, int32_t Mpad, const float* shift,
                        const float* wk, void* y, int32_t* ymeta, int32_t N, int32_t H, int32_t W, int32_t M, void* stream);
int vunet_p2_from_nchw(const float* x, const float* amax, int32_t n_amax, int32_t relu, void* y, int32_t* ymeta, int32_t N,
                       int32_t C, int32_t H, int32_t W, void* stream);
int vunet_p2_to_nchw(const void* x, const int32_t* xmeta, float* y, int32_t N, int32_t C, int32_t H, int32_t W, void* stream);

int vunet_p2_l1_fwd(const void* t, const int32_t* tmeta, const void* p, const int32_t* pmeta, float* partial, float* out,
                    float weight, int32_t N, int32_t C, int32_t H, int32_t W, void* stream);
int vunet_p2_pool_fwd(const void* t, const int32_t* tmeta, const void* p, const int32_t* pmeta, float* partial, float* out,
                      float weight, void* y, int32_t* ymeta, int32_t N, int32_t C, int32_t H, int32_t W, void* stream);
int vunet_p2_l1_bwd(const void* t, const int32_t* tmeta, const void* p, const int32_t* pmeta, const void* add,
                    const int32_t* addmeta, void* g, int32_t* gmeta, float gscale, const float* gout, int32_t N, int32_t C,
                    int32_t H, int32_t W, void* stream);
int vunet_p2_pool_bwd(const void* t, const int32_t* tmeta, const void* p, const int32_t* pmeta, const void* dy,
                      const int32_t* dymeta, void* g, int32_t* gmeta, float gscale, const float* gout, int32_t N, int32_t C,
                      int32_t H, int32_t W, void* stream);

typedef struct vunet_seq_linear_desc {
  int32_t B, M, K, ldx, act0, act1, nets, shared_in, S;
} vunet_seq_linear_desc;
typedef struct vunet_seq_coupling_desc {
  int32_t B, C, c1, ld_in, ld_out, Mp, reverse, affine_on_src, S;
} vunet_seq_coupling_desc;
typedef struct vunet_seq_lstm_desc {
  int32_t B, H, ldx, hoff, n, ldraw;
  int64_t seq_stride;
} vunet_seq_lstm_desc;
int vunet_seq_linear(const vunet_seq_linear_desc* d, const float* w0, const float* w1, const float* x, const float* bias0,
                     const float* bias1, float* y, void* stream);
int vunet_seq_coupling(const vunet_seq_coupling_desc* d, const float* in, const float* st, const float* bias_s, const float* bias_t,
                       const int32_t* map, const float* scale, const float* loc, float* out, float* logdet, void* stream);
int vunet_seq_start(const float* x0, int64_t x0_stride, const float* h0, const float* c0, float* xraw, int32_t ldraw, float* xh,
                    int32_t ldx, int32_t hoff, float* c, int32_t B, int32_t n, int32_t H, void* stream);
int vunet_seq_lstm_gates(const vunet_seq_lstm_desc* d, const float* w_perm, const float* xh, const float* bias_perm, const float* c_in,
                         float* c_out, float* xh_next, float* h_out, const float* x_next, void* stream);
int vunet_seq_decoder_out(const vunet_seq_lstm_desc* d, float* xh, const float* w_out, const float* b_out, float* xraw, float* xs,
                          float* cs, void* stream);
int vunet_seq_lstm_bias(const float* b_ih, const float* b_hh, const float* fold, int32_t H, float* bias_perm, void* stream);
int vunet_seq_fold_input(const float* w_ih, const float* w_in, const float* b_in, int32_t M, int32_t n, float* w_fold,
                         float* bias_fold, void* stream);
int vunet_seq_bottleneck(const float* heads, int32_t Mp, const float* eps, float* mu, float* logstd, float* b_out, int32_t B,
                         int32_t H, void* stream);
int vunet_seq_pack_rows(const float* src, int32_t M, int32_t K, const float* row_scale, float* dst, int32_t ld_dst, int32_t col_off,
                        int32_t row_off, int32_t row_mul, void* stream);
int vunet_seq_pose_project(const float* x, int32_t n_use, const int32_t* dims_to_use, const double* mean, const double* stdv, int32_t D,
                           int32_t f32_math, const double* cam, float* kps, int32_t T, int32_t J, void* stream);
int vunet_seq_actnorm_init(const float* x, int32_t ld, int32_t B, int32_t C, float* loc, float* scale, void* stream);
int vunet_seq_normlinear_rows(const float* v, const float* g, const float* bias, const float* gamma, const float* beta, int32_t M,
                              int32_t K, float* row_scale, float* bias_eff, void* stream);

int vunet_seq_slerp(const float* b1, const float* b2, int64_t ld_in, int pairs, int h, const double* steps, int n_steps, float* out,
                    void* stream);

#ifdef __cplusplus
}
#endif
#endif
```

Baseline: 776.5 frames/s.

## Fuse 2x2 max-pool and L1 perceptual loss into VGG p2 conv epilogue

Adds epilogue variants to the h2 split-fp16 VGG conv kernel that compute the following 2x2 max-pool (via DPP and shuffle lane exchanges) and the per-tap L1 loss against the target features directly from register results. Each block writes a loss partial, and a small finish kernel reduces them. The VGG forward path uses the fused variant when a conv is followed by a pool or carries a loss tap. This removes separate pool and L1 kernels and their re-reads of the conv output, at the cost of a larger epilogue and more register pressure in the conv kernel.

```diff
diff --git a/behavior_driven_video_synthesis_amd/csrc/conv_p2.hip b/behavior_driven_video_synthesis_amd/csrc/conv_p2.hip
--- a/behavior_driven_video_synthesis_amd/csrc/conv_p2.hip
+++ b/behavior_driven_video_synthesis_amd/csrc/conv_p2.hip
@@ -20,7 +20,13 @@
   int* ymeta;
   int N, C, H, W, M;
   int relu;
+  uint4* ypool;
+  int* ypoolmeta;
+  const uint4* t;
+  const int* tmeta;
+  float* partial;
 };
+constexpr int P2_EPI_POOL = 1, P2_EPI_L1 = 2;
 
 __device__ __forceinline__ void p2_dma(uint32_t voff, const void* sbase, uint32_t lds_addr) {
   uint32_t keep;
@@ -66,165 +72,72 @@
   return __builtin_bit_cast(uint32_t, v);
 }
 
-template <int NW, int CT, int XBUF>
-__global__ __launch_bounds__(64 * NW, NW == 8 ? 1 : 2) void conv_p2_kernel(const P2Args a) {
-  static_assert(NW == 4 || NW == 8, "waves");
-  static_assert(CT == 32 || CT == 16, "tile width");
-  constexpr int MW = 16 * NW;
-  constexpr int RT = 8, IH = RT + 2, CW = CT + 2, XPIX = IH * CW, XU = 8 * XPIX;
-  constexpr int NXI = (XU + 63) / 64, XS = NXI * 64;
-  constexpr int NXW = (NXI + NW - 1) / NW;
-  constexpr int WU = MW * 8;
-  constexpr int NWI = WU / 64 / NW;
+__device__ __forceinline__ void p2_unpack(const uint4& h, const uint4& l, float inv, float* v) {
+  const uint32_t hs[4] = {h.x, h.y, h.z, h.w}, ls[4] = {l.x, l.y, l.z, l.w};
+#pragma unroll
+  for (int j = 0; j < 4; ++j) {
+    const h2_f16x2 a = __builtin_bit_cast(h2_f16x2, hs[j]), b = __builtin_bit_cast(h2_f16x2, ls[j]);
+    v[2 * j] = ((float)a[0] + (float)b[0] * (1.f / 2048.f)) * inv;
+    v[2 * j + 1] = ((float)a[1] + (float)b[1] * (1.f / 2048.f)) * inv;
+  }
+}
+
+__device__ __forceinline__ uint4 p2_from_lane_xor1(const uint4& v) {
+  auto f = [](uint32_t x) { return (uint32_t)__builtin_amdgcn_update_dpp(0, (int)x, 0xB1 , 0xF, 0xF, true); };
+  return make_uint4(f(v.x), f(v.y), f(v.z), f(v.w));
+}
+__device__ __forceinline__ uint4 p2_from_lane_xor16(const uint4& v) {
+  return make_uint4(__shfl_xor(v.x, 16, 64), __shfl_xor(v.y, 16, 64), __shfl_xor(v.z, 16, 64), __shfl_xor(v.w, 16, 64));
+}
+
+__device__ __forceinline__ void p2_max_unit(uint4& ah, uint4& al, const uint4& bh, const uint4& bl, float inv) {
+  float va[8], vb[8];
+  p2_unpack(ah, al, inv, va);
+  p2_unpack(bh, bl, inv, vb);
+  uint32_t xh[4] = {ah.x, ah.y, ah.z, ah.w}, xl[4] = {al.x, al.y, al.z, al.w};
+  const uint32_t yh[4] = {bh.x, bh.y, bh.z, bh.w}, yl[4] = {bl.x, bl.y, bl.z, bl.w};
+#pragma unroll
+  for (int j = 0; j < 4; ++j) {
+    const uint32_t take = (va[2 * j] == fmaxf(va[2 * j], vb[2 * j]) ? 0u : 0x0000FFFFu) |
+                          (va[2 * j + 1] == fmaxf(va[2 * j + 1], vb[2 * j + 1]) ? 0u : 0xFFFF0000u);
+    xh[j] = (xh[j] & ~take) | (yh[j] & take);
+    xl[j] = (xl[j] & ~take) | (yl[j] & take);
+  }
+  ah = make_uint4(xh[0], xh[1], xh[2], xh[3]);
+  al = make_uint4(xl[0], xl[1], xl[2], xl[3]);
+}
+
+template <int NW, int CT, int EPI>
+__device__ __forceinline__ void p2_epilogue(const P2Args& a, const f32x4 (&acc)[4][CT / 8], const f32x4 (&acx)[4][CT / 8],
+                                            float descale, float descale2, float sy, int ey, int n, int row0, int col0, int m0,
+                                            int wave, int lane) {
   constexpr int PTR = CT / 16, NPT = 2 * PTR;
-  static_assert(XBUF == 1 || NXW <= 8, "the next chunk's pieces ride on the first taps");
-  extern __shared__ __attribute__((aligned(16))) uint4 smem[];
-  uint4* const xL = smem;
-  uint4* const wL = smem + XBUF * XS;
-
-  const int tid = threadIdx.x, lane = tid & 63;
-  const int wave = __builtin_amdgcn_readfirstlane(tid >> 6);
+  constexpr bool POOL = (EPI & P2_EPI_POOL) != 0, L1 = (EPI & P2_EPI_L1) != 0;
   const int mg = wave >> 2, rg = wave & 3;
   const int px = lane & 15, cg = lane >> 4;
-  const int Hp = a.H + 2, Wp = a.W + 2, CB = a.C >> 3, MB = a.M >> 3;
-
-  const unsigned bid = xcd_remap(blockIdx.x, gridDim.x);
-  const int mblocks = a.M / MW;
-  const int mb = bid % mblocks;
-  int t = bid / mblocks;
-  const int tiles_w = a.W / CT, tiles_h = a.H / RT;
-  const int tx = t % tiles_w;
-  t /= tiles_w;
-  const int ty = t % tiles_h;
-  const int n = t / tiles_h;
-  const int row0 = ty * RT, col0 = tx * CT, m0 = mb * MW;
-
-  uint32_t xoff[NXW];
-#pragma unroll
-  for (int i = 0; i < NXW; ++i) {
-    int j = wave + NW * i;
-    if (j >= NXI) j = NXI - 1;
-    int u = 64 * j + lane;
-    if (u >= XU) u = XU - 1;
-    const int p = u / (4 * XPIX);
-    int rem = u - p * 4 * XPIX;
-    const int kq = rem / XPIX;
-    rem -= kq * XPIX;
-    const int r = rem / CW, c = rem - r * CW;
-    xoff[i] = (uint32_t)((((size_t)p * a.N * CB + kq) * Hp + (row0 + r)) * Wp + col0 + c) * 16u;
-  }
-  const uint32_t xL_addr = (uint32_t)(uintptr_t)(__attribute__((address_space(3))) void*)xL;
-  const uint32_t wL_addr = (uint32_t)(uintptr_t)(__attribute__((address_space(3))) void*)wL;
-  const char* const xsrc0 = reinterpret_cast<const char*>(a.x) + (size_t)n * CB * Hp * Wp * 16;
-  const size_t xchunk = (size_t)4 * Hp * Wp * 16;
-  const char* const wsrc0 = reinterpret_cast<const char*>(a.w) + (size_t)mb * (MW / 16) * 128 * 16;
-  const size_t wslab = (size_t)(a.M / 16) * 128 * 16;
-  const uint32_t lane16 = (uint32_t)lane * 16u;
-
-  auto issue_x = [&](int ch, int i) {
-    int j = wave + NW * i;
-    if (j >= NXI) j = NXI - 1;
-    const int xb = XBUF == 2 ? (ch & 1) : 0;
-    p2_dma(xoff[i], p2_uniform_ptr(xsrc0 + (size_t)ch * xchunk), xL_addr + (uint32_t)(xb * XS + 64 * j) * 16u);
-  };
-  auto issue_w = [&](int g, int buf) {
-    const char* src = wsrc0 + (size_t)g * wslab;
-#pragma unroll
-    for (int i = 0; i < NWI; ++i) {
-      const int part = wave * NWI + i;
-      p2_dma(lane16, p2_uniform_ptr(src + (size_t)part * 1024), wL_addr + (uint32_t)(buf * WU + part * 64) * 16u);
-    }
-  };
-
-  issue_w(0, 0);
-#pragma unroll
-  for (int i = 0; i < NXW; ++i) issue_x(0, i);
-
-  float descale, descale2, sy;
-  {
-    const int ex = a.xmeta[0];
-    const float amax_x = p2_meta_amax(a.xmeta, lane);
-    const int ew = (int)a.wk[2];
-    h2_pow2_pair(-(ex + ew), descale, descale2);
-    const float bound = a.wk[0] * amax_x + a.wk[1];
-    const int ey = h2_scale_exp(bound);
-    sy = h2_pow2(ey);
-    if (blockIdx.x == 0 && tid == 0) a.ymeta[0] = ey;
-  }
-
-  f32x4 acc[4][NPT], acx[4][NPT];
-#pragma unroll
-  for (int mt = 0; mt < 4; ++mt)
-#pragma unroll
-    for (int q = 0; q < NPT; ++q)
-#pragma unroll
-      for (int r = 0; r < 4; ++r) acc[mt][q][r] = acx[mt][q][r] = 0.f;
-
-  p2_dma_wait<0>();
-  __syncthreads();
-
-  const int nch = a.C >> 5;
-  const uint4* const wA0 = wL + (mg * 4) * 128 + lane;
-  const uint4* const xB0 = xL + cg * XPIX + px + (2 * rg) * CW;
-
-  auto chunk = [&](int ch, auto last_c) {
-    constexpr bool LAST = decltype(last_c)::value;
-    const uint4* const xB = xB0 + (XBUF == 2 ? (ch & 1) * XS : 0);
-    const int wpar = (ch * 9) & 1;
-#pragma unroll
-    for (int tap = 0; tap < 9; ++tap) {
-      const int kh = tap / 3, kw = tap - 3 * kh;
-      const int g = ch * 9 + tap;
-      const int buf = wpar ^ (tap & 1);
-      constexpr bool dummy = false;
-      (void)dummy;
-      const bool more_w = !(LAST && tap == 8);
-      const bool xpiece = XBUF == 2 && !LAST && tap < NXW;
-      if (more_w) issue_w(g + 1, buf ^ 1);
-      if (xpiece) issue_x(ch + 1, tap);
-      const uint4* const wA = wA0 + buf * WU;
-      P2Unit av[2][4], bv[2][NPT];
-#pragma unroll
-      for (int p = 0; p < 2; ++p) {
-#pragma unroll
-        for (int mt = 0; mt < 4; ++mt) av[p][mt].u = wA[(mt * 2 + p) * 64];
-#pragma unroll
-        for (int q = 0; q < NPT; ++q) bv[p][q].u = xB[p * 4 * XPIX + (q / PTR + kh) * CW + (q % PTR) * 16 + kw];
-      }
-#pragma unroll
-      for (int mt = 0; mt < 4; ++mt)
-#pragma unroll
-        for (int q = 0; q < NPT; ++q)
-          acx[mt][q] = __builtin_amdgcn_mfma_f32_16x16x32_f16(av[1][mt].b, bv[0][q].b, acx[mt][q], 0, 0, 0);
-#pragma unroll
-      for (int mt = 0; mt < 4; ++mt)
-#pragma unroll
-        for (int q = 0; q < NPT; ++q)
-          acx[mt][q] = __builtin_amdgcn_mfma_f32_16x16x32_f16(av[0][mt].b, bv[1][q].b, acx[mt][q], 0, 0, 0);
-#pragma unroll
-      for (int mt = 0; mt < 4; ++mt)
-#pragma unroll
-        for (int q = 0; q < NPT; ++q)
-          acc[mt][q] = __builtin_amdgcn_mfma_f32_16x16x32_f16(av[0][mt].b, bv[0][q].b, acc[mt][q], 0, 0, 0);
-      __builtin_amdgcn_sched_barrier(0);
-      if (more_w) {
-        if (xpiece) p2_dma_wait<1>();
-        else p2_dma_wait<0>();
-        __syncthreads();
-        if (XBUF == 1 && tap == 8) {
-#pragma unroll
-          for (int i = 0; i < NXW; ++i) issue_x(ch + 1, i);
-          p2_dma_wait<0>();
-          __syncthreads();
-        }
-      }
-    }
-  };
-  for (int ch = 0; ch + 1 < nch; ++ch) chunk(ch, std::false_type{});
-  chunk(nch - 1, std::true_type{});
-
+  const int Hp = a.H + 2, Wp = a.W + 2, MB = a.M >> 3;
   const bool relu = a.relu != 0;
   const size_t plane = (size_t)a.N * MB * Hp * Wp;
+  auto unit_off = [&](int mt, int qp) {
+    const int q = qp + (cg & 1);
+    const int orow = row0 + 2 * rg + q / PTR, ocol = col0 + (q % PTR) * 16 + px;
+    const int cb = ((m0 + 64 * mg + 16 * mt) >> 3) + (cg >> 1);
+    return (((size_t)n * MB + cb) * Hp + (orow + 1)) * Wp + (ocol + 1);
+  };
+  uint4 tu[2][2];
+  float ip = 0.f, it = 0.f, l1 = 0.f;
+  auto load_t = [&](int u) {
+    const size_t o = unit_off(u / PTR, 2 * (u % PTR));
+    tu[u & 1][0] = a.t[o];
+    tu[u & 1][1] = a.t[plane + o];
+  };
+  if constexpr (L1) {
+    load_t(0);
+    it = h2_pow2(-a.tmeta[0]);
+  }
+  if constexpr (EPI != 0) ip = h2_pow2(-ey);
+  const int Hpo = (a.H >> 1) + 2, Wpo = (a.W >> 1) + 2;
+  const size_t plane_o = (size_t)a.N * MB * Hpo * Wpo;
   float ymax = 0.f;
 #pragma unroll
   for (int mt = 0; mt < 4; ++mt) {
@@ -234,8 +147,12 @@
       const float4 s4 = *reinterpret_cast<const float4*>(a.shift + co);
       sh[0] = s4.x; sh[1] = s4.y; sh[2] = s4.z; sh[3] = s4.w;
     }
+    uint4 wh, wl;
 #pragma unroll
     for (int qp = 0; qp < NPT; qp += 2) {
+      const int u = mt * PTR + qp / 2;
+      if constexpr (L1)
+        if (u + 1 < 4 * PTR) load_t(u + 1);
       uint32_t hh[2][2], ll[2][2];
 #pragma unroll
       for (int s = 0; s < 2; ++s) {
@@ -256,10 +173,7 @@
       p2_swap16(ll[0][1], ll[1][1]);
       uint4 uh = make_uint4(hh[0][0], hh[0][1], hh[1][0], hh[1][1]);
       uint4 ul = make_uint4(ll[0][0], ll[0][1], ll[1][0], ll[1][1]);
-      const int q = qp + (cg & 1);
-      const int orow = row0 + 2 * rg + q / PTR, ocol = col0 + (q % PTR) * 16 + px;
-      const int cb = ((m0 + 64 * mg + 16 * mt) >> 3) + (cg >> 1);
-      const size_t o = (((size_t)n * MB + cb) * Hp + (orow + 1)) * Wp + (ocol + 1);
+      const size_t o = unit_off(mt, qp);
       if (a.mask) {
         const uint4 mh = a.mask[o], ml = a.mask[plane + o];
         const uint32_t k0 = p2_nonzero_halves((mh.x | ml.x) & 0x7FFF7FFFu), k1 = p2_nonzero_halves((mh.y | ml.y) & 0x7FFF7FFFu);
@@ -269,17 +183,238 @@
       }
       a.y[o] = uh;
       a.y[plane + o] = ul;
-    }
+      if constexpr (L1) {
+        float pv[8], tv[8];
+        p2_unpack(tu[u & 1][0], tu[u & 1][1], it, tv);
+        p2_unpack(uh, ul, ip, pv);
+        l1 += ((fabsf(tv[0] - pv[0]) + fabsf(tv[1] - pv[1])) + (fabsf(tv[2] - pv[2]) + fabsf(tv[3] - pv[3]))) +
+              ((fabsf(tv[4] - pv[4]) + fabsf(tv[5] - pv[5])) + (fabsf(tv[6] - pv[6]) + fabsf(tv[7] - pv[7])));
+      }
+      if constexpr (POOL) {
+        p2_max_unit(uh, ul, p2_from_lane_xor1(uh), p2_from_lane_xor1(ul), ip);
+        bool store = !(px & 1);
+        if constexpr (CT == 32) {
+          if (qp == 0) {
+            wh = uh;
+            wl = ul;
+            store = false;
+          } else {
+            p2_max_unit(wh, wl, uh, ul, ip);
+            uh = wh;
+            ul = wl;
+          }
+        } else {
+          p2_max_unit(uh, ul, p2_from_lane_xor16(uh), p2_from_lane_xor16(ul), ip);
+          store = store && !(cg & 1);
+        }
+        if (store) {
+          const int prow = (row0 >> 1) + rg, pcol = (col0 >> 1) + (CT == 32 ? 8 * (cg & 1) : 0) + (px >> 1);
+          const int cb = ((m0 + 64 * mg + 16 * mt) >> 3) + (cg >> 1);
+          const size_t oo = (((size_t)n * MB + cb) * Hpo + (prow + 1)) * Wpo + (pcol + 1);
+          a.ypool[oo] = uh;
+          a.ypool[plane_o + oo] = ul;
+        }
+      }
+    }
+    if constexpr (EPI != 0) __builtin_amdgcn_sched_barrier(0);
   }
   {
     const float m_ = wave_max(ymax);
-    if (lane == 0)
-      atomicMax(reinterpret_cast<unsigned*>(a.ymeta) + P2_AMAX0 + ((blockIdx.x * NW + wave) & (P2_NSLOT - 1)), __float_as_uint(m_));
-  }
-}
-
-template <int CT>
-__global__ __launch_bounds__(512, 1) void conv_p2a_kernel(const P2Args a) {
+    if (lane == 0) {
+      const unsigned slot = P2_AMAX0 + ((blockIdx.x * NW + wave) & (P2_NSLOT - 1));
+      atomicMax(reinterpret_cast<unsigned*>(a.ymeta) + slot, __float_as_uint(m_));
+      if constexpr (POOL) atomicMax(reinterpret_cast<unsigned*>(a.ypoolmeta) + slot, __float_as_uint(m_));
+    }
+  }
+  if constexpr (L1) {
+    __shared__ float red[NW];
+    const float w_ = wave_sum(l1);
+    if (lane == 0) red[wave] = w_;
+    __syncthreads();
+    if (threadIdx.x == 0) {
+      float tot = red[0];
+#pragma unroll
+      for (int i = 1; i < NW; ++i) tot += red[i];
+      a.partial[blockIdx.x] = tot;
+    }
+  }
+}
+
+template <int NW, int CT, int XBUF, int EPI>
+__device__ __forceinline__ void conv_p2_body(const P2Args& a) {
+  static_assert(NW == 4 || NW == 8, "waves");
+  static_assert(CT == 32 || CT == 16, "tile width");
+  constexpr int MW = 16 * NW;
+  constexpr int RT = 8, IH = RT + 2, CW = CT + 2, XPIX = IH * CW, XU = 8 * XPIX;
+  constexpr int NXI = (XU + 63) / 64, XS = NXI * 64;
+  constexpr int NXW = (NXI + NW - 1) / NW;
+  constexpr int WU = MW * 8;
+  constexpr int NWI = WU / 64 / NW;
+  constexpr int PTR = CT / 16, NPT = 2 * PTR;
+  static_assert(XBUF == 1 || NXW <= 8, "the next chunk's pieces ride on the first taps");
+  extern __shared__ __attribute__((aligned(16))) uint4 smem[];
+  uint4* const xL = smem;
+  uint4* const wL = smem + XBUF * XS;
+
+  const int tid = threadIdx.x, lane = tid & 63;
+  const int wave = __builtin_amdgcn_readfirstlane(tid >> 6);
+  const int mg = wave >> 2, rg = wave & 3;
+  const int px = lane & 15, cg = lane >> 4;
+  const int Hp = a.H + 2, Wp = a.W + 2, CB = a.C >> 3, MB = a.M >> 3;
+
+  const unsigned bid = xcd_remap(blockIdx.x, gridDim.x);
+  const int mblocks = a.M / MW;
+  const int mb = bid % mblocks;
+  int t = bid / mblocks;
+  const int tiles_w = a.W / CT, tiles_h = a.H / RT;
+  const int tx = t % tiles_w;
+  t /= tiles_w;
+  const int ty = t % tiles_h;
+  const int n = t / tiles_h;
+  const int row0 = ty * RT, col0 = tx * CT, m0 = mb * MW;
+
+  uint32_t xoff[NXW];
+#pragma unroll
+  for (int i = 0; i < NXW; ++i) {
+    int j = wave + NW * i;
+    if (j >= NXI) j = NXI - 1;
+    int u = 64 * j + lane;
+    if (u >= XU) u = XU - 1;
+    const int p = u / (4 * XPIX);
+    int rem = u - p * 4 * XPIX;
+    const int kq = rem / XPIX;
+    rem -= kq * XPIX;
+    const int r = rem / CW, c = rem - r * CW;
+    xoff[i] = (uint32_t)((((size_t)p * a.N * CB + kq) * Hp + (row0 + r)) * Wp + col0 + c) * 16u;
+  }
+  const uint32_t xL_addr = (uint32_t)(uintptr_t)(__attribute__((address_space(3))) void*)xL;
+  const uint32_t wL_addr = (uint32_t)(uintptr_t)(__attribute__((address_space(3))) void*)wL;
+  const char* const xsrc0 = reinterpret_cast<const char*>(a.x) + (size_t)n * CB * Hp * Wp * 16;
+  const size_t xchunk = (size_t)4 * Hp * Wp * 16;
+  const char* const wsrc0 = reinterpret_cast<const char*>(a.w) + (size_t)mb * (MW / 16) * 128 * 16;
+  const size_t wslab = (size_t)(a.M / 16) * 128 * 16;
+  const uint32_t lane16 = (uint32_t)lane * 16u;
+
+  auto issue_x = [&](int ch, int i) {
+    int j = wave + NW * i;
+    if (j >= NXI) j = NXI - 1;
+    const int xb = XBUF == 2 ? (ch & 1) : 0;
+    p2_dma(xoff[i], p2_uniform_ptr(xsrc0 + (size_t)ch * xchunk), xL_addr + (uint32_t)(xb * XS + 64 * j) * 16u);
+  };
+  auto issue_w = [&](int g, int buf) {
+    const char* src = wsrc0 + (size_t)g * wslab;
+#pragma unroll
+    for (int i = 0; i < NWI; ++i) {
+      const int part = wave * NWI + i;
+      p2_dma(lane16, p2_uniform_ptr(src + (size_t)part * 1024), wL_addr + (uint32_t)(buf * WU + part * 64) * 16u);
+    }
+  };
+
+  issue_w(0, 0);
+#pragma unroll
+  for (int i = 0; i < NXW; ++i) issue_x(0, i);
+
+  float descale, descale2, sy;
+  int ey;
+  {
+    const int ex = a.xmeta[0];
+    const float amax_x = p2_meta_amax(a.xmeta, lane);
+    const int ew = (int)a.wk[2];
+    h2_pow2_pair(-(ex + ew), descale, descale2);
+    const float bound = a.wk[0] * amax_x + a.wk[1];
+    ey = h2_scale_exp(bound);
+    sy = h2_pow2(ey);
+    if (blockIdx.x == 0 && tid == 0) {
+      a.ymeta[0] = ey;
+      if constexpr ((EPI & P2_EPI_POOL) != 0) a.ypoolmeta[0] = ey;
+    }
+  }
+
+  f32x4 acc[4][NPT], acx[4][NPT];
+#pragma unroll
+  for (int mt = 0; mt < 4; ++mt)
+#pragma unroll
+    for (int q = 0; q < NPT; ++q)
+#pragma unroll
+      for (int r = 0; r < 4; ++r) acc[mt][q][r] = acx[mt][q][r] = 0.f;
+
+  p2_dma_wait<0>();
+  __syncthreads();
+
+  const int nch = a.C >> 5;
+  const uint4* const wA0 = wL + (mg * 4) * 128 + lane;
+  const uint4* const xB0 = xL + cg * XPIX + px + (2 * rg) * CW;
+
+  auto chunk = [&](int ch, auto last_c) {
+    constexpr bool LAST = decltype(last_c)::value;
+    const uint4* const xB = xB0 + (XBUF == 2 ? (ch & 1) * XS : 0);
+    const int wpar = (ch * 9) & 1;
+#pragma unroll
+    for (int tap = 0; tap < 9; ++tap) {
+      const int kh = tap / 3, kw = tap - 3 * kh;
+      const int g = ch * 9 + tap;
+      const int buf = wpar ^ (tap & 1);
+      constexpr bool dummy = false;
+      (void)dummy;
+      const bool more_w = !(LAST && tap == 8);
+      const bool xpiece = XBUF == 2 && !LAST && tap < NXW;
+      if (more_w) issue_w(g + 1, buf ^ 1);
+      if (xpiece) issue_x(ch + 1, tap);
+      const uint4* const wA = wA0 + buf * WU;
+      P2Unit av[2][4], bv[2][NPT];
+#pragma unroll
+      for (int p = 0; p < 2; ++p) {
+#pragma unroll
+        for (int mt = 0; mt < 4; ++mt) av[p][mt].u = wA[(mt * 2 + p) * 64];
+#pragma unroll
+        for (int q = 0; q < NPT; ++q) bv[p][q].u = xB[p * 4 * XPIX + (q / PTR + kh) * CW + (q % PTR) * 16 + kw];
+      }
+#pragma unroll
+      for (int mt = 0; mt < 4; ++mt)
+#pragma unroll
+        for (int q = 0; q < NPT; ++q)
+          acx[mt][q] = __builtin_amdgcn_mfma_f32_16x16x32_f16(av[1][mt].b, bv[0][q].b, acx[mt][q], 0, 0, 0);
+#pragma unroll
+      for (int mt = 0; mt < 4; ++mt)
+#pragma unroll
+        for (int q = 0; q < NPT; ++q)
+          acx[mt][q] = __builtin_amdgcn_mfma_f32_16x16x32_f16(av[0][mt].b, bv[1][q].b, acx[mt][q], 0, 0, 0);
+#pragma unroll
+      for (int mt = 0; mt < 4; ++mt)
+#pragma unroll
+        for (int q = 0; q < NPT; ++q)
+          acc[mt][q] = __builtin_amdgcn_mfma_f32_16x16x32_f16(av[0][mt].b, bv[0][q].b, acc[mt][q], 0, 0, 0);
+      __builtin_amdgcn_sched_barrier(0);
+      if (more_w) {
+        if (xpiece) p2_dma_wait<1>();
+        else p2_dma_wait<0>();
+        __syncthreads();
+        if (XBUF == 1 && tap == 8) {
+#pragma unroll
+          for (int i = 0; i < NXW; ++i) issue_x(ch + 1, i);
+          p2_dma_wait<0>();
+          __syncthreads();
+        }
+      }
+    }
+  };
+  for (int ch = 0; ch + 1 < nch; ++ch) chunk(ch, std::false_type{});
+  chunk(nch - 1, std::true_type{});
+
+  p2_epilogue<NW, CT, EPI>(a, acc, acx, descale, descale2, sy, ey, n, row0, col0, m0, wave, lane);
+}
+
+template <int NW, int CT, int XBUF>
+__global__ __launch_bounds__(64 * NW, NW == 8 ? 1 : 2) void conv_p2_kernel(const P2Args a) {
+  conv_p2_body<NW, CT, XBUF, 0>(a);
+}
+template <int NW, int CT, int XBUF, int EPI>
+__global__ __launch_bounds__(64 * NW, NW == 8 ? 1 : 2) void conv_p2_taps_kernel(const P2Args a) {
+  conv_p2_body<NW, CT, XBUF, EPI>(a);
+}
+
+template <int CT, int EPI>
+__device__ __forceinline__ void conv_p2a_body(const P2Args& a) {
   constexpr int NW = 8, MW = 128;
   constexpr int RT = 8, IH = RT + 2, CW = CT + 2, XPIX = IH * CW, XU = 8 * XPIX;
   constexpr int NXI = (XU + 63) / 64, XS = NXI * 64;
@@ -351,15 +486,19 @@
     for (int i = 0; i < NXG; ++i) issue_x(0, i);
   }
   float descale, descale2, sy;
+  int ey;
   {
     const int ex = a.xmeta[0];
     const float amax_x = p2_meta_amax(a.xmeta, lane);
     const int ew = (int)a.wk[2];
     h2_pow2_pair(-(ex + ew), descale, descale2);
     const float bound = a.wk[0] * amax_x + a.wk[1];
-    const int ey = h2_scale_exp(bound);
+    ey = h2_scale_exp(bound);
     sy = h2_pow2(ey);
-    if (blockIdx.x == 0 && tid == 0) a.ymeta[0] = ey;
+    if (blockIdx.x == 0 && tid == 0) {
+      a.ymeta[0] = ey;
+      if constexpr ((EPI & P2_EPI_POOL) != 0) a.ypoolmeta[0] = ey;
+    }
   }
   f32x4 acc[4][NPT], acx[4][NPT];
 #pragma unroll
@@ -433,82 +572,49 @@
   chunk(nch - 1, std::true_type{});
   if (mg == 0) __builtin_amdgcn_s_barrier();
 
-  const bool relu = a.relu != 0;
-  const size_t plane = (size_t)a.N * MB * Hp * Wp;
-  float ymax = 0.f;
-#pragma unroll
-  for (int mt = 0; mt < 4; ++mt) {
-    const int co = m0 + 64 * mg + 16 * mt + 4 * cg;
-    float sh[4] = {0.f, 0.f, 0.f, 0.f};
-    if (a.shift) {
-      const float4 s4 = *reinterpret_cast<const float4*>(a.shift + co);
-      sh[0] = s4.x; sh[1] = s4.y; sh[2] = s4.z; sh[3] = s4.w;
-    }
-#pragma unroll
-    for (int qp = 0; qp < NPT; qp += 2) {
-      uint32_t hh[2][2], ll[2][2];
-#pragma unroll
-      for (int s = 0; s < 2; ++s) {
-        float v[4];
-#pragma unroll
-        for (int r = 0; r < 4; ++r) {
-          float c = (acc[mt][qp + s][r] + acx[mt][qp + s][r] * (1.f / 2048.f)) * descale * descale2 + sh[r];
-          c = (relu && !(c > 0.f)) ? 0.f : c;
-          ymax = fmaxf(ymax, fabsf(c));
-          v[r] = c * sy;
-        }
-        h2_split2(v[0], v[1], hh[s][0], ll[s][0]);
-        h2_split2(v[2], v[3], hh[s][1], ll[s][1]);
-      }
-      p2_swap16(hh[0][0], hh[1][0]);
-      p2_swap16(hh[0][1], hh[1][1]);
-      p2_swap16(ll[0][0], ll[1][0]);
-      p2_swap16(ll[0][1], ll[1][1]);
-      uint4 uh = make_uint4(hh[0][0], hh[0][1], hh[1][0], hh[1][1]);
-      uint4 ul = make_uint4(ll[0][0], ll[0][1], ll[1][0], ll[1][1]);
-      const int q = qp + (cg & 1);
-      const int orow = row0 + 2 * rg + q / PTR, ocol = col0 + (q % PTR) * 16 + px;
-      const int cb = ((m0 + 64 * mg + 16 * mt) >> 3) + (cg >> 1);
-      const size_t o = (((size_t)n * MB + cb) * Hp + (orow + 1)) * Wp + (ocol + 1);
-      if (a.mask) {
-        const uint4 mh = a.mask[o], ml = a.mask[plane + o];
-        const uint32_t k0 = p2_nonzero_halves((mh.x | ml.x) & 0x7FFF7FFFu), k1 = p2_nonzero_halves((mh.y | ml.y) & 0x7FFF7FFFu);
-        const uint32_t k2 = p2_nonzero_halves((mh.z | ml.z) & 0x7FFF7FFFu), k3 = p2_nonzero_halves((mh.w | ml.w) & 0x7FFF7FFFu);
-        uh.x &= k0; uh.y &= k1; uh.z &= k2; uh.w &= k3;
-        ul.x &= k0; ul.y &= k1; ul.z &= k2; ul.w &= k3;
-      }
-      a.y[o] = uh;
-      a.y[plane + o] = ul;
-    }
-  }
-  {
-    const float m_ = wave_max(ymax);
-    if (lane == 0)
-      atomicMax(reinterpret_cast<unsigned*>(a.ymeta) + P2_AMAX0 + ((blockIdx.x * NW + wave) & (P2_NSLOT - 1)), __float_as_uint(m_));
-  }
+  p2_epilogue<NW, CT, EPI>(a, acc, acx, descale, descale2, sy, ey, n, row0, col0, m0, wave, lane);
 }
 
 template <int CT>
+__global__ __launch_bounds__(512, 1) void conv_p2a_kernel(const P2Args a) {
+  conv_p2a_body<CT, 0>(a);
+}
+template <int CT, int EPI>
+__global__ __launch_bounds__(512, 1) void conv_p2a_taps_kernel(const P2Args a) {
+  conv_p2a_body<CT, EPI>(a);
+}
+
+template <int CT, int EPI = 0>
 int p2a_launch(const P2Args& a, hipStream_t st) {
   constexpr int XU = 8 * 10 * (CT + 2), XS = (XU + 63) / 64 * 64, WU = 128 * 8;
   constexpr size_t lds = (size_t)(2 * XS + 2 * WU) * 16;
   const int blocks = a.N * (a.H / 8) * (a.W / CT) * (a.M / 128);
-  auto kern = conv_p2a_kernel<CT>;
+  void (*kern)(const P2Args);
+  if constexpr (EPI == 0) kern = conv_p2a_kernel<CT>;
+  else kern = conv_p2a_taps_kernel<CT, EPI>;
   if (hipFuncSetAttribute((const void*)kern, hipFuncAttributeMaxDynamicSharedMemorySize, (int)lds) != hipSuccess) return VUNET_ERR_LAUNCH;
   VUNET_LAUNCH(kern, dim3((unsigned)blocks), dim3(512), lds, st, a);
   return vunet_check_launch();
 }
 
-template <int NW, int CT, int XBUF>
+template <int NW, int CT, int XBUF, int EPI = 0>
 int p2_launch(const P2Args& a, hipStream_t st) {
   constexpr int XU = 8 * 10 * (CT + 2), XS = (XU + 63) / 64 * 64, WU = 16 * NW * 8;
   constexpr size_t lds = (size_t)(XBUF * XS + 2 * WU) * 16;
   const int blocks = a.N * (a.H / 8) * (a.W / CT) * (a.M / (16 * NW));
-  auto kern = conv_p2_kernel<NW, CT, XBUF>;
+  void (*kern)(const P2Args);
+  if constexpr (EPI == 0) kern = conv_p2_kernel<NW, CT, XBUF>;
+  else kern = conv_p2_taps_kernel<NW, CT, XBUF, EPI>;
   if (lds > 64 * 1024 && hipFuncSetAttribute((const void*)kern, hipFuncAttributeMaxDynamicSharedMemorySize, (int)lds) != hipSuccess)
     return VUNET_ERR_LAUNCH;
   VUNET_LAUNCH(kern, dim3((unsigned)blocks), dim3(64 * NW), lds, st, a);
   return vunet_check_launch();
+}
+
+template <int EPI>
+int p2_taps_launch(const P2Args& a, int form, hipStream_t st) {
+  if (a.W == 16) return form == 8 ? p2a_launch<16, EPI>(a, st) : p2_launch<4, 16, 1, EPI>(a, st);
+  return form == 8 ? p2a_launch<32, EPI>(a, st) : p2_launch<4, 32, 1, EPI>(a, st);
 }
 
 }
@@ -538,11 +644,36 @@
   a.x = (const uint4*)x; a.xmeta = xmeta; a.w = (const uint4*)w_image; a.wk = wk; a.shift = shift; a.mask = (const uint4*)mask;
   a.y = (uint4*)y; a.ymeta = ymeta;
   a.N = d->N; a.C = d->C; a.H = d->H; a.W = d->W; a.M = d->M; a.relu = d->relu;
+  a.ypool = nullptr; a.ypoolmeta = nullptr; a.t = nullptr; a.tmeta = nullptr; a.partial = nullptr;
   hipStream_t st = (hipStream_t)stream;
   const int form = p2_form(d);
   const bool lockstep = g_vunet_tune[VUNET_TUNE_P2_FORM] == 3;
   if (d->W == 16) return form == 8 ? (lockstep ? p2_launch<8, 16, 2>(a, st) : p2a_launch<16>(a, st)) : p2_launch<4, 16, 1>(a, st);
   return form == 8 ? (lockstep ? p2_launch<8, 32, 2>(a, st) : p2a_launch<32>(a, st)) : p2_launch<4, 32, 1>(a, st);
+}
+
+extern "C" int vunet_p2_conv_taps_partials(const vunet_p2_desc* d) {
+  if (!p2_shape_ok(d)) return VUNET_ERR_UNSUPPORTED;
+  return d->N * (d->H / 8) * (d->W / (d->W == 16 ? 16 : 32)) * (d->M / (16 * p2_form(d)));
+}
+
+extern "C" int vunet_p2_conv_taps(const vunet_p2_desc* d, const void* x, const int32_t* xmeta, const void* w_image, const float* wk,
+                                  const float* shift, const void* mask, void* y, int32_t* ymeta, void* ypool, int32_t* ypoolmeta,
+                                  const void* t, const int32_t* tmeta, float* partial, void* stream) {
+  if (!ypool && !t) return vunet_p2_conv(d, x, xmeta, w_image, wk, shift, mask, y, ymeta, stream);
+  if (!d || !x || !xmeta || !w_image || !wk || !y || !ymeta) return VUNET_ERR_ARG;
+  if (!p2_shape_ok(d)) return VUNET_ERR_UNSUPPORTED;
+  if (mask || !d->relu || (ypool && !ypoolmeta) || (t && (!tmeta || !partial))) return VUNET_ERR_ARG;
+  if (((uintptr_t)x | (uintptr_t)w_image | (uintptr_t)y | (uintptr_t)shift | (uintptr_t)ypool | (uintptr_t)t) & 15) return VUNET_ERR_ARG;
+  P2Args a;
+  a.x = (const uint4*)x; a.xmeta = xmeta; a.w = (const uint4*)w_image; a.wk = wk; a.shift = shift; a.mask = nullptr;
+  a.y = (uint4*)y; a.ymeta = ymeta;
+  a.N = d->N; a.C = d->C; a.H = d->H; a.W = d->W; a.M = d->M; a.relu = 1;
+  a.ypool = (uint4*)ypool; a.ypoolmeta = ypoolmeta; a.t = (const uint4*)t; a.tmeta = tmeta; a.partial = partial;
+  hipStream_t st = (hipStream_t)stream;
+  const int form = p2_form(d);
+  if (ypool && t) return p2_taps_launch<P2_EPI_POOL | P2_EPI_L1>(a, form, st);
+  return ypool ? p2_taps_launch<P2_EPI_POOL>(a, form, st) : p2_taps_launch<P2_EPI_L1>(a, form, st);
 }
 
 extern "C" int vunet_p2_conv_variant(const vunet_p2_desc* d, char* name, int32_t len) {
@@ -712,15 +843,6 @@
     y[plane + o] = l;
   }
 }
-__device__ __forceinline__ void p2_unpack(const uint4& h, const uint4& l, float inv, float* v) {
-  const uint32_t hs[4] = {h.x, h.y, h.z, h.w}, ls[4] = {l.x, l.y, l.z, l.w};
-#pragma unroll
-  for (int j = 0; j < 4; ++j) {
-    const h2_f16x2 a = __builtin_bit_cast(h2_f16x2, hs[j]), b = __builtin_bit_cast(h2_f16x2, ls[j]);
-    v[2 * j] = ((float)a[0] + (float)b[0] * (1.f / 2048.f)) * inv;
-    v[2 * j + 1] = ((float)a[1] + (float)b[1] * (1.f / 2048.f)) * inv;
-  }
-}
 __global__ __launch_bounds__(256) void p2_to_nchw_kernel(const uint4* __restrict__ x, const int* __restrict__ xmeta,
                                                          float* __restrict__ y, int N, int C, int H, int W) {
   const int CB = C >> 3, Hp = H + 2, Wp = W + 2;
diff --git a/behavior_driven_video_synthesis_amd/csrc/planes.hip b/behavior_driven_video_synthesis_amd/csrc/planes.hip
--- a/behavior_driven_video_synthesis_amd/csrc/planes.hip
+++ b/behavior_driven_video_synthesis_amd/csrc/planes.hip
@@ -243,6 +243,12 @@
   return vunet_check_launch();
 }
 
+extern "C" int vunet_p2_finish_sum(const float* partial, int32_t n, float* out, float scale, void* stream) {
+  if (!partial || !out || n < 1) return VUNET_ERR_ARG;
+  VUNET_LAUNCH(p2_finish_sum_kernel, dim3(1), dim3(256), 0, (hipStream_t)stream, partial, (int)n, out, scale);
+  return vunet_check_launch();
+}
+
 extern "C" int vunet_p2_pool_fwd(const void* t, const int32_t* tmeta, const void* p, const int32_t* pmeta, float* partial, float* out,
                                  float weight, void* y, int32_t* ymeta, int32_t N, int32_t C, int32_t H, int32_t W, void* stream) {
   if (!p || !pmeta || !y || !ymeta || C % 8 || N < 1 || (H & 1) || (W & 1)) return VUNET_ERR_ARG;
diff --git a/behavior_driven_video_synthesis_amd/models/imagenet_pretrained.py b/behavior_driven_video_synthesis_amd/models/imagenet_pretrained.py
--- a/behavior_driven_video_synthesis_amd/models/imagenet_pretrained.py
+++ b/behavior_driven_video_synthesis_amd/models/imagenet_pretrained.py
@@ -85,6 +85,13 @@
 _p2_switch = {"on": __import__("os").environ.get("VUNET_VGG_P2", "1") != "0"}
 
 
+_p2_fused_taps = {"on": __import__("os").environ.get("VUNET_P2_FUSED_TAPS", "1") != "0"}
+
+
+def enable_p2_fused_taps(on: bool = True):
+    _p2_fused_taps["on"] = bool(on)
+
+
 def enable_p2(on: bool = True):
     _p2_switch["on"] = bool(on)
 
@@ -207,16 +214,27 @@
                   ops._p(A[0].buf), ops._p(A[0].meta), n, h, w, A[0].shape[1], ops._stream())
         taps, losses = {}, {}
         steps = self.program[1]
+        fused = _p2_fused_taps["on"]
+        pooled = set()
         for k, step in enumerate(steps, start=1):
             if step[0] == "conv":
-                ops.p2_conv(A[k - 1], self._weights(step[1]), A[k], relu=True)
                 tap = step[2]
+                pool_next = k < len(steps) and steps[k][0] == "pool"
+                t = targets[tap] if (targets is not None and tap is not None) else None
+                if fused and (pool_next or t is not None):
+                    loss = ops.p2_conv_taps(A[k - 1], self._weights(step[1]), A[k], pool=A[k + 1] if pool_next else None, t=t,
+                                            weight=0.0 if t is None else tap_weights[tap])
+                    if t is not None:
+                        losses[tap] = loss
+                    if pool_next:
+                        pooled.add(k + 1)
+                else:
+                    ops.p2_conv(A[k - 1], self._weights(step[1]), A[k], relu=True)
+                    if t is not None and not pool_next:
+                        losses[tap] = ops.p2_l1_fwd(t, A[k], tap_weights[tap])
                 if tap is not None:
                     taps[tap] = A[k]
-                    pool_next = k < len(steps) and steps[k][0] == "pool"
-                    if targets is not None and not pool_next:
-                        losses[tap] = ops.p2_l1_fwd(targets[tap], A[k], tap_weights[tap])
-            else:
+            elif k not in pooled:
                 prev = steps[k - 2] if k >= 2 else None
                 tap = prev[2] if (prev is not None and prev[0] == "conv") else None
                 if targets is not None and tap is not None:
diff --git a/behavior_driven_video_synthesis_amd/ops.py b/behavior_driven_video_synthesis_amd/ops.py
--- a/behavior_driven_video_synthesis_amd/ops.py
+++ b/behavior_driven_video_synthesis_amd/ops.py
@@ -1705,6 +1705,44 @@
     return out
 
 
+def p2_conv_taps(x: Planes, wts: P2Weights, out: Planes, pool: Planes = None, t: Planes = None, weight: float = 0.0):
+    if pool is None and t is None:
+        p2_conv(x, wts, out, relu=True)
+        return None
+    n, c, h, w = x.shape
+    m = wts.cout
+    assert c == wts.cin and out.shape == (n, m, h, w)
+    assert pool is None or pool.shape == (n, m, h // 2, w // 2)
+    assert t is None or t.shape == out.shape
+    img, wk = wts.image(False)
+    d = P2Desc(n, c, h, w, m, 1)
+    loss = partial = None
+    nparts = 0
+    if t is not None:
+        nparts = _lib.lib().vunet_p2_conv_taps_partials(ctypes.byref(d))
+        if nparts < 1:
+            raise RuntimeError(f"vunet_p2_conv_taps_partials failed ({nparts})")
+        loss = _zero_scalar(x.buf.device)
+        partial = torch.empty(nparts, device=x.buf.device, dtype=torch.float32)
+    timer = _NO_TIMER
+    if _prof["on"]:
+        buf = ctypes.create_string_buffer(96)
+        _call("vunet_p2_conv_variant", ctypes.byref(d), buf, 96)
+        epi = (1 if pool is not None else 0) | (2 if t is not None else 0)
+        name = buf.value.decode()
+        if name.startswith("conv_p2_kernel<8"):
+            name = f"conv_p2a_kernel<{16 if w == 16 else 32}>"
+        name = name.replace("_kernel<", "_taps_kernel<")[:-1] + f", {epi}>"
+        timer = _Timed(("conv_gather_fwd", n, c, 0, h, w, m, 3, 1, 0, name), 2.0 * n * h * w * c * m * 9)
+    with timer:
+        _call("vunet_p2_conv_taps", ctypes.byref(d), _p(x.buf), _p(x.meta), _p(img), _p(wk), _p(wts.bias), None, _p(out.buf), _p(out.meta),
+              _p(None if pool is None else pool.buf), _p(None if pool is None else pool.meta), _p(None if t is None else t.buf),
+              _p(None if t is None else t.meta), _p(partial), _stream())
+    if t is not None:
+        _call("vunet_p2_finish_sum", _p(partial), nparts, _p(loss), float(weight) / (float(n) * m * h * w), _stream())
+    return loss
+
+
 def p2_l1_fwd(t: Planes, p: Planes, weight: float):
     n, c, h, w = p.shape
     assert t.shape == p.shape
diff --git a/include/vunet_hip.h b/include/vunet_hip.h
--- a/include/vunet_hip.h
+++ b/include/vunet_hip.h
@@ -272,6 +272,11 @@
 int vunet_p2_conv_variant(const vunet_p2_desc* d, char* name, int32_t len);
 int vunet_p2_conv(const vunet_p2_desc* d, const void* x, const int32_t* xmeta, const void* w_image, const float* wk,
                   const float* shift, const void* mask, void* y, int32_t* ymeta, void* stream);
+int vunet_p2_conv_taps_partials(const vunet_p2_desc* d);
+int vunet_p2_conv_taps(const vunet_p2_desc* d, const void* x, const int32_t* xmeta, const void* w_image, const float* wk,
+                       const float* shift, const void* mask, void* y, int32_t* ymeta, void* ypool, int32_t* ypoolmeta,
+                       const void* t, const int32_t* tmeta, float* partial, void* stream);
+int vunet_p2_finish_sum(const float* partial, int32_t n, float* out, float scale, void* stream);
 int vunet_p2_weight_image_bytes(int32_t Cout, int32_t Cin, int32_t dgrad);
 int vunet_p2_pack_weights(const float* w, const float* shift, int32_t Cout, int32_t Cin, int32_t dgrad, void* image, float* wk,
                           float* workspace, void* stream);
```

Measured after the change: 780.6 frames/s (median of 6 runs). About the same (+0.5%).
